# LabJunBMI/E3-invaraint-diffusion-model

Hardware: AMD Instinct MI355X
Metric: denoising-steps/sec (batched pocket graphs) (higher is better)
Workload: dtype f32 storage and accumulation, f16x3 products (fp32 grade); 1 GPU; structure_model sampling step, 256 x 256-residue pockets per GPU, 12+12 layers x 768, T=1000 schedule, encoder recomputed every step (as the reference); pockets_per_gpu=256, seq_len=256, parallelism=pocket-sharded x1, no collective

## Files before the change

### e3-invaraint-diffusion-model_amd/autograd.py

```python
import os

import torch

from . import hip, ops
from .ops import _chk, _p, _stream


def gemm_general(a, a_kmajor, b, b_kmajor, M, N, K, bias=None, act=ops.ACT_NONE, mode=None):
    _chk(a, "gemm_general.a"); _chk(b, "gemm_general.b"); _chk(bias, "gemm_general.bias")
    assert a.dim() == 2 and b.dim() == 2 and a.stride(1) == 1 and b.stride(1) == 1
    out = torch.empty((M, N), device=a.device, dtype=torch.float32)
    terms = ops.GEMM_MODES[ops.GEMM_MODE if mode is None else mode] or 6
    hip.check(hip.lib().e3d_gemm_f32_split_general(_p(a), a.stride(0), int(a_kmajor), _p(b), b.stride(0),
                                                   int(b_kmajor), _p(bias), _p(out), out.stride(0), M, N, K, act,
                                                   terms, _stream()), "e3d_gemm_f32_split_general")
    return out


class deferred_weight_grads:
    active = None

    MAX_BYTES = int(float(os.environ.get("E3D_DEFER_WGRAD_MAX_GB", "16")) * 2 ** 30)

    OVERLAP = os.environ.get("E3D_WGRAD_OVERLAP", "0") == "1"
# ... 406 lines not shown
    @staticmethod
    def forward(ctx, x, residual, gamma, beta, eps, p_drop=0.0, row_keys=None):
        ctx.drop = ops.site_drop(p_drop, row_keys) if p_drop and p_drop > 0 else None
        out, s = ops.residual_layernorm(x, residual, gamma, beta, eps, want_s=True, drop=ctx.drop)
        ctx.save_for_backward(s, gamma)
        ctx.eps, ctx.has_res = eps, residual is not None
        return out

    @staticmethod
    def backward(ctx, dy):
        s, gamma = ctx.saved_tensors
        if ctx.drop is not None:
            ds, dg, db, dsd = layernorm_bwd(dy.contiguous(), s, gamma, ctx.eps, drop=ctx.drop)
            return dsd, (ds if ctx.has_res else None), dg, db, None, None, None
        ds, dg, db = layernorm_bwd(dy.contiguous(), s, gamma, ctx.eps)
        return ds, (ds if ctx.has_res else None), dg, db, None, None, None


class _AdaLNGate(torch.autograd.Function):
    @staticmethod
    def forward(ctx, x, y, mod, branch, rows_per_cond):
        ctx.save_for_backward(y, mod)
        ctx.branch, ctx.rpc = branch, rows_per_cond
        return ops.adaln_gate(x, y, mod, branch, rows_per_cond)

    @staticmethod
    def backward(ctx, dout):
        y, mod = ctx.saved_tensors
        dout = dout.contiguous()
        M, H = y.shape
        dy = torch.empty_like(y)
        dmod = torch.zeros_like(mod)
        hip.check(hip.lib().e3d_adaln_gate_bwd(_p(dout), _p(y), _p(mod), ctx.branch, ctx.rpc, _p(dy), _p(dmod), M, H,
                                               _stream()), "e3d_adaln_gate_bwd")
        return dout, dy, dmod, None, None


class _EmbedLayerNorm(torch.autograd.Function):

    @staticmethod
    def forward(ctx, x, weight, bias, gamma, beta, eps, post_add, rows_per_add):
        out, z = ops.embed_layernorm(x, weight, bias, gamma, beta, eps, post_add, rows_per_add, want_z=True)
        ctx.save_for_backward(x, z, gamma)
        ctx.eps, ctx.rpa, ctx.has_add = eps, rows_per_add, post_add is not None
        return out

    @staticmethod
    def backward(ctx, dout):
        x, z, gamma = ctx.saved_tensors
        dout = dout.contiguous()
        dz, dg, db_ln = layernorm_bwd(dout, z, gamma, ctx.eps)
        dW, db = small_k_wgrad(dz, x)
        dadd = group_sum(dout, ctx.rpa) if (ctx.has_add and ctx.needs_input_grad[6]) else None
        return None, dW, db, dg, db_ln, None, dadd, None


class _HeadLinear(torch.autograd.Function):
    @staticmethod
    def forward(ctx, x, weight, bias):
        ctx.save_for_backward(x, weight)
        return ops.head_linear(x, weight, bias)

    @staticmethod
    def backward(ctx, dout):
        x, weight = ctx.saved_tensors
        dout = dout.contiguous()
        M, H = x.shape
        dx = torch.empty_like(x)
        hip.check(hip.lib().e3d_head_linear_bwd_dx(_p(dout), _p(weight), _p(dx), M, H, weight.shape[0], _stream()),
                  "e3d_head_linear_bwd_dx")
        dW, _ = small_k_wgrad(x, dout, transpose_out=True, want_bias=False)
        return dx, dW, colsum(dout)


FUSE_HIDDEN_DROPOUT = os.environ.get("E3D_FUSE_HIDDEN_DROPOUT", "1") == "1"


def _needs_grad(*tensors):
    return torch.is_grad_enabled() and any(t is not None and t.requires_grad for t in tensors)


class functional:
    @staticmethod
    def linear(x, weight, bias=None, act=ops.ACT_NONE, absmax=None, planes_for=None):
        if _needs_grad(x, weight, bias):
            out = _Linear.apply(x, weight, bias, act, absmax)
        elif planes_for is not None and absmax is None and ops.gemm_planes_ok(x, weight, bias, act, planes_for[0].shape[0],
                                                                              planes_for[1]):
            return ops.gemm(x, weight, bias, act, planes_out=True)
        else:
            out = ops.gemm(x, weight, bias, act, absmax=absmax)
        if absmax is not None:
            out._e3d_absmax = absmax
        return out

    @staticmethod
    def attention(q_src, kv_src, B, nh, Lq, Lk, key_mask=None, dist_emb=None, max_pos=0, drop_p=0.0, row_keys=None,
                  planes_for=None):
        q_abs = getattr(q_src, "_e3d_absmax", None)
        k_abs = q_abs if kv_src is None else getattr(kv_src, "_e3d_absmax", None)
        bounds = (q_abs, k_abs) if q_abs is not None and k_abs is not None else None
        if _needs_grad(q_src, kv_src, dist_emb):
            return _Attention.apply(q_src, kv_src, dist_emb, key_mask, B, nh, Lq, Lk, max_pos, drop_p, bounds, row_keys)
        q, k, v = _Attention._views(q_src, kv_src, nh * 64)
        drop = ops.site_drop(drop_p, row_keys) if drop_p > 0 else None
        planes = (planes_for is not None and drop is None and
                  ops.attention_planes_ok(q, k, v, nh, Lq, Lk, planes_for[0].shape[0], planes_for[1]))
        return ops.attention(q, k, v, B, nh, Lq, Lk, key_mask=key_mask, dist_emb=dist_emb, max_pos=max_pos, drop=drop,
                             bounds=bounds, planes_out=planes)

    @staticmethod
    def dropout(x, p, training=True, row_keys=None):
        if not training or not p:
            return x
        if _needs_grad(x):
            return _Dropout.apply(x, p, row_keys)
        p, seed = ops.site_drop(p, row_keys)[:2]
        return ops.dropout(x.contiguous(), p, seed, row_keys=row_keys)

    @staticmethod
    def residual_layernorm(x, residual, gamma, beta, eps, p_drop=0.0, row_keys=None):
        if _needs_grad(x, residual, gamma, beta):
            return _ResidualLayerNorm.apply(x, residual, gamma, beta, eps, p_drop, row_keys)
        drop = ops.site_drop(p_drop, row_keys) if p_drop and p_drop > 0 else None
        return ops.residual_layernorm(x, residual, gamma, beta, eps, drop=drop)

    @staticmethod
    def linear_residual_layernorm(x, weight, bias, residual, gamma, beta, eps, p_drop=0.0, row_keys=None):
        if not p_drop and not _needs_grad(x, weight, bias, residual, gamma, beta):
            return ops.linear_residual_layernorm(x, weight, bias, residual, gamma, beta, eps)
        fn = functional
        if FUSE_HIDDEN_DROPOUT:
            return fn.residual_layernorm(fn.linear(x, weight, bias), residual, gamma, beta, eps, p_drop, row_keys)
        return fn.residual_layernorm(fn.dropout(fn.linear(x, weight, bias), p_drop, row_keys=row_keys), residual, gamma, beta, eps)

    @staticmethod
    def adaln_gate(x, y, mod, branch, rows_per_cond):
        if _needs_grad(x, y, mod):
            return _AdaLNGate.apply(x, y, mod, branch, rows_per_cond)
        return ops.adaln_gate(x, y, mod, branch, rows_per_cond)

    @staticmethod
    def embed_layernorm(x, weight, bias, gamma, beta, eps, post_add=None, rows_per_add=1):
        if _needs_grad(weight, bias, gamma, beta, post_add):
            return _EmbedLayerNorm.apply(x, weight, bias, gamma, beta, eps, post_add, rows_per_add)
        return ops.embed_layernorm(x, weight, bias, gamma, beta, eps, post_add, rows_per_add)

    @staticmethod
    def head_linear(x, weight, bias):
        if _needs_grad(x, weight, bias):
            return _HeadLinear.apply(x, weight, bias)
        return ops.head_linear(x, weight, bias)
```

### e3-invaraint-diffusion-model_amd/bert.py

```python
from dataclasses import dataclass

import os

import torch
from torch import nn

from . import ops
from .autograd import functional as F


@dataclass
class BertConfig:
    hidden_size: int = 768
    num_attention_heads: int = 12
    intermediate_size: int = 1024
    num_hidden_layers: int = 12
    max_position_embeddings: int = 64
    position_embedding_type: str = "relative_key"
    hidden_dropout_prob: float = 0.1
    attention_probs_dropout_prob: float = 0.1
    layer_norm_eps: float = 1e-12
    hidden_act: str = "gelu"
    use_cache: bool = False
    is_decoder: bool = False
# ... 92 lines not shown

    @staticmethod
    def backward(ctx, gw, gb):
        gws = gw.split(ctx.rows, 0) if gw is not None else (None,) * ctx.n
        gbs = gb.split(ctx.rows, 0) if gb is not None else (None,) * ctx.n
        return (None, None, None) + tuple(gws) + tuple(gbs)


def _tie(owner, name, tensors):
    tied = owner.__dict__.setdefault("_e3d_tied", {})
    ent = tied.get(name)
    ok = ent is not None and ent.device == tensors[0].device
    if ok:
        at = ent.data_ptr()
        for t in tensors:
            if t.data_ptr() != at or not t.is_contiguous():
                ok = False
                break
            at += 4 * t.numel()
    if not ok:
        with torch.no_grad():
            ent = torch.cat([t.detach() for t in tensors], dim=0).contiguous()
            r0 = 0
            for t in tensors:
                t.data = ent[r0:r0 + t.shape[0]]
                r0 += t.shape[0]
        tied[name] = ent
    return ent


def _packed(owner, name, weights, biases):
    if torch.is_grad_enabled() and any(t.requires_grad for t in weights):
        if TIE_PACKED and all(t.dtype == torch.float32 for t in list(weights) + list(biases)):
            w, b = _TiedPack.apply(_tie(owner, "w_" + name, weights), _tie(owner, "b_" + name, biases), len(weights),
                                   *weights, *biases)
        else:
            w, b = torch.cat(list(weights), dim=0), torch.cat(list(biases), dim=0)
        w._e3d_parts, b._e3d_parts = list(weights), list(biases)
        return w, b
    out = []
    cache = owner.__dict__.setdefault("_e3d_pack", {})
    for key_name, tensors in (("w_" + name, weights), ("b_" + name, biases)):
        key = ops.weight_key(*tensors)
        hit = cache.get(key_name)
        if hit is None or hit[0] != key:
            with torch.no_grad():
                hit = (key, torch.cat([t.detach() for t in tensors], dim=0).contiguous())
            cache[key_name] = hit
        out.append(hit[1])
    return out[0], out[1]


def qkv_weights(sa):
    return _packed(sa, "qkv", [sa.query.weight, sa.key.weight, sa.value.weight], [sa.query.bias, sa.key.bias, sa.value.bias])


def kv_weights(sa):
    return _packed(sa, "kv", [sa.key.weight, sa.value.weight], [sa.key.bias, sa.value.bias])


def dropout_rates(module):
    if not module.training:
        return 0.0, 0.0
    cfg = module.config
    return float(getattr(cfg, "hidden_dropout_prob", 0.0)), float(getattr(cfg, "attention_probs_dropout_prob", 0.0))


def _attention_output(att, ctx, x, p_hidden=0.0, row_keys=None):
    return F.linear_residual_layernorm(ctx, att.output.dense.weight, att.output.dense.bias, x, att.output.LayerNorm.weight,
                                       att.output.LayerNorm.bias, att.eps, p_hidden, row_keys)


def _planes_for(att, x, drop):
    return (att.output.dense.weight, x) if drop[0] == 0 and drop[1] == 0 else None


def drop_keys(drop):
    return drop[2] if len(drop) > 2 else None


def run_self_attention(att, x, mask, B, L, drop=(0.0, 0.0), layout=None):
    sa = att.self
    w, b = qkv_weights(sa)
    qkv = F.linear(x, w, b, absmax=ops.absmax_slot(sa, "qkv", x.device))
    relkey = sa.position_embedding_type == "relative_key"
    if layout is not None:
        H = att.num_heads * 64
        ctx = ops.attention_varlen(qkv[:, :H], qkv[:, H:2 * H], qkv[:, 2 * H:], layout, layout, att.num_heads,
                                   dist_emb=sa.distance_embedding.weight if relkey else None,
                                   max_pos=sa.max_position_embeddings)
        return _attention_output(att, ctx, x)
    ctx = F.attention(qkv, None, B, att.num_heads, L, L, key_mask=mask,
                      dist_emb=sa.distance_embedding.weight if relkey else None,
                      max_pos=sa.max_position_embeddings, drop_p=drop[1], row_keys=drop_keys(drop),
                      planes_for=_planes_for(att, x, drop))
    return _attention_output(att, ctx, x, drop[0], drop_keys(drop))


def project_cross_kv(att, enc):
    w, b = kv_weights(att.self)
    return F.linear(enc, w, b, absmax=torch.zeros(1, device=enc.device, dtype=torch.float32))


def run_cross_attention(att, x, kv, enc_mask, B, Lq, Lk, drop=(0.0, 0.0), layout=None, enc_layout=None):
    q = F.linear(x, att.self.query.weight, att.self.query.bias, absmax=ops.absmax_slot(att.self, "q", x.device))
    if layout is not None:
        H = att.num_heads * 64
        ctx = ops.attention_varlen(q, kv[:, :H], kv[:, H:], layout, enc_layout, att.num_heads)
        return _attention_output(att, ctx, x)
    ctx = F.attention(q, kv, B, att.num_heads, Lq, Lk, key_mask=enc_mask, drop_p=drop[1], row_keys=drop_keys(drop),
                      planes_for=_planes_for(att, x, drop))
    return _attention_output(att, ctx, x, drop[0], drop_keys(drop))


def run_layer(layer, x, mask, B, L, cross_kv=None, enc_mask=None, Lk=None, drop=(0.0, 0.0), layout=None,
              enc_layout=None):
    x = run_self_attention(layer.attention, x, mask, B, L, drop, layout=layout)
    if hasattr(layer, "crossattention"):
        if cross_kv is None:
            raise ValueError("decoder layer needs encoder states")
        x = run_cross_attention(layer.crossattention, x, cross_kv, enc_mask, B, L, Lk, drop, layout=layout,
                                enc_layout=enc_layout)
    inter = F.linear(x, layer.intermediate.dense.weight, layer.intermediate.dense.bias, ops.ACT_GELU,
                     planes_for=(layer.output.dense.weight, x) if drop[0] == 0 and drop[1] == 0 else None)
    return F.linear_residual_layernorm(inter, layer.output.dense.weight, layer.output.dense.bias, x,
                                       layer.output.LayerNorm.weight, layer.output.LayerNorm.bias, layer.eps, drop[0],
                                       drop_keys(drop))


def run_encoder(encoder, x, mask, B, L, enc=None, enc_mask=None, Lk=None, cross_kv=None, layout=None, enc_layout=None,
                row_keys=None):
    drop = dropout_rates(encoder)
    if layout is not None and drop != (0.0, 0.0):
        raise RuntimeError("packed layouts are inference-only: put the model in eval mode")
    if row_keys is not None:
        drop = drop + (row_keys,)
    for i, layer in enumerate(encoder.layer):
        kv = None
        if hasattr(layer, "crossattention"):
            kv = cross_kv[i] if cross_kv is not None else project_cross_kv(layer.crossattention, enc)
        x = run_layer(layer, x, mask, B, L, kv, enc_mask, Lk, drop, layout=layout, enc_layout=enc_layout)
    return x
```

### e3-invaraint-diffusion-model_amd/csrc/attn_relkey_coop.hip

```cpp
#include <type_traits>

#include "e3d_common.h"

namespace {

typedef __bf16 bf16x8 __attribute__((ext_vector_type(8)));
typedef __bf16 bf16x4 __attribute__((ext_vector_type(4)));
typedef _Float16 f16x8 __attribute__((ext_vector_type(8)));
typedef _Float16 f16x4 __attribute__((ext_vector_type(4)));
template <typename E> struct AV;
template <> struct AV<__bf16> { typedef bf16x8 x8; typedef bf16x4 x4; };
template <> struct AV<_Float16> { typedef f16x8 x8; typedef f16x4 x4; };
template <typename X> struct Elem;
template <> struct Elem<bf16x8> { typedef __bf16 type; };
template <> struct Elem<bf16x4> { typedef __bf16 type; };
template <> struct Elem<f16x8> { typedef _Float16 type; };
template <> struct Elem<f16x4> { typedef _Float16 type; };
__device__ __forceinline__ f32x16 mma16(const bf16x8 a, const bf16x8 b, const f32x16 c) {
    return __builtin_amdgcn_mfma_f32_32x32x16_bf16(a, b, c, 0, 0, 0);
}
__device__ __forceinline__ f32x16 mma16(const f16x8 a, const f16x8 b, const f32x16 c) {
    return __builtin_amdgcn_mfma_f32_32x32x16_f16(a, b, c, 0, 0, 0);
}

constexpr int D = 64;
constexpr int RING_LD = 34;
constexpr int RING_F = 64 * RING_LD;
constexpr int OUT_LD = 68;
constexpr int K_ROW_B = 144;
constexpr int V_ROW_B = 192;
constexpr int K_PLANE_B = 32 * K_ROW_B, V_PLANE_B = 32 * V_ROW_B;
constexpr float LOG2E = 1.4426950408889634f, LN2 = 0.6931471805599453f;
constexpr float Q_SCALE = 0.125f * LOG2E;
constexpr float MASK_BIAS = -10000.0f * LOG2E;
float g_rescale_tau = 8.0f;
constexpr int KV_BUF_B = 2 * K_PLANE_B + 2 * V_PLANE_B + 128;

template <typename X4>
__device__ __forceinline__ void split4x2(const f32x4 v, X4& hi, X4& lo) {
    typedef typename Elem<X4>::type E;
#pragma unroll
    for (int j = 0; j < 4; ++j) {
        const E p = (E)v[j];
        hi[j] = p;
        lo[j] = (E)(v[j] - (float)p);
    }
}

template <typename X8>
__device__ __forceinline__ void split8x2(const float (&x)[8], X8& hi, X8& lo) {
    typedef typename Elem<X8>::type E;
#pragma unroll
    for (int j = 0; j < 8; ++j) {
        const E p = (E)x[j];
        hi[j] = p;
        lo[j] = (E)(x[j] - (float)p);
    }
}

__device__ __forceinline__ void split4x2(const f32x4 v, f16x4& hi, f16x4& lo) {
    e3d_f16x2 h0, l0, h1, l1;
    e3d_split2_f16(v[0], v[1], h0, l0);
    e3d_split2_f16(v[2], v[3], h1, l1);
    hi = f16x4{h0[0], h0[1], h1[0], h1[1]};
    lo = f16x4{l0[0], l0[1], l1[0], l1[1]};
}
__device__ __forceinline__ void split8x2(const float (&x)[8], f16x8& hi, f16x8& lo) {
#pragma unroll
    for (int j = 0; j < 8; j += 2) {
        e3d_f16x2 h, l;
        e3d_split2_f16(x[j], x[j + 1], h, l);
        hi[j] = h[0]; hi[j + 1] = h[1];
        lo[j] = l[0]; lo[j + 1] = l[1];
    }
}

template <typename X8>
__device__ __forceinline__ f32x16 mfma3(const X8 (&a)[2], const X8 (&b)[2], f32x16 acc) {
    acc = mma16(a[0], b[1], acc);
    acc = mma16(a[1], b[0], acc);
    acc = mma16(a[0], b[0], acc);
    return acc;
}

typedef short short4v __attribute__((ext_vector_type(4)));
typedef short short8v __attribute__((ext_vector_type(8)));
template <typename X8>
__device__ __forceinline__ X8 tr_read8(const unsigned char* lo4, const unsigned char* hi4) {
    typedef __attribute__((address_space(3))) short4v* lds_p;
    const short4v a = __builtin_amdgcn_ds_read_tr16_b64_v4i16((lds_p)(lo4));
    const short4v b = __builtin_amdgcn_ds_read_tr16_b64_v4i16((lds_p)(hi4));
    const short8v c = __builtin_shufflevector(a, b, 0, 1, 2, 3, 4, 5, 6, 7);
    return __builtin_bit_cast(X8, c);
}

template <typename E>
__global__ __launch_bounds__(256) void e_fragments_kernel(const float* __restrict__ e, typename AV<E>::x8* __restrict__ frag,
                                                          int P, int J0, int n_items, float* __restrict__ e_absmax) {
    const int i = blockIdx.x * 256 + threadIdx.x;
    if (i >= n_items) return;
    const int lane = i & 63, kb = (i >> 6) & 3, plane = (i >> 8) & 1, j = i >> 9;
    const int row = min(max(P + 32 * (j - J0) + (lane & 31), 0), 2 * P - 2);
    const float* src = e + row * D + 16 * kb + 8 * (lane >> 5);
    typename AV<E>::x8 out;
    unsigned amax = 0;
#pragma unroll
    for (int t = 0; t < 8; ++t) {
        const float v = src[t];
        const E hi = (E)v;
        out[t] = plane ? (E)(v - (float)hi) : hi;
        e3d_absmax_accum(amax, v);
    }
    frag[i] = out;
    if (e_absmax && plane == 0) e3d_absmax_commit(amax, e_absmax, lane);
}

#ifdef E3D_ATTN_STAMPS
__device__ long long e3d_attn_stamps[16][8];
#define ASTAMP(slot)                                                                                     \
    do {                                                                                                 \
        if (blockIdx.x == 1000 && wid == 1 && lane == 0 && kt < 16) e3d_attn_stamps[kt][slot] = __builtin_readcyclecounter(); \
    } while (0)
#define KSTAMP(i)                                                                                        \
    do {                                                                                                 \
        if (blockIdx.x == 1000 && wid == 1 && lane == 0) e3d_attn_stamps[15][i] = __builtin_readcyclecounter(); \
    } while (0)
#else
#define ASTAMP(slot) do {} while (0)
#define KSTAMP(i) do {} while (0)
#endif

template <int W, bool RELKEY, typename E, bool DROP = false, bool PLANES = false>
__global__ __launch_bounds__(W * 64, 2) void attn_coop_kernel(
    const float* __restrict__ q, int64_t q_bs, int64_t q_rs, const float* __restrict__ k, int64_t k_bs,
    int64_t k_rs, const float* __restrict__ v, int64_t v_bs, int64_t v_rs, const typename AV<E>::x8* __restrict__ e_frag,
    int P, const float* __restrict__ key_mask, float* __restrict__ out, float* __restrict__ lse, int nh, int Lq, int Lk,
    int groups_per_bh, int skip_padded_tiles, E3dBounds bnd, float rescale_tau, E3dDrop drop_in) {
    const E3dDrop drop = e3d_drop_resolve(drop_in);
    typedef typename AV<E>::x8 bf16x8;
    typedef typename AV<E>::x4 bf16x4;
    extern __shared__ __attribute__((aligned(16))) unsigned char smem_raw[];
    constexpr int NT = W * 64, NI = 512 / NT;
    const int tid = threadIdx.x, lane = tid & 63, wid = tid >> 6;
    const int qi = lane & 31, half = lane >> 5;
    const int blk = xcd_remap(blockIdx.x, gridDim.x);
    const int grp = blk % groups_per_bh, bh = blk / groups_per_bh, h = bh % nh, b = bh / nh;
    const int q0 = (grp * W + wid) * 32;
    float* ring = reinterpret_cast<float*>(smem_raw + 2 * KV_BUF_B) + wid * RING_F;
    KSTAMP(0);

    const float* kb_ = k + b * k_bs + h * D;
    const float* vb_ = v + b * v_bs + h * D;
    const float* mb = key_mask ? key_mask + (int64_t)b * Lk : nullptr;
    f32x4 qraw[8];
    {
        const float* qrow = q + b * q_bs + (int64_t)min(q0 + qi, Lq - 1) * q_rs + h * D + 8 * half;
#pragma unroll
        for (int kb = 0; kb < 4; ++kb) {
            qraw[2 * kb] = *reinterpret_cast<const f32x4*>(qrow + 16 * kb);
            qraw[2 * kb + 1] = *reinterpret_cast<const f32x4*>(qrow + 16 * kb + 4);
        }
    }
    uint64_t drop_row = 0;
    if (DROP) drop_row = e3d_drop_attn_row(drop, b, h, nh, Lq, Lk, min(q0 + qi, Lq - 1));
    const bool scan_mask = mb && skip_padded_tiles && e3d_mask_skip_is_exact(bnd);
    float mv[4];
    {
        const float* mp = mb ? mb : kb_;
#pragma unroll
        for (int c = 0; c < 4; ++c) mv[c] = mp[min(64 * c + lane, Lk - 1)];
    }

    bf16x8 qf[4][2];
    int k_tiles = (Lk + 31) >> 5;

    constexpr bool DEEP = NI <= 2;
    constexpr int NSET = DEEP ? 2 : 1;
    f32x4 sk[NSET][NI], sv[NSET][NI];
    float smask[NSET];
    int voff_k[NI], voff_v[NI];
#pragma unroll
    for (int i = 0; i < NI; ++i) {
        const int f = tid + NT * i;
        voff_k[i] = ((f >> 4) * (int)k_rs + 4 * (f & 15)) * 4;
        voff_v[i] = ((f >> 4) * (int)v_rs + 4 * (f & 15)) * 4;
    }
    const int voff_m = (tid & 31) * 4;
    auto tile_rsrc = [&](const float* base, int64_t rs, int r0, int tail_floats) {
        const int rows = Lk - r0;
        return __builtin_amdgcn_make_buffer_rsrc(const_cast<float*>(base + (int64_t)r0 * rs), 0,
                                                 (int)(((int64_t)(rows - 1) * rs + tail_floats) * 4), 0x00020000);
    };
    auto stage_load = [&](auto set_tag, int r0) {
        constexpr int SET = decltype(set_tag)::value;
        const auto rk = tile_rsrc(kb_, k_rs, r0, D), rv = tile_rsrc(vb_, v_rs, r0, D);
#pragma unroll
        for (int i = 0; i < NI; ++i) {
            sk[SET][i] = __builtin_bit_cast(f32x4, __builtin_amdgcn_raw_buffer_load_b128(rk, voff_k[i], 0, 0));
            sv[SET][i] = __builtin_bit_cast(f32x4, __builtin_amdgcn_raw_buffer_load_b128(rv, voff_v[i], 0, 0));
        }
        const auto rm = tile_rsrc(mb ? mb : kb_, 1, r0, 1);
        const float mval = __builtin_bit_cast(float, __builtin_amdgcn_raw_buffer_load_b32(rm, voff_m, 0, 0));
        smask[SET] = mb ? mval : 1.0f;
    };
    auto stage_store = [&](auto set_tag, int r0, unsigned char* buf) {
        constexpr int SET = decltype(set_tag)::value;
#pragma unroll
        for (int i = 0; i < NI; ++i) {
            const int f = tid + NT * i, row = f >> 4, c4 = f & 15;
            bf16x4 hi, lo;
            split4x2(sk[SET][i], hi, lo);
            *reinterpret_cast<bf16x4*>(buf + row * K_ROW_B + 8 * c4) = hi;
            *reinterpret_cast<bf16x4*>(buf + K_PLANE_B + row * K_ROW_B + 8 * c4) = lo;
            split4x2(sv[SET][i], hi, lo);
            *reinterpret_cast<bf16x4*>(buf + 2 * K_PLANE_B + row * V_ROW_B + 8 * c4) = hi;
            *reinterpret_cast<bf16x4*>(buf + 2 * K_PLANE_B + V_PLANE_B + row * V_ROW_B + 8 * c4) = lo;
        }
        if (tid < 32)
            reinterpret_cast<float*>(buf + 2 * K_PLANE_B + 2 * V_PLANE_B)[tid] =
                r0 + tid < Lk ? (1.0f - smask[SET]) * MASK_BIAS : -INFINITY;
    };
    using Set0 = std::integral_constant<int, 0>;
    using Set1 = std::integral_constant<int, DEEP ? 1 : 0>;

    bf16x8 ef[4][2];
    const int J0 = (Lk + 31) >> 5, qt = q0 >> 5;
    const auto e_rsrc = __builtin_amdgcn_make_buffer_rsrc(const_cast<bf16x8*>(e_frag ? e_frag : reinterpret_cast<const bf16x8*>(k)), 0,
                                                          2 * ((Lk + 31) >> 5) * 512 * 16, 0x00020000);
    const int voff_e = lane * 16;
    auto e_load = [&](int j) {
        const int so = __builtin_amdgcn_readfirstlane(j * 8192);
#pragma unroll
        for (int kb = 0; kb < 4; ++kb) {
            ef[kb][0] = __builtin_bit_cast(bf16x8, __builtin_amdgcn_raw_buffer_load_b128(e_rsrc, voff_e + kb * 1024, so, 0));
            ef[kb][1] = __builtin_bit_cast(bf16x8, __builtin_amdgcn_raw_buffer_load_b128(e_rsrc, voff_e + kb * 1024, so + 4096, 0));
        }
    };
    auto dot_q_acc = [&](const bf16x8 (&x)[4][2], f32x16 acc) {
#pragma unroll
        for (int kb = 0; kb < 4; ++kb) acc = mfma3(x[kb], qf[kb], acc);
        return acc;
    };
    auto dot_q = [&](const bf16x8 (&x)[4][2]) {
        f32x16 acc;
#pragma unroll
        for (int r = 0; r < 16; ++r) acc[r] = 0.f;
        return dot_q_acc(x, acc);
    };

    stage_load(Set0{}, 0);
    if (RELKEY) e_load(qt + J0);

    if (scan_mask) {
        int last = -1;
#pragma unroll
        for (int c = 0; c < 4; ++c) {
            const bool valid = 64 * c + lane < Lk && mv[c] != 0.f;
            const unsigned long long bits = __ballot(valid);
            if (bits) last = 64 * c + 63 - __builtin_clzll(bits);
        }
        for (int base = 256; base < Lk; base += 64) {
            const int key = base + lane;
            const bool valid = key < Lk && mb[key] != 0.f;
            const unsigned long long bits = __ballot(valid);
            if (bits) last = base + 63 - __builtin_clzll(bits);
        }
        if (last >= 0) k_tiles = (last >> 5) + 1;
    }
#pragma unroll
    for (int kb = 0; kb < 4; ++kb) {
        const f32x4 lo4 = qraw[2 * kb], hi4 = qraw[2 * kb + 1];
        float x[8] = {lo4[0] * Q_SCALE, lo4[1] * Q_SCALE, lo4[2] * Q_SCALE, lo4[3] * Q_SCALE,
                      hi4[0] * Q_SCALE, hi4[1] * Q_SCALE, hi4[2] * Q_SCALE, hi4[3] * Q_SCALE};
#pragma unroll
        for (int j = 0; j < 8; ++j) asm volatile("" : "+v"(x[j]));
        split8x2(x, qf[kb][0], qf[kb][1]);
    }
    if (RELKEY) {
        f32x16 t = dot_q(ef);
        e_load(qt - 1 + J0);
#pragma unroll
        for (int r = 0; r < 16; ++r) ring[(32 + mfma32_row(r, half)) * RING_LD + qi] = t[r];
        t = dot_q(ef);
        e_load(qt - (k_tiles > 1 ? 1 : 0) - 1 + J0);
#pragma unroll
        for (int r = 0; r < 16; ++r) ring[mfma32_row(r, half) * RING_LD + qi] = t[r];
    }
    stage_store(Set0{}, 0, smem_raw);
    if (DEEP) stage_load(Set1{}, (k_tiles > 1 ? 1 : 0) * 32);
    __syncthreads();
    KSTAMP(1);

    f32x16 o0, o1;
#pragma unroll
    for (int r = 0; r < 16; ++r) { o0[r] = 0.f; o1[r] = 0.f; }
    float m_run = 0.f, l_run = 0.f;
    float* const ring_w = ring + 4 * half * RING_LD + qi;
    const float* const ring_e = ring + (qi + 31 - 4 * half - 27) * RING_LD + qi;
    int rd_odd[16];
    if (RELKEY) {
#pragma unroll
        for (int r = 0; r < 16; ++r) rd_odd[r] = (((qi - mfma32_row(r, half) + 31) ^ 32) * RING_LD + qi);
    }

    auto tile = [&](auto par_tag, int kt) {
        constexpr int PAR = decltype(par_tag)::value;
        const unsigned char* buf = smem_raw + PAR * KV_BUF_B;
        const bool more = kt + 1 < k_tiles;
        const int kt_next = more ? kt + 1 : kt;
        ASTAMP(0);
        ASTAMP(1);

        const float* kbias = reinterpret_cast<const float*>(buf + 2 * K_PLANE_B + 2 * V_PLANE_B);
        f32x16 s;
#pragma unroll
        for (int g = 0; g < 4; ++g) {
            const f32x4 bv = *reinterpret_cast<const f32x4*>(kbias + 8 * g + 4 * half);
#pragma unroll
            for (int j = 0; j < 4; ++j) s[4 * g + j] = bv[j] - m_run;
        }
        if (RELKEY) {
#pragma unroll
            for (int r = 0; r < 16; ++r)
                s[r] += PAR ? ring[rd_odd[r]] : ring_e[(27 - ((r & 3) + 8 * (r >> 2))) * RING_LD];
        }
        {
            bf16x8 kf[4][2];
            const unsigned char* kr = buf + qi * K_ROW_B + 16 * half;
#pragma unroll
            for (int kb = 0; kb < 4; ++kb) {
                kf[kb][0] = *reinterpret_cast<const bf16x8*>(kr + 32 * kb);
                kf[kb][1] = *reinterpret_cast<const bf16x8*>(kr + K_PLANE_B + 32 * kb);
            }
            s = dot_q_acc(kf, s);
        }
        ASTAMP(2);
        const int kt_ld = DEEP ? (kt + 2 < k_tiles ? kt + 2 : k_tiles - 1) : kt_next;
        if (PAR == 0) stage_load(Set0{}, kt_ld * 32);
        else stage_load(Set1{}, kt_ld * 32);
        ASTAMP(3);

        float tmax = -INFINITY;
#pragma unroll
        for (int r = 0; r < 16; ++r) tmax = fmaxf(tmax, s[r]);
        tmax = fmaxf(tmax, __shfl_xor(tmax, 32, 64));
        const bool grow = kt == 0 || tmax > rescale_tau;
        if (__builtin_amdgcn_ballot_w64(grow) != 0ull) {
            const float delta = grow ? tmax : 0.f;
            const float alpha = kt == 0 ? 0.f : __builtin_amdgcn_exp2f(-delta);
            m_run += delta;
            l_run *= alpha;
#pragma unroll
            for (int r = 0; r < 16; ++r) { o0[r] *= alpha; o1[r] *= alpha; s[r] -= delta; }
        }
        float psum = 0.f;
#pragma unroll
        for (int r = 0; r < 16; ++r) {
            s[r] = __builtin_amdgcn_exp2f(s[r]);
            psum += s[r];
        }
        l_run += psum;
        if (DROP) {
#pragma unroll
            for (int g = 0; g < 4; ++g) {
                float m[4];
                e3d_drop_mult4_row(drop, drop_row, (uint32_t)(kt * 8 + 2 * g + half), m);
#pragma unroll
                for (int j = 0; j < 4; ++j) s[4 * g + j] *= m[j];
            }
        }
        ASTAMP(4);

        const unsigned char* vr = buf + 2 * K_PLANE_B + (4 * half + ((lane >> 2) & 3)) * V_ROW_B +
                                  2 * (16 * ((lane >> 4) & 1) + 4 * (lane & 3));
#pragma unroll
        for (int st = 0; st < 2; ++st) {
            float pv[8];
#pragma unroll
            for (int j = 0; j < 8; ++j) pv[j] = s[8 * st + j];
            bf16x8 pb[2], a0[2], a1[2];
            split8x2(pv, pb[0], pb[1]);
            const unsigned char* v0 = vr + 16 * st * V_ROW_B;
#pragma unroll
            for (int pl = 0; pl < 2; ++pl) {
                a0[pl] = tr_read8<bf16x8>(v0 + pl * V_PLANE_B, v0 + pl * V_PLANE_B + 8 * V_ROW_B);
                a1[pl] = tr_read8<bf16x8>(v0 + pl * V_PLANE_B + 64, v0 + pl * V_PLANE_B + 8 * V_ROW_B + 64);
            }
            o0 = mfma3(a0, pb, o0);
            o1 = mfma3(a1, pb, o1);
        }

        ASTAMP(5);
        if (more) {
            if (DEEP == (PAR == 0)) stage_store(Set1{}, kt_next * 32, smem_raw + (PAR ^ 1) * KV_BUF_B);
            else stage_store(Set0{}, kt_next * 32, smem_raw + (PAR ^ 1) * KV_BUF_B);
        }
        ASTAMP(6);
        if (RELKEY && more) {
            const f32x16 t = dot_q(ef);
            e_load(qt - (kt + 2 < k_tiles ? kt + 2 : k_tiles - 1) - 1 + J0);
#pragma unroll
            for (int r = 0; r < 16; ++r) ring_w[(32 * (PAR ^ 1) + (r & 3) + 8 * (r >> 2)) * RING_LD] = t[r];
        }
        __syncthreads();
        ASTAMP(7);
    };
    for (int kt = 0; kt < k_tiles; kt += 2) {
        tile(std::integral_constant<int, 0>{}, kt);
        if (kt + 1 < k_tiles) tile(std::integral_constant<int, 1>{}, kt + 1);
    }

    KSTAMP(2);
    const float l_tot = l_run + __shfl_xor(l_run, 32, 64);
    const float inv = 1.0f / l_tot;
    if constexpr (PLANES) {
        unsigned char* pb = reinterpret_cast<unsigned char*>(out) +
                            ((((int64_t)b * Lq + q0) >> 5) * (nh * 4) + 4 * h) * 2048 + lane * 16;
#pragma unroll
        for (int ks = 0; ks < 4; ++ks) {
            const int r0 = 8 * (ks & 1);
            float x[8];
#pragma unroll
            for (int j = 0; j < 4; ++j) {
                float a = (ks < 2 ? o0[r0 + j] : o1[r0 + j]) * inv, c = (ks < 2 ? o0[r0 + 4 + j] : o1[r0 + 4 + j]) * inv;
                asm volatile("" : "+v"(a));
                asm volatile("" : "+v"(c));
                const auto sw = __builtin_amdgcn_permlane32_swap(__float_as_uint(a), __float_as_uint(c), false, false);
                x[j] = __uint_as_float(sw[0]);
                x[4 + j] = __uint_as_float(sw[1]);
            }
            bf16x8 hi, lo;
            split8x2(x, hi, lo);
            *reinterpret_cast<bf16x8*>(pb + ks * 2048) = hi;
            *reinterpret_cast<bf16x8*>(pb + ks * 2048 + 1024) = lo;
        }
        if (lse && half == 0 && q0 + qi < Lq) lse[((int64_t)b * nh + h) * Lq + q0 + qi] = m_run * LN2 + logf(l_tot);
        return;
    }
    __builtin_amdgcn_wave_barrier();
#pragma unroll
    for (int g = 0; g < 4; ++g) {
        f32x4 a, c;
#pragma unroll
        for (int j = 0; j < 4; ++j) { a[j] = o0[4 * g + j] * inv; c[j] = o1[4 * g + j] * inv; }
        *reinterpret_cast<f32x4*>(ring + qi * OUT_LD + 8 * g + 4 * half) = a;
        *reinterpret_cast<f32x4*>(ring + qi * OUT_LD + 32 + 8 * g + 4 * half) = c;
    }
    __builtin_amdgcn_fence(__ATOMIC_RELEASE, "wavefront");
    __builtin_amdgcn_wave_barrier();
    __builtin_amdgcn_fence(__ATOMIC_ACQUIRE, "wavefront");
    float* obase = out + ((int64_t)b * Lq + q0) * (nh * D) + h * D;
#pragma unroll
    for (int i = 0; i < 8; ++i) {
        const int row = 4 * i + (lane >> 4);
        if (q0 + row < Lq)
            *reinterpret_cast<f32x4*>(obase + (int64_t)row * (nh * D) + 4 * (lane & 15)) =
                *reinterpret_cast<const f32x4*>(ring + row * OUT_LD + 4 * (lane & 15));
    }
    if (lse && half == 0 && q0 + qi < Lq) lse[((int64_t)b * nh + h) * Lq + q0 + qi] = m_run * LN2 + logf(l_tot);
    KSTAMP(3);
#ifdef E3D_ATTN_STAMPS
    asm volatile("s_waitcnt vmcnt(0)" ::: "memory");
    KSTAMP(4);
#endif
}

template <int W, bool RELKEY, typename E>
int launch_w(const E3dAttnFwd& a, const void* e_frag, int skip, E3dBounds bnd, const E3dAttnDrop& drop, bool planes,
             hipStream_t s) {
    const size_t lds = 2 * KV_BUF_B + (size_t)W * RING_F * sizeof(float);
    const int groups = (a.Lq + 31) / 32 / W;
    auto go = [&](auto kernel, std::atomic<uint64_t>& ok, const char* what) {
        e3d_allow_lds(ok, kernel, lds);
        hipLaunchKernelGGL(kernel, dim3(a.B * a.nh * groups), dim3(W * 64), lds, s, E3D_VIEW(a.q), E3D_VIEW(a.k), E3D_VIEW(a.v),
                           reinterpret_cast<const typename AV<E>::x8*>(e_frag), a.P, a.key_mask, a.out, a.lse, a.nh, a.Lq, a.Lk,
                           groups, skip, bnd, g_rescale_tau, drop.d);
        return e3d_launch_status(what);
    };
    if (planes) {
        if constexpr (W == 4) {
            static std::atomic<uint64_t> lds_ok_p{0};
            if (!drop.on() && a.Lq % 32 == 0)
                return go(attn_coop_kernel<W, RELKEY, E, false, true>, lds_ok_p, "e3d_relkey_attn_fwd_split_planes (cooperative)");
        }
        e3d_set_error("attn_coop: plane output exists for the 4-wave inference forms with Lq %% 32 == 0 only");
        return -1;
    }
    if constexpr (std::is_same<E, __bf16>::value) {
        static std::atomic<uint64_t> lds_ok_d{0};
        if (drop.on()) return go(attn_coop_kernel<W, RELKEY, E, true>, lds_ok_d, "e3d_relkey_attn_fwd_split (cooperative, dropout)");
    }
    static std::atomic<uint64_t> lds_ok{0};
    return go(attn_coop_kernel<W, RELKEY, E>, lds_ok, "e3d_relkey_attn_fwd_split (cooperative)");
}

template <bool RELKEY, typename E>
int launch_any(int W, const E3dAttnFwd& a, const void* e_frag, int skip, E3dBounds bnd, const E3dAttnDrop& drop, bool planes,
               hipStream_t s) {
    if (W == 8) return launch_w<8, RELKEY, E>(a, e_frag, skip, bnd, drop, planes, s);
    return launch_w<4, RELKEY, E>(a, e_frag, skip, bnd, drop, planes, s);
}

}

template <typename E>
static int coop_launch_t(const E3dAttnFwd& a, int skip, E3dBounds bnd, void* e_scratch, int e_ready, const E3dAttnDrop& drop,
                         bool planes, hipStream_t s) {
    const int q_tiles = (a.Lq + 31) / 32;
    static int w_pref = 0;
    if (!w_pref) {
        const char* e = getenv("E3D_ATTN_W");
        w_pref = e ? atoi(e) : 4;
    }
    const int W = (w_pref == 8 && q_tiles % 8 == 0) ? 8 : 4;
    if (!a.dist_emb) return launch_any<false, E>(W, a, nullptr, skip, bnd, drop, planes, s);
    if (!e_scratch) {
        e3d_set_error("attn_coop: rel-key attention needs the caller's scratch for the distance-table planes");
        return -1;
    }
    const int J0 = (a.Lk + 31) / 32, n_items = 2 * J0 * 512;
    if (!e_ready)
        hipLaunchKernelGGL(e_fragments_kernel<E>, dim3((n_items + 255) / 256), dim3(256), 0, s, a.dist_emb,
                           reinterpret_cast<typename AV<E>::x8*>(e_scratch), a.P, J0, n_items, (float*)nullptr);
    return launch_any<true, E>(W, a, e_scratch, skip, bnd, drop, planes, s);
}

int e3d_attn_coop_waves(int Lq) {
    const char* e = getenv("E3D_ATTN_W");
    return ((e ? atoi(e) : 4) == 8 && ((Lq + 31) / 32) % 8 == 0) ? 8 : 4;
}

int e3d_attn_coop_launch(const E3dAttnFwd& a, int skip, E3dBounds bnd, void* e_scratch, int e_ready, int f16,
                         const E3dAttnDrop& drop, bool planes, hipStream_t s) {
    if (f16) return coop_launch_t<_Float16>(a, skip, bnd, e_scratch, e_ready, drop, planes, s);
    return coop_launch_t<__bf16>(a, skip, bnd, e_scratch, e_ready, drop, planes, s);
}

extern "C" float e3d_attn_rescale_tau(float tau) {
    const float prev = g_rescale_tau;
    if (tau >= 0.f) g_rescale_tau = tau;
    return prev;
}

#ifdef E3D_ATTN_STAMPS
extern "C" int e3d_debug_read_attn_stamps(long long* host_out) {
    return (int)hipMemcpyFromSymbol(host_out, HIP_SYMBOL(e3d_attn_stamps), sizeof(long long) * 16 * 8);
}
#endif

int e3d_attn_fill_planes(const float* dist_emb, int P, int Lk, void* scratch, int f16, float* e_absmax, hipStream_t s) {
    const int J0 = (Lk + 31) / 32, n_items = 2 * J0 * 512;
    if (f16)
        hipLaunchKernelGGL(e_fragments_kernel<_Float16>, dim3((n_items + 255) / 256), dim3(256), 0, s, dist_emb,
                           reinterpret_cast<f16x8*>(scratch), P, J0, n_items, e_absmax);
    else
        hipLaunchKernelGGL(e_fragments_kernel<__bf16>, dim3((n_items + 255) / 256), dim3(256), 0, s, dist_emb,
                           reinterpret_cast<bf16x8*>(scratch), P, J0, n_items, e_absmax);
    return e3d_launch_status("e3d_relkey_attn_fwd_split (distance-table planes)");
}

extern "C" int64_t e3d_attn_scratch_bytes(int Lk) { return (int64_t)2 * ((Lk + 31) / 32) * 512 * 16; }
```

### e3-invaraint-diffusion-model_amd/csrc/attn_relkey_split.hip

```cpp
#include "attn_split_frag.h"

namespace {

template <int NS, bool RELKEY, bool DROP, typename E>
__global__ __launch_bounds__(256, 2) void attn_fwd_split_kernel(
    const float* __restrict__ q, int64_t q_bs, int64_t q_rs, const float* __restrict__ k, int64_t k_bs,
    int64_t k_rs, const float* __restrict__ v, int64_t v_bs, int64_t v_rs, const float* __restrict__ dist_emb,
    int P, const float* __restrict__ key_mask, float* __restrict__ out, float* __restrict__ lse, int nh, int Lq,
    int Lk, int q_tiles, int n_units, int skip_padded_tiles, E3dBounds bnd, E3dDrop drop_in) {
    const E3dDrop drop = e3d_drop_resolve(drop_in);
    typedef typename AV<E>::x8 bf16x8;
    extern __shared__ __attribute__((aligned(16))) float smem[];
    const int lane = threadIdx.x & 63, wid = threadIdx.x >> 6;
    const int qi = lane & 31, half = lane >> 5;
    const int unit = xcd_remap(blockIdx.x, gridDim.x) * (blockDim.x >> 6) + wid;
    if (unit >= n_units) return;
    const int qt = unit % q_tiles, bh = unit / q_tiles, h = bh % nh, b = bh / nh;
    float* ring = smem + wid * WAVE_LDS_F;
    float* stg = ring + RING_F;
    float* kbias = stg + STG_F;

    const int q0 = qt * 32;
    const int lq = min(q0 + qi, Lq - 1);
    uint64_t drop_row = 0;
// ... 204 lines not shown
    hipStream_t s = (hipStream_t)stream;
    if (a.dist_emb && e_scratch && !e_scratch_ready) {
        const int rc = e3d_attn_fill_planes(a.dist_emb, a.P, a.Lk, e_scratch, f16, e_absmax, s);
        if (rc) return rc;
        e_scratch_ready = 1;
    }
    if (attn_coop_ok(a.k.rs, a.v.bs, a.v.rs, a.Lq, a.Lk, terms, drop.on(), !a.dist_emb || e_scratch))
        return e3d_attn_coop_launch(a, g_skip_padded, bnd, e_scratch, e_scratch_ready, f16, drop, planes_out, s);
    E3D_REQUIRE(!planes_out, "attn_split: plane output needs the cooperative kernel (e3d_attn_planes_supported)");
    if (drop.on())
        return terms == 3 ? launch<2, true>(a, bnd, s, drop.d) : launch<3, true>(a, bnd, s, drop.d);
    if (f16) return launch<2, false, _Float16>(a, bnd, s);
    return terms == 3 ? launch<2>(a, bnd, s) : launch<3>(a, bnd, s);
}

extern "C" int e3d_relkey_attn_fwd_split_ex(const float* q, int64_t q_bs, int64_t q_rs, const float* k, int64_t k_bs,
                                            int64_t k_rs, const float* v, int64_t v_bs, int64_t v_rs,
                                            const float* dist_emb, int P, const float* key_mask, float* out,
                                            float* lse, int B, int nh, int Lq, int Lk, int terms, float drop_p,
                                            uint64_t drop_seed, void* e_scratch, int e_scratch_ready, const float* q_absmax,
                                            const float* k_absmax, float* e_absmax, void* stream) {
    return attn_fwd_dispatch({{q, q_bs, q_rs}, {k, k_bs, k_rs}, {v, v_bs, v_rs}, dist_emb, P, key_mask, out, lse, B, nh, Lq, Lk},
                             terms, {drop_p, e3d_drop_make(drop_p, drop_seed)}, e_scratch, e_scratch_ready, q_absmax, k_absmax,
                             e_absmax, stream);
}

extern "C" int e3d_relkey_attn_fwd_split_ex_keyed(const float* q, int64_t q_bs, int64_t q_rs, const float* k, int64_t k_bs,
                                                  int64_t k_rs, const float* v, int64_t v_bs, int64_t v_rs,
                                                  const float* dist_emb, int P, const float* key_mask, float* out,
                                                  float* lse, int B, int nh, int Lq, int Lk, int terms, float drop_p,
                                                  uint32_t site, const uint64_t* row_keys, void* e_scratch, int e_scratch_ready,
                                                  const float* q_absmax, const float* k_absmax, float* e_absmax, void* stream) {
    E3D_REQUIRE(row_keys && drop_p > 0.f, "attn_split (keyed): row keys and drop_p > 0 required");
    E3D_REQUIRE(site < E3D_DROP_MAX_SITE && nh < E3D_DROP_MAX_HEADS, "attn_split (keyed): site %u / %d heads out of range", site, nh);
    return attn_fwd_dispatch({{q, q_bs, q_rs}, {k, k_bs, k_rs}, {v, v_bs, v_rs}, dist_emb, P, key_mask, out, lse, B, nh, Lq, Lk},
                             terms, {drop_p, e3d_drop_make_keyed(drop_p, site, row_keys)}, e_scratch, e_scratch_ready, q_absmax,
                             k_absmax, e_absmax, stream);
}

extern "C" int e3d_relkey_attn_fwd_split(const float* q, int64_t q_bs, int64_t q_rs, const float* k, int64_t k_bs,
                                         int64_t k_rs, const float* v, int64_t v_bs, int64_t v_rs,
                                         const float* dist_emb, int P, const float* key_mask, float* out, float* lse,
                                         int B, int nh, int Lq, int Lk, int terms, void* stream) {
    return e3d_relkey_attn_fwd_split_ex(q, q_bs, q_rs, k, k_bs, k_rs, v, v_bs, v_rs, dist_emb, P, key_mask, out, lse, B,
                                        nh, Lq, Lk, terms, 0.f, 0, nullptr, 0, nullptr, nullptr, nullptr, stream);
}

extern "C" int e3d_relkey_attn_fwd_split_drop(const float* q, int64_t q_bs, int64_t q_rs, const float* k, int64_t k_bs,
                                              int64_t k_rs, const float* v, int64_t v_bs, int64_t v_rs,
                                              const float* dist_emb, int P, const float* key_mask, float* out,
                                              float* lse, int B, int nh, int Lq, int Lk, int terms, float drop_p,
                                              uint64_t drop_seed, void* stream) {
    return e3d_relkey_attn_fwd_split_ex(q, q_bs, q_rs, k, k_bs, k_rs, v, v_bs, v_rs, dist_emb, P, key_mask, out, lse, B,
                                        nh, Lq, Lk, terms, drop_p, drop_seed, nullptr, 0, nullptr, nullptr, nullptr, stream);
}

extern "C" int e3d_relkey_attn_fwd_split_drop_keyed(const float* q, int64_t q_bs, int64_t q_rs, const float* k, int64_t k_bs,
                                                    int64_t k_rs, const float* v, int64_t v_bs, int64_t v_rs,
                                                    const float* dist_emb, int P, const float* key_mask, float* out,
                                                    float* lse, int B, int nh, int Lq, int Lk, int terms, float drop_p,
                                                    uint32_t site, const uint64_t* row_keys, void* stream) {
    return e3d_relkey_attn_fwd_split_ex_keyed(q, q_bs, q_rs, k, k_bs, k_rs, v, v_bs, v_rs, dist_emb, P, key_mask, out, lse, B,
                                              nh, Lq, Lk, terms, drop_p, site, row_keys, nullptr, 0, nullptr, nullptr, nullptr,
                                              stream);
}

extern "C" int e3d_attn_planes_supported(int64_t k_rs, int64_t v_bs, int64_t v_rs, int Lq, int Lk, int terms, int have_scratch) {
    return (terms == 3 || terms == E3D_TERMS_F16X3) && Lq > 0 && Lq % 32 == 0 && Lk > 0 &&
           attn_coop_ok(k_rs, v_bs, v_rs, Lq, Lk, terms, false, have_scratch != 0) && e3d_attn_coop_waves(Lq) == 4;
}

extern "C" int e3d_relkey_attn_fwd_split_planes(const float* q, int64_t q_bs, int64_t q_rs, const float* k, int64_t k_bs,
                                                int64_t k_rs, const float* v, int64_t v_bs, int64_t v_rs,
                                                const float* dist_emb, int P, const float* key_mask, void* out_planes,
                                                int B, int nh, int Lq, int Lk, int terms, void* e_scratch, int e_scratch_ready,
                                                const float* q_absmax, const float* k_absmax, float* e_absmax, void* stream) {
    E3D_REQUIRE(e3d_attn_planes_supported(k_rs, v_bs, v_rs, Lq, Lk, terms, !dist_emb || e_scratch),
                "attn_split (planes): this call does not land on the 4-wave cooperative kernel (Lq=%d Lk=%d terms=%d)", Lq, Lk, terms);
    return attn_fwd_dispatch({{q, q_bs, q_rs}, {k, k_bs, k_rs}, {v, v_bs, v_rs}, dist_emb, P, key_mask,
                              reinterpret_cast<float*>(out_planes), nullptr, B, nh, Lq, Lk},
                             terms, {0.f, e3d_drop_make(0.f, 0)}, e_scratch, e_scratch_ready, q_absmax, k_absmax, e_absmax, stream,
                             true);
}
```

### e3-invaraint-diffusion-model_amd/csrc/e3d_common.h

```cpp
#pragma once
#include <hip/hip_runtime.h>
#include <stdint.h>
#include <stdio.h>
#include <math.h>
#include <atomic>
#include <type_traits>

#include "../../include/e3d_hip.h"

typedef float f32x4 __attribute__((ext_vector_type(4)));
typedef float f32x16 __attribute__((ext_vector_type(16)));

void e3d_set_error(const char* fmt, ...);

struct E3dBounds { const float* q; const float* k; const float* e; };


#define E3D_REQUIRE(cond, ...)       \
    do {                             \
        if (!(cond)) {               \
            e3d_set_error(__VA_ARGS__); \
            return -1;               \
        }                            \
    } while (0)
// ... 136 lines not shown
    return d;
}
#define E3D_DROP_MAX_SITE (1u << 24)
#define E3D_DROP_MAX_HEADS (1 << 16)
static inline E3dDrop e3d_drop_make_keyed(float p, uint32_t site, const uint64_t* row_keys) {
    E3dDrop d = e3d_drop_make(p, 0);
    d.epoch = nullptr;
    d.row_keys = row_keys;
    d.site = (uint64_t)site << 40;
    return d;
}
__device__ __forceinline__ E3dDrop e3d_drop_resolve(E3dDrop d) {
    if (d.epoch) d.seed += *d.epoch * 0xD1342543DE82EF95ull;
    d.epoch = nullptr;
    return d;
}
__device__ __forceinline__ void e3d_drop_mult4_row(const E3dDrop d, uint64_t row_term, uint32_t group, float (&m)[4]) {
    uint64_t z = row_term + group;
    z = (z ^ (z >> 30)) * 0xBF58476D1CE4E5B9ull;
    z = (z ^ (z >> 27)) * 0x94D049BB133111EBull;
    z ^= z >> 31;
#pragma unroll
    for (int j = 0; j < 4; ++j) m[j] = ((uint32_t)(z >> (16 * j)) & 0xFFFFu) >= d.thr ? d.scale : 0.f;
}
__device__ __forceinline__ uint64_t e3d_drop_hidden_row(const E3dDrop d, int64_t row, int H4) {
    if (d.row_keys) return d.row_keys[row] * 0x9E3779B97F4A7C15ull + 0x9E3779B97F4A7C15ull + d.site;
    return (uint64_t)row * (uint64_t)H4 + d.seed * 0x9E3779B97F4A7C15ull + 0x9E3779B97F4A7C15ull;
}
__device__ __forceinline__ uint64_t e3d_drop_attn_row(const E3dDrop d, int b, int h, int nh, int Lq, int Lk, int q) {
    if (d.row_keys)
        return d.row_keys[(int64_t)b * Lq + q] * 0x9E3779B97F4A7C15ull + 0x9E3779B97F4A7C15ull + (d.site | (uint64_t)h << 24);
    return ((uint64_t)(b * nh + h) * Lq + q) * (uint64_t)((Lk + 3) >> 2) + d.seed * 0x9E3779B97F4A7C15ull +
           0x9E3779B97F4A7C15ull;
}
__device__ __forceinline__ void e3d_drop_mult4(const E3dDrop d, uint64_t idx4, float (&m)[4]) {
    uint64_t z = idx4 + d.seed * 0x9E3779B97F4A7C15ull + 0x9E3779B97F4A7C15ull;
    z = (z ^ (z >> 30)) * 0xBF58476D1CE4E5B9ull;
    z = (z ^ (z >> 27)) * 0x94D049BB133111EBull;
    z ^= z >> 31;
#pragma unroll
    for (int j = 0; j < 4; ++j) m[j] = ((uint32_t)(z >> (16 * j)) & 0xFFFFu) >= d.thr ? d.scale : 0.f;
}

int e3d_attn_fill_planes(const float* dist_emb, int P, int Lk, void* scratch, int f16, float* e_absmax, hipStream_t s);

template <typename T>
struct E3dViewT { T* p; int64_t bs, rs; };
typedef E3dViewT<const float> E3dView;
typedef E3dViewT<float> E3dGradView;
#define E3D_VIEW(x) (x).p, (x).bs, (x).rs
struct E3dAttnFwd {
    E3dView q, k, v;
    const float* dist_emb; int P; const float* key_mask;
    float *out, *lse;
    int B, nh, Lq, Lk;
};
struct E3dAttnBwd {
    E3dView q, k, v;
    const float* dist_emb; int P; const float* key_mask;
    const float *out, *lse, *dout;
    E3dGradView dq, dk, dv;
    float* d_dist_emb;
    int B, nh, Lq, Lk;
};
struct E3dAttnDrop {
    float p;
    E3dDrop d;
    bool on() const { return p > 0.f; }
};
template <typename F>
static inline void e3d_attn_form(bool relkey, bool dropping, F&& f) {
    if (relkey) {
        if (dropping) f(std::true_type{}, std::true_type{});
        else f(std::true_type{}, std::false_type{});
    } else {
        if (dropping) f(std::false_type{}, std::true_type{});
        else f(std::false_type{}, std::false_type{});
    }
}

int e3d_attn_coop_launch(const E3dAttnFwd& a, int skip, E3dBounds bnd, void* e_scratch, int e_ready, int f16,
                         const E3dAttnDrop& drop, bool planes, hipStream_t s);
int e3d_attn_coop_waves(int Lq);

struct E3dBwdLayout { int64_t Pm, dSm, part, chunk_sums, unit_live, total; };
E3dBwdLayout e3d_attn_bwd_layout(int B, int nh, int Lq, int Lk, bool relkey);

int e3d_attn_bwd_split_launch(const E3dAttnBwd& a, float* workspace, const E3dBwdLayout& w, const E3dAttnDrop& drop,
                              hipStream_t s);

bool e3d_attn_bwd_coop_supported(int Lq, int Lk, bool dropping);
int e3d_attn_bwd_coop_launch(const E3dAttnBwd& a, float* workspace, const E3dBwdLayout& w, const E3dAttnDrop& drop,
                             hipStream_t s);

__device__ __forceinline__ int xcd_remap(int id, int n) {
    const int q = n >> 3, r = n & 7, xcd = id & 7, slot = id >> 3;
    return (xcd < r ? xcd * (q + 1) : r * (q + 1) + (xcd - r) * q) + slot;
}
```

### e3-invaraint-diffusion-model_amd/csrc/gemm_split.hip

```cpp
#include <type_traits>

#include "e3d_common.h"

namespace {

typedef __bf16 bf16x8 __attribute__((ext_vector_type(8)));
typedef __bf16 bf16x4 __attribute__((ext_vector_type(4)));
typedef _Float16 f16x8 __attribute__((ext_vector_type(8)));
typedef _Float16 f16x4 __attribute__((ext_vector_type(4)));

template <typename E> struct Vec;
template <> struct Vec<__bf16> { typedef bf16x8 x8; typedef bf16x4 x4; };
template <> struct Vec<_Float16> { typedef f16x8 x8; typedef f16x4 x4; };
__device__ __forceinline__ f32x16 mma16(const bf16x8 a, const bf16x8 b, const f32x16 c) {
    return __builtin_amdgcn_mfma_f32_32x32x16_bf16(a, b, c, 0, 0, 0);
}
__device__ __forceinline__ f32x16 mma16(const f16x8 a, const f16x8 b, const f32x16 c) {
    return __builtin_amdgcn_mfma_f32_32x32x16_f16(a, b, c, 0, 0, 0);
}

struct Epi { float* absmax; float scale; int plan_m = 0; const int* run_if = nullptr; };

constexpr int BN = 128, BK = 32;
#ifdef GEMM_STAMPS
// ... 635 lines not shown
                            item_load(i, kt2);
                        }
                }
#pragma unroll
                for (int n = 0; n < 2; ++n) {
                    if constexpr (NS == 3) {
                        acc[m][n] = mma16(fa[1][m], fb[1][n], acc[m][n]);
                        acc[m][n] = mma16(fa[0][m], fb[NS - 1][n], acc[m][n]);
                        acc[m][n] = mma16(fa[NS - 1][m], fb[0][n], acc[m][n]);
                    }
                    if constexpr (NS >= 2) {
                        acc[m][n] = mma16(fa[0][m], fb[1][n], acc[m][n]);
                        acc[m][n] = mma16(fa[1][m], fb[0][n], acc[m][n]);
                    }
                    acc[m][n] = mma16(fa[0][m], fb[0][n], acc[m][n]);
                }
                if (PIPE) __builtin_amdgcn_sched_barrier(0);
            }
            STAMP(2 + ks);
        }
        if (PIPE) {
            STAMP(5);
            __syncthreads();
            STAMP(6);
            cur ^= 1;
        } else if (NBUF == 2) {
#ifdef E3D_STAMPS
            asm volatile("s_waitcnt vmcnt(0)" ::: "memory");
            STAMP(4);
#endif
            if (more) {
#pragma unroll
                for (int i = 0; i < NI; ++i) item_store(i, next);
            }
            STAMP(5);
            __syncthreads();
            STAMP(6);
            cur ^= 1;
        } else {
            __syncthreads();
            if (more) {
#pragma unroll
                for (int i = 0; i < NI; ++i) item_store(i, smem_raw);
            }
            __syncthreads();
        }
    }

    STAMP_K(3);
    unsigned amax = 0;
#pragma unroll
    for (int m = 0; m < 4; ++m) {
#pragma unroll
        for (int n = 0; n < 2; ++n) {
            const int col = col0 + wc * 64 + n * 32 + l31;
            const float bv = bias ? bias[col] : 0.f;
#pragma unroll
            for (int r = 0; r < 16; ++r) {
                const int row = row0 + wr * 128 + m * 32 + mfma32_row(r, half);
                float v = fmaf(acc[m][n][r], out_scale, bv);
                if (ACT == E3D_ACT_GELU) v = gelu_erf(v);
                if (ACT == E3D_ACT_SILU) v = silu(v);
                if (row < M) {
                    out[(int64_t)row * ldc + col] = v;
                    if (ACT == E3D_ACT_NONE && absmax) e3d_absmax_accum(amax, v);
                }
            }
        }
    }
    if (ACT == E3D_ACT_NONE && absmax) e3d_absmax_commit(amax, absmax, lane);
    STAMP_K(4);
#ifdef E3D_STAMPS
    asm volatile("s_waitcnt vmcnt(0)" ::: "memory");
    STAMP_K(5);
#endif
}

#ifdef E3D_NT_STORES
#define E3D_STORE_OUT(ptr, val) __builtin_nontemporal_store((val), (ptr))
#else
#define E3D_STORE_OUT(ptr, val) (*(ptr) = (val))
#endif

template <int ACT, typename E, bool PLANES = false>
__global__ __launch_bounds__(512, 2) void gemm_split256p_kernel(const float* __restrict__ A, int64_t lda,
                                                                 const float* __restrict__ W,
                                                                 const float* __restrict__ bias,
                                                                 float* __restrict__ out, int64_t ldc, int N, int K,
                                                                 int tiles_m, int tiles_n, float* __restrict__ absmax, float out_scale,
                                                                 const int* __restrict__ run_if) {
    if (run_if && *run_if == 0) return;
    extern __shared__ __attribute__((aligned(16))) unsigned char smem_raw[];
    constexpr int NS = 2, T_BYTES = BT * ROW64, BUF_BYTES = 2 * NS * T_BYTES;
    constexpr int NI = 8;
    const int total = tiles_m * tiles_n, nk = K / BK;
    const int tid = threadIdx.x, lane = tid & 63, wid = tid >> 6;
    const int wr = wid >> 2, wc = wid & 3;
    const int l31 = lane & 31, half = lane >> 5;

    unsigned goff[NI];
    int dst[NI];
#pragma unroll
    for (int i = 0; i < NI; ++i) {
        const int f = tid + 512 * (i & 3), r = f >> 3, kg = f & 7;
        goff[i] = (unsigned)(r * (i < 4 ? (int)lda : K) + kg * 4);
        dst[i] = (i < 4 ? 0 : NS * T_BYTES) + swz_off(r, kg >> 1) + (kg & 1) * 8;
    }

    int ld_tile = blockIdx.x, ld_k = 0;
    const float* ld_a;
    const float* ld_w;
    auto cursor_bases = [&]() {
        const int lid = xcd_remap(ld_tile, total);
        ld_a = A + (int64_t)(lid / tiles_n) * BT * lda + ld_k * BK;
        ld_w = W + (int64_t)(lid % tiles_n) * BT * K + ld_k * BK;
    };
    auto cursor_advance = [&]() {
        if (ld_k + 1 < nk) {
            ++ld_k;
            ld_a += BK;
            ld_w += BK;
        } else if (ld_tile + (int)gridDim.x < total) {
            ld_tile += gridDim.x;
            ld_k = 0;
            cursor_bases();
        }
    };
    f32x4 rg[NI];
    auto item_load = [&](int i) { rg[i] = *reinterpret_cast<const f32x4*>((i < 4 ? ld_a : ld_w) + goff[i]); };
    auto item_store = [&](int i, unsigned char* buf) {
        typename Vec<E>::x4 p[NS];
        split4<NS, E>(rg[i], p);
#pragma unroll
        for (int s = 0; s < NS; ++s) *reinterpret_cast<typename Vec<E>::x4*>(buf + s * T_BYTES + dst[i]) = p[s];
    };
    cursor_bases();
#pragma unroll
    for (int i = 0; i < NI; ++i) item_load(i);
    cursor_advance();
#pragma unroll
    for (int i = 0; i < NI; ++i) item_store(i, smem_raw);
#pragma unroll
    for (int i = 0; i < NI; ++i) item_load(i);
    cursor_advance();
    __syncthreads();

    int a_row[4], b_row[2];
#pragma unroll
    for (int m = 0; m < 4; ++m) a_row[m] = wr * 128 + m * 32 + l31;
#pragma unroll
    for (int n = 0; n < 2; ++n) b_row[n] = wc * 64 + n * 32 + l31;
    int cur = 0;
    unsigned amax = 0;

    for (int tile = blockIdx.x; tile < total; tile += gridDim.x) {
        f32x16 acc[4][2];
#pragma unroll
        for (int m = 0; m < 4; ++m)
#pragma unroll
            for (int n = 0; n < 2; ++n)
#pragma unroll
                for (int r = 0; r < 16; ++r) acc[m][n][r] = 0.f;
        for (int kt = 0; kt < nk; ++kt) {
            const unsigned char* base = smem_raw + cur * BUF_BYTES;
            unsigned char* next = smem_raw + (cur ^ 1) * BUF_BYTES;
#pragma unroll
            for (int ks = 0; ks < 2; ++ks) {
                typename Vec<E>::x8 fa[NS][4], fb[NS][2];
#pragma unroll
                for (int s = 0; s < NS; ++s) {
#pragma unroll
                    for (int n = 0; n < 2; ++n)
                        fb[s][n] = *reinterpret_cast<const typename Vec<E>::x8*>(base + (NS + s) * T_BYTES +
                                                                    swz_off(b_row[n], 2 * ks + half));
#pragma unroll
                    for (int m = 0; m < 4; ++m)
                        fa[s][m] = *reinterpret_cast<const typename Vec<E>::x8*>(base + s * T_BYTES + swz_off(a_row[m], 2 * ks + half));
                }
#pragma unroll
                for (int m = 0; m < 4; ++m) {
                    const int g = ks * 4 + m;
                    item_store(g, next);
                    item_load(g);
#pragma unroll
                    for (int n = 0; n < 2; ++n) {
                        if constexpr (PLANES) {
                            acc[m][n] = mma16(fb[1][n], fa[0][m], acc[m][n]);
                            acc[m][n] = mma16(fb[0][n], fa[1][m], acc[m][n]);
                            acc[m][n] = mma16(fb[0][n], fa[0][m], acc[m][n]);
                        } else {
                            acc[m][n] = mma16(fa[0][m], fb[1][n], acc[m][n]);
                            acc[m][n] = mma16(fa[1][m], fb[0][n], acc[m][n]);
                            acc[m][n] = mma16(fa[0][m], fb[0][n], acc[m][n]);
                        }
                    }
                    __builtin_amdgcn_sched_barrier(0);
                }
            }
            cursor_advance();
            __syncthreads();
            cur ^= 1;
        }

        if constexpr (PLANES) {
            const int lid = xcd_remap(tile, total);
            const int row0 = (lid / tiles_n) * BT, col0 = (lid % tiles_n) * BT;
            unsigned char* const ob = reinterpret_cast<unsigned char*>(out) + lane * 16;
            const int nks = N >> 4;
#pragma unroll
            for (int n = 0; n < 2; ++n) {
                const int colb = __builtin_amdgcn_readfirstlane(col0 + wc * 64 + n * 32);
                float bs[32];
#pragma unroll
                for (int c = 0; c < 32; ++c) bs[c] = 0.f;
                if (bias) {
#pragma unroll
                    for (int c = 0; c < 32; ++c) bs[c] = bias[colb + c];
                }
                float bl[16];
#pragma unroll
                for (int r = 0; r < 16; ++r) {
                    bl[r] = half ? bs[8 * (r >> 2) + 4 + (r & 3)] : bs[8 * (r >> 2) + (r & 3)];
                    asm volatile("" : "+v"(bl[r]));
                }
#pragma unroll
                for (int m = 0; m < 4; ++m) {
                    unsigned char* o = ob + ((int64_t)((row0 + wr * 128 + m * 32) >> 5) * nks + (colb >> 4)) * 2048;
#pragma unroll
                    for (int kl = 0; kl < 2; ++kl) {
                        f32x4 x0, x1;
#pragma unroll
                        for (int j = 0; j < 4; ++j) {
                            float a = fmaf(acc[m][n][8 * kl + j], out_scale, bl[8 * kl + j]);
                            float c = fmaf(acc[m][n][8 * kl + 4 + j], out_scale, bl[8 * kl + 4 + j]);
                            if (ACT == E3D_ACT_GELU) { a = gelu_erf(a); c = gelu_erf(c); }
                            if (ACT == E3D_ACT_SILU) { a = silu(a); c = silu(c); }
                            if (ACT == E3D_ACT_NONE && absmax) { e3d_absmax_accum(amax, a); e3d_absmax_accum(amax, c); }
                            asm volatile("" : "+v"(a));
                            asm volatile("" : "+v"(c));
                            const auto sw = __builtin_amdgcn_permlane32_swap(__float_as_uint(a), __float_as_uint(c), false, false);
                            x0[j] = __uint_as_float(sw[0]);
                            x1[j] = __uint_as_float(sw[1]);
                        }
                        typename Vec<E>::x4 p0[2], p1[2];
                        split4<2, E>(x0, p0);
                        split4<2, E>(x1, p1);
                        typedef typename Vec<E>::x8 X8;
                        *reinterpret_cast<X8*>(o + kl * 2048) = __builtin_shufflevector(p0[0], p1[0], 0, 1, 2, 3, 4, 5, 6, 7);
                        *reinterpret_cast<X8*>(o + kl * 2048 + 1024) = __builtin_shufflevector(p0[1], p1[1], 0, 1, 2, 3, 4, 5, 6, 7);
                    }
                }
            }
            continue;
        }
        const int lid = xcd_remap(tile, total);
        const int row0 = (lid / tiles_n) * BT, col0 = (lid % tiles_n) * BT;
#pragma unroll
        for (int m = 0; m < 4; ++m) {
#pragma unroll
            for (int n = 0; n < 2; ++n) {
                const int col = col0 + wc * 64 + n * 32 + l31;
                const float bv = bias ? bias[col] : 0.f;
                float* o = out + (int64_t)(row0 + wr * 128 + m * 32 + 4 * half) * ldc + col;
#pragma unroll
                for (int r = 0; r < 16; ++r) {
                    float v = fmaf(acc[m][n][r], out_scale, bv);
                    if (ACT == E3D_ACT_GELU) v = gelu_erf(v);
                    if (ACT == E3D_ACT_SILU) v = silu(v);
                    E3D_STORE_OUT(&o[(int64_t)((r & 3) + 8 * (r >> 2)) * ldc], v);
                    if (ACT == E3D_ACT_NONE && absmax) e3d_absmax_accum(amax, v);
                }
            }
        }
    }
    if (ACT == E3D_ACT_NONE && absmax) e3d_absmax_commit(amax, absmax, lane);
}

template <int ACT, typename E, bool PLANES = false>
int launch256p(const float* A, int64_t lda, const float* W, const float* bias, float* out, int64_t ldc, int M, int N,
               int K, Epi epi, hipStream_t s) {
    const int tiles_m = M / BT, tiles_n = N / BT;
    constexpr size_t lds = 2 * 2 * 2 * BT * ROW64;
    static std::atomic<uint64_t> lds_ok{0};
    const int n_cu = e3d_cu_count();
    const int total = tiles_m * tiles_n;
    e3d_allow_lds(lds_ok, gemm_split256p_kernel<ACT, E, PLANES>, lds);
    hipLaunchKernelGGL((gemm_split256p_kernel<ACT, E, PLANES>), dim3(total < n_cu ? total : n_cu), dim3(512), lds, s, A, lda, W, bias, out,
                       ldc, N, K, tiles_m, tiles_n, epi.absmax, epi.scale, epi.run_if);
    return e3d_launch_status(PLANES ? "e3d_gemm_bias_act_planes_split (persistent 256x256)" : "e3d_gemm_f32_split (persistent 256x256)");
}

int g_general_form = -1;
int g_tile_pref = -1;

template <int NS, int ACT, int WR, int WC, int NBUF, bool PIPE, typename E>
int launch256(const float* A, int64_t lda, const float* W, const float* bias, float* out, int64_t ldc, int M, int N,
              int K, Epi epi, hipStream_t s) {
    constexpr int TM = WR * 128, TN = WC * 64;
    const int tiles_m = (M + TM - 1) / TM, tiles_n = N / TN;
    const size_t lds = (size_t)NBUF * NS * (TM + TN) * ROW64;
    static std::atomic<uint64_t> lds_ok{0};
    e3d_allow_lds(lds_ok, gemm_split256_kernel<NS, ACT, WR, WC, NBUF, PIPE, E>, lds);
    hipLaunchKernelGGL((gemm_split256_kernel<NS, ACT, WR, WC, NBUF, PIPE, E>), dim3(tiles_m * tiles_n), dim3(WR * WC * 64), lds, s,
                       A, lda, W, bias, out, ldc, M, N, K, tiles_m, tiles_n, epi.absmax, epi.scale, epi.run_if);
    return e3d_launch_status("e3d_gemm_f32_split (128x64 wave tiles)");
}

template <int NS, int ACT, bool A_KMAJ, bool B_KMAJ, int WM, int WN, typename E, int TN = 2, bool TR = false>
int launch_general(const float* A, int64_t lda, const float* B, int64_t ldb, const float* bias, float* out, int64_t ldc,
                   int M, int N, int K, Epi epi, hipStream_t s);

int p_min() {
    static int v = 0;
    if (!v) {
        const char* e = getenv("E3D_GEMM_P_MIN");
        v = e ? atoi(e) : 160;
    }
    return v;
}

bool persistent_ok(int M, int Mp, int N, int K, int64_t lda, int64_t ldb, int k_min = 2 * BK) {
    if (g_tile_pref < 0) {
        const char* e = getenv("E3D_GEMM_TILE");
        g_tile_pref = e ? atoi(e) : 4;
    }
    const int64_t n_tiles = (int64_t)(Mp / BT) * (N / BT);
    return N % BT == 0 && M % BT == 0 && Mp % BT == 0 && ldb == K && g_tile_pref >= 4 && K >= k_min && lda < (1 << 22) &&
           (g_tile_pref >= 5 || n_tiles >= p_min() || (n_tiles >= 96 && N >= 6 * BT && !getenv("E3D_GEMM_P_MIN")));
}

template <int NS, int ACT, bool A_KMAJ, bool B_KMAJ, typename E>
int launch(const float* A, int64_t lda, const float* B, int64_t ldb, const float* bias, float* out, int64_t ldc,
           int M, int N, int K, Epi epi, hipStream_t s) {
    if (g_tile_pref < 0) {
        const char* e = getenv("E3D_GEMM_TILE");
        g_tile_pref = e ? atoi(e) : 4;
    }
    const int Mp = epi.plan_m > 0 ? epi.plan_m : M;
    if constexpr (!A_KMAJ && !B_KMAJ) {
        if constexpr (NS == 2) {
            if (persistent_ok(M, Mp, N, K, lda, ldb))
                return launch256p<ACT, E>(A, lda, B, bias, out, ldc, M, N, K, epi, s);
            if (N % BT == 0 && ldb == K && g_tile_pref >= 3 && (int64_t)((Mp + BT - 1) / BT) * (N / BT) >= 256)
                return launch256<NS, ACT, 2, 4, 2, true, E>(A, lda, B, bias, out, ldc, M, N, K, epi, s);
        }
        if constexpr (NS == 1) {
            if (N % BT == 0 && ldb == K && g_tile_pref >= 3 && (int64_t)((Mp + BT - 1) / BT) * (N / BT) >= 160)
                return launch256<NS, ACT, 2, 4, 2, true, E>(A, lda, B, bias, out, ldc, M, N, K, epi, s);
        }
        if (N % BT == 0 && ldb == K && g_tile_pref >= 1 &&
            (int64_t)((Mp + BT - 1) / BT) * (N / BT) >= 256)
            return launch256<NS, ACT, 2, 4, (NS <= 2 ? 2 : 1), false, E>(A, lda, B, bias, out, ldc, M, N, K, epi, s);
    }
    if (g_general_form < 0) {
        const char* e = getenv("E3D_GEMM_FORM");
        g_general_form = e ? atoi(e) : 0;
    }
    int form = g_general_form;
    if (form != 1 && form != 2 && form != 3 && form != 4) {
        const int64_t g256 = (int64_t)((Mp + 255) / 256) * ((N + 127) / 128), g128 = (int64_t)((Mp + 127) / 128) * ((N + 127) / 128);
        const int64_t cus = e3d_cu_count();
        if (NS == 3) form = g256 < 128 && !A_KMAJ && !B_KMAJ ? 2 : 1;
        else if (A_KMAJ && B_KMAJ) form = 1;
        else if (A_KMAJ) form = g128 <= cus ? 2 : (g256 <= cus ? 1 : (45 * ((g128 + 2 * cus - 1) / (2 * cus)) < 37 * ((g256 + cus - 1) / cus) ? 2 : 1));
        else form = 25 * ((g128 + cus - 1) / cus) <= 38 * ((g256 + cus - 1) / cus) ? 3 : 1;
        if (NS == 2 && !A_KMAJ && !B_KMAJ && Mp <= 2048 && N <= 1024) form = 4;
    }
    if constexpr (NS == 2 && !A_KMAJ && !B_KMAJ) {
        if (form == 4) return launch_general<NS, ACT, A_KMAJ, B_KMAJ, 2, 2, E, 1>(A, lda, B, ldb, bias, out, ldc, M, N, K, epi, s);
    }
    if (form == 4) form = 3;
// ... 201 lines not shown
                    "gemm_wgrad_ragged: bad shape in problem %d: N=%d K=%d ldz=%lld ldx=%lld", q, N[q], K[q], (long long)ldz[q],
                    (long long)ldx[q]);
        g.dz[p] = dz[q]; g.x[p] = x[q]; g.dw[p] = dw[q]; g.db[p] = db ? db[q] : nullptr;
        g.N[p] = N[q]; g.K[p] = K[q]; g.ldz[p] = (int)ldz[q]; g.ldx[p] = (int)ldx[q];
        g.tile_start[p] = (int)tiles;
        if (p < count) {
            tiles += (int64_t)((N[q] + 255) / 256) * ((K[q] + 127) / 128);
            tr = tr && N[q] % 4 == 0 && K[q] % 4 == 0 && ldz[q] % 4 == 0 && ldx[q] % 4 == 0 && ((uintptr_t)dz[q] % 16) == 0 &&
                 ((uintptr_t)x[q] % 16) == 0 && e3d_tr_span_ok(M, ldz[q]) && e3d_tr_span_ok(M, ldx[q]);
        }
    }
    E3D_REQUIRE(tiles < (1ll << 30), "gemm_wgrad_ragged: too many tiles");
    for (int p = count; p <= 64; ++p) g.tile_start[p] = (int)tiles;
    g.accumulate = accumulate_bits;
    const dim3 grid((unsigned)tiles), block(512);
    hipStream_t s = (hipStream_t)stream;
    auto go = [&](auto kern, size_t lds, std::atomic<uint64_t>& lds_ok) {
        e3d_allow_lds(lds_ok, kern, lds);
        hipLaunchKernelGGL(kern, grid, block, lds, s, g, M, count);
    };
    static std::atomic<uint64_t> ok1{0}, ok1t{0}, ok2{0}, ok2t{0}, ok3{0}, ok3t{0};
    if (terms == E3D_TERMS_BF16) {
        const size_t lds = (size_t)2 * 1 * (256 + 128) * ROW_B;
        if (tr) go(gemm_wgrad_ragged_kernel<1, true>, lds, ok1t);
        else go(gemm_wgrad_ragged_kernel<1, false>, lds, ok1);
    } else if (terms == 3) {
        const size_t lds = (size_t)2 * 2 * (256 + 128) * ROW_B;
        if (tr) go(gemm_wgrad_ragged_kernel<2, true>, lds, ok2t);
        else go(gemm_wgrad_ragged_kernel<2, false>, lds, ok2);
    } else {
        const size_t lds = (size_t)1 * 3 * (256 + 128) * ROW_B;
        if (tr) go(gemm_wgrad_ragged_kernel<3, true>, lds, ok3t);
        else go(gemm_wgrad_ragged_kernel<3, false>, lds, ok3);
    }
    return e3d_launch_status("e3d_gemm_wgrad_ragged_f32_split");
}

extern "C" int e3d_gemm_bias_act_f32_split(const float* A, int64_t lda, const float* W,
                                           const float* bias, float* out, int64_t ldc, int M,
                                           int N, int K, int act, int terms, void* stream) {
    E3D_REQUIRE(N % BN == 0, "gemm_split: need N%%128==0 (N=%d)", N);
    return gemm_split_general(A, lda, 0, W, (int64_t)K, 0, bias, out, ldc, M, N, K, act, terms, nullptr, 1.0f, stream);
}

extern "C" int e3d_gemm_bias_act_f32_split_ex(const float* A, int64_t lda, const float* W, const float* bias, float* out,
                                              int64_t ldc, int M, int N, int K, int act, int terms, float* out_absmax,
                                              float out_scale, void* stream) {
    E3D_REQUIRE(N % BN == 0, "gemm_split: need N%%128==0 (N=%d)", N);
    return gemm_split_general(A, lda, 0, W, (int64_t)K, 0, bias, out, ldc, M, N, K, act, terms, out_absmax, out_scale, stream);
}

extern "C" int e3d_gemm_bias_act_f32_split_gated(const float* A, int64_t lda, const float* W, const float* bias, float* out,
                                                 int64_t ldc, int M, int N, int K, int act, int terms, float* out_absmax,
                                                 float out_scale, int plan_m, const int* run_if, void* stream) {
    E3D_REQUIRE(N % BN == 0, "gemm_split: need N%%128==0 (N=%d)", N);
    return gemm_split_general(A, lda, 0, W, (int64_t)K, 0, bias, out, ldc, M, N, K, act, terms, out_absmax, out_scale, stream,
                              plan_m, run_if);
}

extern "C" int e3d_gemm_planes_supported(int M, int N, int K, int64_t lda, int act, int terms) {
    return (terms == 3 || terms == E3D_TERMS_F16X3) && (act == E3D_ACT_NONE || act == E3D_ACT_GELU) && M > 0 && N > 0 && K > 0 &&
           K % BK == 0 && lda >= K && lda % 4 == 0 && persistent_ok(M, M, N, K, lda, K, BK);
}

extern "C" int e3d_gemm_bias_act_planes_split(const float* A, int64_t lda, const float* W, const float* bias, void* out_planes,
                                              int M, int N, int K, int act, int terms, float* out_absmax, float out_scale,
                                              void* stream) {
    E3D_REQUIRE(A && W && out_planes, "gemm_split (planes): null pointer");
    E3D_REQUIRE(e3d_gemm_planes_supported(M, N, K, lda, act, terms),
                "gemm_split (planes): this launch does not take the persistent kernel (M=%d N=%d K=%d act=%d terms=%d)", M, N, K, act, terms);
    E3D_REQUIRE(((uintptr_t)A % 16) == 0 && ((uintptr_t)W % 16) == 0 && ((uintptr_t)bias % 16) == 0 && ((uintptr_t)out_planes % 16) == 0,
                "gemm_split (planes): A, W, bias and the planes must be 16-byte aligned");
    E3D_REQUIRE(!out_absmax || act == E3D_ACT_NONE, "gemm_split (planes): out_absmax exists for act = none");
    const Epi epi{out_absmax, out_scale, 0, nullptr};
    hipStream_t s = (hipStream_t)stream;
    float* out = reinterpret_cast<float*>(out_planes);
    if (terms == 3) {
        if (act == E3D_ACT_GELU) return launch256p<E3D_ACT_GELU, __bf16, true>(A, lda, W, bias, out, N, M, N, K, epi, s);
        return launch256p<E3D_ACT_NONE, __bf16, true>(A, lda, W, bias, out, N, M, N, K, epi, s);
    }
    if (act == E3D_ACT_GELU) return launch256p<E3D_ACT_GELU, _Float16, true>(A, lda, W, bias, out, N, M, N, K, epi, s);
    return launch256p<E3D_ACT_NONE, _Float16, true>(A, lda, W, bias, out, N, M, N, K, epi, s);
}
```

### e3-invaraint-diffusion-model_amd/hip.py

```python
import ctypes
import os
from ctypes import c_char_p, c_float, c_int, c_int64, c_uint32, c_uint64, c_void_p

_HERE = os.path.dirname(os.path.abspath(__file__))
LIB_PATH = os.environ.get("E3D_HIP_LIB", os.path.join(_HERE, "libe3d_hip.so"))
ABI_VERSION = 5

_P = c_void_p
_VIEW = [_P, c_int64, c_int64]
_QKV = 3 * _VIEW + [_P, c_int, _P]
_SHAPE = 4 * [c_int]
_ATTN_FWD = _QKV + [_P, _P] + _SHAPE
_ATTN_BWD = _QKV + 3 * [_P] + 3 * _VIEW + [_P, _P] + _SHAPE
_STREAM = [_P]
_DROP = [c_float, c_uint64]
_DROP_KEYED = [c_float, c_uint32, _P]
_BOUNDS = [_P, c_int, _P, _P, _P]
_SIGNATURES = {
    "e3d_abi_version": (c_int, []),
    "e3d_last_error": (c_char_p, []),
    "e3d_gemm_bias_act_f32": (c_int, [_P, c_int64, _P, _P, _P, c_int64, c_int, c_int, c_int, c_int, _P]),
    "e3d_gemm_bias_act_f32_split": (c_int, [_P, c_int64, _P, _P, _P, c_int64, c_int, c_int, c_int, c_int, c_int, _P]),
    "e3d_gemm_bias_act_f32_split_ex": (c_int, [_P, c_int64, _P, _P, _P, c_int64, c_int, c_int, c_int, c_int, c_int, _P, c_float, _P]),
    "e3d_gemm_bias_act_f32_split_gated": (c_int, [_P, c_int64, _P, _P, _P, c_int64, c_int, c_int, c_int, c_int, c_int, _P, c_float,
                                                  c_int, _P, _P]),
    "e3d_absmax_f32": (c_int, [_P, c_int64, _P, _P]),
    "e3d_relkey_attn_fwd": (c_int, _ATTN_FWD + _STREAM),
    "e3d_relkey_attn_fwd_split": (c_int, _ATTN_FWD + [c_int] + _STREAM),
    "e3d_gemm_skinny_workspace_bytes": (c_int64, [c_int, c_int, c_int]),
    "e3d_gemm_skinny_f32_split": (c_int, [_P, c_int64, _P, _P, _P, c_int64, c_int, c_int, c_int, c_int, c_int, _P, c_int64, _P]),
    "e3d_gemm_skinny_f32_split_ex": (c_int, [_P, c_int64, _P, _P, _P, c_int64, c_int, c_int, c_int, c_int, c_int, _P, c_int64, _P, c_float, _P]),
    "e3d_gemm_skinny_plan_select": (None, [c_int, c_int]),
    "e3d_gemm_skinny_residual_layernorm_f32_split": (c_int, [_P, c_int64, _P, _P, _P, _P, _P, c_float, _P, c_int, c_int, c_int,
                                                     c_int, _P, c_int64, _P]),
    "e3d_gemm_skinny_residual_layernorm_f32_split_ex": (c_int, [_P, c_int64, _P, _P, _P, _P, _P, c_float, _P, c_int, c_int, c_int,
                                                        c_int, _P, c_int64, c_float, _P]),
    "e3d_attn_skip_padded_tiles": (c_int, [c_int]),
    "e3d_gemm_kernel_select": (c_int, [c_int]),
    "e3d_gemm_general_select": (c_int, [c_int]),
    "e3d_attn_rescale_tau": (c_float, [c_float]),
    "e3d_residual_layernorm_fwd": (c_int, [_P, _P, _P, _P, c_float, _P, _P, c_int, c_int, _P]),
    "e3d_adaln_gate_fwd": (c_int, [_P, _P, _P, c_int, c_int, _P, c_int, c_int, _P]),
    "e3d_embed_layernorm_fwd": (c_int, [_P, c_int, _P, _P, _P, _P, c_float, _P, c_int, _P, _P, c_int, c_int, _P]),
    "e3d_adaln_gate_indexed_fwd": (c_int, [_P, _P, _P, _P, c_int, _P, c_int, _P, c_int, c_int, _P]),
    "e3d_classify_onehot_rows": (c_int, [_P, c_int, _P, _P, c_int, _P]),
    "e3d_embed_layernorm_fwd_ex": (c_int, [_P, c_int, _P, _P, _P, _P, c_float, _P, c_int, _P, _P, c_int, c_int, _P, _P]),
    "e3d_nerf_backbone": (c_int, [_P, _P, _P, c_int, c_int, c_int, _P]),
    "e3d_gemm_f32_split_general": (c_int, [_P, c_int64, c_int, _P, c_int64, c_int, _P, _P, c_int64, c_int, c_int,
                                           c_int, c_int, c_int, _P]),
    "e3d_transpose_grouped_f32": (c_int, [_P, _P, c_int, c_int, c_int, c_int64, c_int64, _P]),
    "e3d_gemm_wgrad_grouped_f32_split": (c_int, [_P, _P, _P, _P, c_uint64, c_int, c_int64, c_int64, c_int, c_int, c_int, c_int, _P]),
    "e3d_residual_layernorm_drop_fwd": (c_int, [_P, _P, _P, _P, c_float, _P, _P, c_int, c_int, c_float, c_uint64, _P]),
    "e3d_layernorm_bwd_drop": (c_int, [_P, _P, _P, c_float, _P, _P, _P, _P, c_int, c_int, c_float, c_uint64, _P]),
    "e3d_weight_planes_bytes": (c_int64, [c_int, c_int]),
    "e3d_weight_planes_f32_split": (c_int, [_P, c_int, c_int, c_int, _P, _P]),
    "e3d_gemm_residual_layernorm_supported": (c_int, [c_int, c_int, c_int, c_int64]),
    "e3d_gemm_residual_layernorm_f32_split": (c_int, [_P, c_int64, _P, _P, _P, c_int64, _P, _P, c_float, _P, c_int64,
                                                      c_int, c_int, c_int, c_int, c_float, _P]),
    "e3d_activation_planes_bytes": (c_int64, [c_int, c_int]),
    "e3d_activation_planes_f32_split": (c_int, [_P, c_int64, c_int, c_int, c_int, _P, _P]),
    "e3d_gemm_residual_layernorm_planes_split": (c_int, [_P, _P, _P, _P, c_int64, _P, _P, c_float, _P, c_int64,
                                                         c_int, c_int, c_int, c_int, c_float, _P]),
    "e3d_gemm_planes_supported": (c_int, [c_int, c_int, c_int, c_int64, c_int, c_int]),
    "e3d_gemm_bias_act_planes_split": (c_int, [_P, c_int64, _P, _P, _P, c_int, c_int, c_int, c_int, c_int, _P, c_float, _P]),
    "e3d_attn_planes_supported": (c_int, [c_int64, c_int64, c_int64, c_int, c_int, c_int, c_int]),
    "e3d_relkey_attn_fwd_split_planes": (c_int, _QKV + [_P] + _SHAPE + [c_int] + _BOUNDS + _STREAM),
    "e3d_gemm_wgrad_ragged_f32_split": (c_int, [_P, _P, _P, _P, _P, _P, _P, _P, c_uint64, c_int, c_int, c_int, _P]),
    "e3d_relkey_attn_bwd_workspace_floats": (c_int64, [c_int, c_int, c_int, c_int, c_int]),
    "e3d_relkey_attn_bwd": (c_int, _ATTN_BWD + _STREAM),
    "e3d_dropout_f32": (c_int, [_P, c_float, c_uint64, _P, c_int64, _P]),
    "e3d_relkey_attn_fwd_split_drop": (c_int, _ATTN_FWD + [c_int] + _DROP + _STREAM),
    "e3d_relkey_attn_fwd_split_ex": (c_int, _ATTN_FWD + [c_int] + _DROP + _BOUNDS + _STREAM),
    "e3d_attn_scratch_bytes": (c_int64, [c_int]),
    "e3d_ddpm_step_wrap_table": (c_int, [_P, _P, _P, _P, _P, c_int, _P, c_int64, _P]),
    "e3d_relkey_attn_bwd_drop": (c_int, _ATTN_BWD + _DROP + _STREAM),
    "e3d_relkey_attn_bwd_ex": (c_int, _ATTN_BWD + [c_int] + _DROP + _STREAM),
    "e3d_attn_dropout_mask": (c_int, [c_int, c_int, c_int, c_int, c_float, c_uint64, _P, _P]),
    "e3d_layernorm_bwd": (c_int, [_P, _P, _P, c_float, _P, _P, _P, c_int, c_int, _P]),
    "e3d_layernorm_bwd_workspace_floats": (c_int64, [c_int, c_int]),
    "e3d_layernorm_bwd_ws": (c_int, [_P, _P, _P, c_float, _P, _P, _P, _P, c_int, c_int, c_float, c_uint64, _P, c_int64, _P]),
    "e3d_adaln_gate_bwd": (c_int, [_P, _P, _P, c_int, c_int, _P, _P, c_int, c_int, _P]),
    "e3d_act_fwd": (c_int, [_P, c_int, _P, c_int64, _P]),
    "e3d_act_bwd": (c_int, [_P, _P, c_int, _P, c_int64, _P]),
    "e3d_colsum": (c_int, [_P, c_int64, _P, c_int, c_int, _P]),
    "e3d_group_sum": (c_int, [_P, c_int, _P, c_int, c_int, _P]),
    "e3d_small_k_wgrad": (c_int, [_P, _P, _P, _P, c_int, c_int, c_int, c_int, _P]),
    "e3d_head_linear_bwd_dx": (c_int, [_P, _P, _P, c_int, c_int, c_int, _P]),
    "e3d_head_linear_fwd": (c_int, [_P, _P, _P, _P, c_int, c_int, c_int, _P]),
    "e3d_ddpm_step_wrap": (c_int, [_P, _P, _P, c_float, c_float, c_float, c_float, c_int, _P, c_int64, _P]),
    "e3d_q_sample_wrap": (c_int, [_P, _P, _P, _P, _P, _P, c_int, c_int64, _P]),
    "e3d_discrete_posterior_sample": (c_int, [_P, _P, _P, _P, _P, c_int, _P, _P, c_int, c_int, c_int, _P]),
    "e3d_discrete_q_sample": (c_int, [_P, _P, _P, c_int, _P, c_int, c_int, c_int, _P]),
    "e3d_optim_chunk_elems": (c_int, []),
    "e3d_grad_global_norm": (c_int, [_P, _P, _P, _P, c_int, c_float, _P, _P, _P]),
    "e3d_adamw_step_dyn": (c_int, [_P, _P, _P, _P, _P, _P, _P, c_int, _P, _P, c_float, c_float, c_float, c_float, _P]),
    "e3d_adamw_step_dev": (c_int, [_P, _P, _P, _P, _P, _P, _P, c_int, _P, _P, _P]),
    "e3d_dropout_set_epoch_ptr": (c_int, [_P]),
    "e3d_adamw_step": (c_int, [_P, _P, _P, _P, _P, _P, _P, c_int, _P, c_float, c_float, c_float, c_float, c_float, c_int, _P]),
    "e3d_adamw_ema_step": (c_int, [_P, _P, _P, _P, _P, _P, _P, _P, c_int, _P, c_float, c_float, c_float, c_float, c_float, c_int,
                                   c_float, _P]),
    "e3d_adamw_ema_step_dev": (c_int, [_P, _P, _P, _P, _P, _P, _P, _P, c_int, _P, _P, _P]),
    "e3d_attn_varlen_fwd": (c_int, [_P, c_int64, _P, c_int64, _P, c_int64, _P, _P, _P, _P, _P, c_int, _P, c_int, _P,
                                    c_int64, c_int, c_int, c_int, c_int, _P]),
    "e3d_keyed_ddpm_step_wrap": (c_int, [_P, _P, _P, _P, _P, c_uint64, c_int, _P, c_int64, c_int, _P]),
    "e3d_keyed_discrete_posterior_sample": (c_int, [_P, _P, _P, _P, _P, c_uint64, _P, _P, c_int, c_int, c_int, _P]),
    "e3d_keyed_draws": (c_int, [_P, c_uint64, c_int, c_int, c_int, c_int, c_int, c_float, _P, c_int64, _P]),
    "e3d_strided_step_wrap": (c_int, [_P, _P, _P, _P, _P, c_int, c_int, c_int, _P, c_int64, _P]),
    "e3d_keyed_strided_step_wrap": (c_int, [_P, _P, _P, _P, c_int, _P, c_uint64, c_int, c_int, _P, c_int64, c_int, _P]),
    "e3d_known_compose_wrap": (c_int, [_P, _P, _P, _P, _P, _P, c_int, c_float, c_int64, _P]),
    "e3d_keyed_known_compose_wrap": (c_int, [_P, _P, _P, _P, _P, c_int, c_float, _P, c_uint64, c_int64, c_int, _P]),
    "e3d_discrete_known_compose": (c_int, [_P, _P, _P, _P, _P, c_int, c_int, c_int, c_int, _P]),
    "e3d_keyed_discrete_known_compose": (c_int, [_P, _P, _P, _P, _P, c_uint64, _P, c_int, c_int, c_int, _P]),
    "e3d_discrete_posterior_sample_ctl": (c_int, [_P, _P, _P, c_float, _P, _P, _P, c_int, _P, _P, c_int, c_int, c_int, _P]),
    "e3d_keyed_discrete_posterior_sample_ctl": (c_int, [_P, _P, _P, c_float, _P, _P, _P, c_uint64, _P, _P, c_int, c_int, c_int,
                                                        _P]),
    "e3d_discrete_final_pick": (c_int, [_P, _P, c_float, _P, _P, _P, c_int64, c_int, _P]),
    "e3d_keyed_discrete_forward_levels": (c_int, [_P, _P, _P, _P, c_int, c_uint64, _P, c_int, c_int, c_int, _P]),
    "e3d_discrete_score_rows": (c_int, [_P, _P, _P, _P, _P, _P, _P, _P, _P, _P, c_int, c_int, c_int, _P]),
    "e3d_masked_item_sums": (c_int, [_P, _P, _P, _P, c_int, c_int, _P]),
    "e3d_keyed_timesteps": (c_int, [_P, _P, c_uint64, c_int, c_int, _P, c_int, _P]),
    "e3d_keyed_q_sample_wrap": (c_int, [_P, _P, _P, _P, c_int, c_float, _P, _P, c_uint64, _P, _P, c_int, c_int, c_int, _P]),
    "e3d_keyed_discrete_q_sample": (c_int, [_P, _P, _P, _P, c_uint64, _P, c_int, c_int, c_int, _P]),
    "e3d_keyed_drop_row_keys": (c_int, [_P, c_int, c_int, _P, c_uint64, c_int, _P, _P]),
    "e3d_dropout_f32_keyed": (c_int, [_P, c_float, c_uint32, _P, _P, c_int, c_int, _P]),
    "e3d_keyed_attn_dropout_mask": (c_int, [c_int, c_int, c_int, c_int, c_float, c_uint32, _P, _P, _P]),
    "e3d_residual_layernorm_drop_fwd_keyed": (c_int, [_P, _P, _P, _P, c_float, _P, _P, c_int, c_int, c_float, c_uint32, _P, _P]),
    "e3d_layernorm_bwd_drop_keyed": (c_int, [_P, _P, _P, c_float, _P, _P, _P, _P, c_int, c_int, c_float, c_uint32, _P, _P]),
    "e3d_layernorm_bwd_ws_keyed": (c_int, [_P, _P, _P, c_float, _P, _P, _P, _P, c_int, c_int, c_float, c_uint32, _P, _P, c_int64,
                                           _P]),
    "e3d_relkey_attn_fwd_split_drop_keyed": (c_int, _ATTN_FWD + [c_int] + _DROP_KEYED + _STREAM),
    "e3d_relkey_attn_fwd_split_ex_keyed": (c_int, _ATTN_FWD + [c_int] + _DROP_KEYED + _BOUNDS + _STREAM),
    "e3d_relkey_attn_bwd_drop_keyed": (c_int, _ATTN_BWD + _DROP_KEYED + _STREAM),
    "e3d_relkey_attn_bwd_ex_keyed": (c_int, _ATTN_BWD + [c_int] + _DROP_KEYED + _STREAM),
    "e3d_backbone_angles": (c_int, [_P, _P, _P, _P, c_int, c_float, _P]),
    "e3d_contact_residues": (c_int, [_P, _P, _P, _P, _P, _P, c_int, c_int, c_int, c_int, c_float, _P]),
    "e3d_superpose_pairs": (c_int, [_P, _P, _P, _P, _P, _P, _P, _P, c_int, c_int, c_int, _P]),
}
EXPORTS = tuple(_SIGNATURES)

_lib = None


class HipExtensionMissing(RuntimeError):
    pass


def lib():
    global _lib
    if _lib is None:
# ... 21 lines not shown
```

### e3-invaraint-diffusion-model_amd/ops.py

```python
import contextlib
import math
import os
import warnings

import torch

from . import hip, keyed

ACT_NONE, ACT_GELU, ACT_SILU = 0, 1, 2


def _stream():
    return torch.cuda.current_stream().cuda_stream


TRACE = None


_ROCTX = None


def _roctx():
    global _ROCTX
    if _ROCTX is None:
# ... 538 lines not shown
        return ent[1], ent[2]
    if torch.cuda.is_current_stream_capturing():
        raise RuntimeError("weight_planes: cache miss inside a stream capture (warm the op up before capturing)")
    src, scale = f16_weight(weight) if terms == 19 else (weight.detach(), 1.0)
    N, K = src.shape
    nbytes = hip.lib().e3d_weight_planes_bytes(N, K)
    if nbytes < 0:
        raise ValueError(f"weight_planes: unsupported shape {tuple(src.shape)}")
    planes = torch.empty((nbytes,), dtype=torch.uint8, device=src.device)
    hip.check(hip.lib().e3d_weight_planes_f32_split(_p(src), N, K, terms, _p(planes), _stream()), "e3d_weight_planes_f32_split")
    try:
        weight._e3d_planes_w = (key, planes, scale)
    except AttributeError:
        pass
    return planes, scale


def rowln_ok(terms, M, H, K, a, residual=None):
    return (terms in (3, 19) and M >= ROWLN_MIN_M and (a is None or (a.stride(1) == 1 and a.data_ptr() % 16 == 0))
            and (residual is None or (residual.stride(1) == 1 and residual.stride(0) % 4 == 0 and residual.data_ptr() % 16 == 0))
            and bool(hip.lib().e3d_gemm_residual_layernorm_supported(M, H, K, K if a is None else a.stride(0))))


ACT_PLANES = {"1": True, "0": False, "gemm": "gemm", "attn": "attn"}.get(os.environ.get("E3D_ACT_PLANES", "1"))
if ACT_PLANES is None:
    raise ValueError(f"E3D_ACT_PLANES must be 1, 0, gemm or attn, got {os.environ['E3D_ACT_PLANES']!r}")
ACT_PLANES_CALLS = 0


class ActPlanes:
    __slots__ = ("data", "shape", "terms")
    requires_grad = False

    def __init__(self, data, M, K, terms):
        self.data, self.shape, self.terms = data, (M, K), terms

    @property
    def device(self):
        return self.data.device

    def decode(self):
        M, K = self.shape
        dt = torch.float16 if self.terms == 19 else torch.bfloat16
        t = self.data.view(dt).view(M // 32, K // 16, 2, 2, 32, 8)
        t = t.permute(2, 0, 4, 1, 3, 5).reshape(2, M, K)
        return t[0], t[1]


def activation_planes(x, mode=None):
    _chk(x, "activation_planes.x")
    M, K = x.shape
    terms = GEMM_MODES[GEMM_MODE if mode is None else mode]
    nbytes = hip.lib().e3d_activation_planes_bytes(M, K)
    if nbytes < 0 or terms not in (3, 19) or x.stride(1) != 1:
        raise ValueError(f"activation_planes: unsupported shape {tuple(x.shape)} / terms {terms}")
    out = torch.empty((nbytes,), dtype=torch.uint8, device=x.device)
    hip.check(hip.lib().e3d_activation_planes_f32_split(_p(x), x.stride(0), M, K, terms, _p(out), _stream()),
              "e3d_activation_planes_f32_split")
    return ActPlanes(out, M, K, terms)


def gemm_planes_ok(a, weight, bias, act, out_features, residual=None, mode=None):
    if ACT_PLANES not in (True, "gemm") or torch.is_grad_enabled():
        return False
    terms = GEMM_MODES[GEMM_MODE if mode is None else mode]
    M, K = a.shape
    N = weight.shape[0]
    return (terms in (3, 19) and rowln_ok(terms, M, out_features, N, None, residual) and a.stride(1) == 1
            and a.data_ptr() % 16 == 0 and (bias is None or bias.data_ptr() % 16 == 0)
            and not (_skinny_ok(terms, M, N, K, a) and M <= min(SKINNY_MAX_M, SKINNY_GEMM_MAX_M))
            and bool(hip.lib().e3d_gemm_planes_supported(M, N, K, a.stride(0), act, terms)))


def attention_planes_ok(q, k, v, nh, Lq, Lk, out_features, residual=None, mode=None):
    if ACT_PLANES not in (True, "attn") or torch.is_grad_enabled():
        return False
    terms = GEMM_MODES[ATTN_MODE if mode is None else mode]
    if terms != GEMM_MODES[GEMM_MODE] or terms not in (3, 19):
        return False
    return (rowln_ok(terms, q.shape[0], out_features, nh * 64, None, residual) and v.stride(1) == 1 and k.stride(1) == 1
            and bool(hip.lib().e3d_attn_planes_supported(k.stride(0), Lk * v.stride(0), v.stride(0), Lq, Lk, terms, 1)))


def linear_residual_layernorm(a, weight, bias, residual, gamma, beta, eps, mode=None):
    M, K = a.shape
    H = weight.shape[0]
    terms = GEMM_MODES[GEMM_MODE if mode is None else mode]
    if isinstance(a, ActPlanes):
        global ACT_PLANES_CALLS
        if a.terms != terms or not rowln_ok(terms, M, H, K, None, residual):
            raise RuntimeError(f"linear_residual_layernorm: no kernel reads activation planes at M={M} H={H} K={K} terms={terms}")
        _chk(a.data, "linear_residual_layernorm.a", torch.uint8)
        for t, n in ((weight, "weight"), (bias, "bias"), (residual, "residual"), (gamma, "gamma"), (beta, "beta")):
            _chk(t, "linear_residual_layernorm." + n)
        assert weight.is_contiguous() and weight.shape[1] == K and (residual is None or residual.shape == (M, H))
        planes, scale = weight_planes(weight, terms)
        out = torch.empty((M, H), device=a.device, dtype=torch.float32)
        with _timed("gemm_layernorm", (M, H, K)):
            hip.check(hip.lib().e3d_gemm_residual_layernorm_planes_split(
                _p(a.data), _p(planes), _p(bias), _p(residual), residual.stride(0) if residual is not None else 0,
                _p(gamma), _p(beta), eps, _p(out), out.stride(0), M, H, K, terms, scale, _stream()),
                "e3d_gemm_residual_layernorm_planes_split")
        ACT_PLANES_CALLS += 1
        return out
    if rowln_ok(terms, M, H, K, a, residual):
        for t, n in ((a, "a"), (weight, "weight"), (bias, "bias"), (residual, "residual"), (gamma, "gamma"), (beta, "beta")):
            _chk(t, "linear_residual_layernorm." + n)
        assert weight.is_contiguous() and weight.shape[1] == K and (residual is None or residual.shape == (M, H))
        planes, scale = weight_planes(weight, terms)
        out = torch.empty((M, H), device=a.device, dtype=torch.float32)
        with _timed("gemm_layernorm", (M, H, K)):
            hip.check(hip.lib().e3d_gemm_residual_layernorm_f32_split(
                _p(a), a.stride(0), _p(planes), _p(bias), _p(residual), residual.stride(0) if residual is not None else 0,
                _p(gamma), _p(beta), eps, _p(out), out.stride(0), M, H, K, terms, scale, _stream()),
                "e3d_gemm_residual_layernorm_f32_split")
        return out
    if not (_skinny_ok(terms, M, H, K, a) and H in (256, 512, 768, 1024) and a.stride(1) == 1):
        return residual_layernorm(gemm(a, weight, bias, mode=mode), residual, gamma, beta, eps)
    for t, n in ((a, "a"), (weight, "weight"), (bias, "bias"), (residual, "residual"), (gamma, "gamma"), (beta, "beta")):
        _chk(t, "linear_residual_layernorm." + n)
    assert weight.is_contiguous() and weight.shape[1] == K and (residual is None or (residual.is_contiguous() and residual.shape == (M, H)))
    out = torch.empty((M, H), device=a.device, dtype=torch.float32)
    ws = _skinny_workspace(a.device, M, H, K)
    scale = 1.0
    if terms == 19:
        weight, scale = f16_weight(weight)
    with _timed("gemm_layernorm", (M, H, K)):
        hip.check(hip.lib().e3d_gemm_skinny_residual_layernorm_f32_split_ex(
            _p(a), a.stride(0), _p(weight), _p(bias), _p(residual), _p(gamma), _p(beta), eps, _p(out), M, H, K, terms,
            _p(ws), ws.numel(), scale, _stream()), "e3d_gemm_skinny_residual_layernorm_f32_split_ex")
    return out

def adaln_gate(x, y, mod, branch, rows_per_cond):
    for n, t in (("x", x), ("y", y), ("mod", mod)):
        _chk(t, "adaln_gate." + n)
    assert x.is_contiguous() and y.is_contiguous() and mod.is_contiguous()
    M, H = x.shape
    assert mod.shape[1] == 6 * H and mod.shape[0] * rows_per_cond == M, (mod.shape, M, rows_per_cond)
    out = torch.empty_like(x)
    with _timed("adaln_gate", (M, H)):
        hip.check(hip.lib().e3d_adaln_gate_fwd(_p(x), _p(y), _p(mod), branch, rows_per_cond, _p(out),
                                               M, H, _stream()), "e3d_adaln_gate_fwd")
    return out


def adaln_gate_indexed(x, y, idx, table, mod, branch):
    for n, t in (("x", x), ("y", y), ("table", table), ("mod", mod)):
        _chk(t, "adaln_gate_indexed." + n)
    _chk(idx, "adaln_gate_indexed.idx", torch.int32)
    assert x.is_contiguous() and y.is_contiguous() and mod.is_contiguous() and table.is_contiguous() and idx.is_contiguous()
    M, H = x.shape
    assert y.shape == x.shape and mod.shape == (M, 6 * H) and table.shape[1] == 6 * H and idx.shape == (M,), (mod.shape, table.shape, idx.shape)
    out = torch.empty_like(x)
    with _timed("adaln_gate", (M, H)):
        hip.check(hip.lib().e3d_adaln_gate_indexed_fwd(_p(x), _p(y), _p(idx), _p(table), table.shape[0], _p(mod), branch,
                                                       _p(out), M, H, _stream()), "e3d_adaln_gate_indexed_fwd")
    return out


def classify_onehot_rows(x, flag=None):
    _chk(x, "classify_onehot_rows.x")
    assert x.dim() == 2 and x.is_contiguous()
    M, F = x.shape
    if flag is None:
        flag = torch.zeros(1, device=x.device, dtype=torch.int32)
    _chk(flag, "classify_onehot_rows.flag", torch.int32)
# ... 436 lines not shown
```

### e3-invaraint-diffusion-model_amd/structure_model/model.py

```python
import functools
from typing import List

import torch
from torch import nn

from .. import bert, keyed, ops
from ..blocks import (BertEmbeddings, GaussianFourierProjection, KeyedDropoutSwitch, Predictor, SELayer, drop_row_keys,
                      flat2d, onehot_modulation, require_gpu)
from ..training import adamw
import os

from .utils import elementwise_form, radian_l1_loss, radian_smooth_l1_loss

MASKED_LOSS = os.environ.get("E3D_MASKED_LOSS", "1") == "1"


class ReceptorCache:

    def __init__(self, encoder_states, cross_kv, mask, B, L, layout=None):
        self.encoder_states, self.cross_kv, self.mask, self.B, self.L = encoder_states, cross_kv, mask, B, L
        self.layout = layout


class ConditionalBertForDiffusionBase(nn.Module):
    def __init__(self, encoder_config, decoder_config, feature_size: int) -> None:
        super().__init__()
        self.encoder_config = encoder_config
        self.decoder_config = decoder_config
        self.receptor_seq_emb = BertEmbeddings(20, encoder_config)
        self.receptor_angle_emb = BertEmbeddings(feature_size, encoder_config)
        self.receptor_emb = SELayer(encoder_config)
        self.encoder = bert.BertEncoder(encoder_config)
        self.ligand_angle_emb = BertEmbeddings(feature_size, decoder_config)
        self.timestep_projector = GaussianFourierProjection(decoder_config.hidden_size)
        self.timestep_emb = SELayer(decoder_config)
        self.decoder = bert.BertEncoder(decoder_config)
        self.angles_predictor = Predictor(decoder_config.hidden_size, feature_size)

    def encode_receptor(self, receptor_seq, receptor_angles, receptor_attention_masks,
                        project_cross_kv=True, layout=None) -> ReceptorCache:
        require_gpu(receptor_seq, receptor_angles, receptor_attention_masks)
        B, L = receptor_angles.shape[:2]
        ops.reset_absmax(receptor_angles.device)
        if layout is not None:
            ang = self.receptor_angle_emb.run(flat2d(layout.pack(receptor_angles)))
            seq2d = flat2d(layout.pack(receptor_seq))
            mod = onehot_modulation(self.receptor_emb, self.receptor_seq_emb, seq2d)
            seq = self.receptor_seq_emb.run(seq2d) if mod is None else None
            x = self.receptor_emb.run(ang, seq, None, 1, layout.rows, mod=mod, layout=layout)
            x = bert.run_encoder(self.encoder, x, None, 1, layout.rows, layout=layout)
            kv = [bert.project_cross_kv(layer.crossattention, x) for layer in self.decoder.layer] if project_cross_kv else None
            return ReceptorCache(x, kv, None, B, L, layout=layout)
        mask = receptor_attention_masks.contiguous().float()
        rk = drop_row_keys(keyed.DROP_POCKET, L)
        ang = self.receptor_angle_emb.run(flat2d(receptor_angles), row_keys=rk)
        seq2d = flat2d(receptor_seq)
        mod = onehot_modulation(self.receptor_emb, self.receptor_seq_emb, seq2d)
        seq = self.receptor_seq_emb.run(seq2d, row_keys=rk) if mod is None else None
        x = self.receptor_emb.run(ang, seq, mask, B, L, mod=mod, row_keys=rk)
        x = bert.run_encoder(self.encoder, x, mask, B, L, row_keys=rk)
        kv = None
        if project_cross_kv:
            kv = [bert.project_cross_kv(layer.crossattention, x) for layer in self.decoder.layer]
        return ReceptorCache(x, kv, mask, B, L)

    def timestep_modulation(self, timesteps):
        temb = self.timestep_projector(timesteps.reshape(-1)).contiguous()
        return self.timestep_emb.modulation(temb)

    def decode(self, timestep, noised_ligand_angles, ligand_attention_masks, receptor: ReceptorCache, mod=None,
               layout=None):
        if layout is not None:
            return self._decode_packed(timestep, noised_ligand_angles, receptor, mod, layout)
        require_gpu(timestep, noised_ligand_angles, ligand_attention_masks)
        B, L = noised_ligand_angles.shape[:2]
        mask = ligand_attention_masks.contiguous().float()
        lk = drop_row_keys(keyed.DROP_LIGAND, L)
        x = self.ligand_angle_emb.run(flat2d(noised_ligand_angles), row_keys=lk)
        if mod is None:
            mod = self.timestep_modulation(timestep.squeeze(dim=-1))
        x = self.timestep_emb.run(x, None, mask, B, L, mod=mod, row_keys=lk)
        x = bert.run_encoder(self.decoder, x, mask, B, L, enc=receptor.encoder_states,
                             enc_mask=receptor.mask, Lk=receptor.L, cross_kv=receptor.cross_kv, row_keys=lk)
        return self.angles_predictor.run(x).view(B, L, -1)

    def _decode_packed(self, timestep, x_packed, receptor, mod, layout):
        require_gpu(x_packed)
        if receptor.layout is None:
            raise ValueError("a packed decode needs the pocket packed as well: encode_receptor(..., layout=)")
        assert x_packed.dim() == 2 and x_packed.shape[0] == layout.rows, (tuple(x_packed.shape), layout.rows)
        if mod is None:
            t = timestep.reshape(-1)
            assert bool((t == t[0]).all()), "a packed batch shares one timestep"
            mod = self.timestep_modulation(t[:1])
        assert mod.shape[0] == 1, "a packed batch shares one timestep: mod must be one row [1,6H]"
        x = self.ligand_angle_emb.run(x_packed.contiguous().float())
        x = self.timestep_emb.run(x, None, None, 1, layout.rows, mod=mod, layout=layout)
        x = bert.run_encoder(self.decoder, x, None, 1, layout.rows, enc=receptor.encoder_states,
                             cross_kv=receptor.cross_kv, layout=layout, enc_layout=receptor.layout)
        return self.angles_predictor.run(x)

    def forward(self, timestep, noised_ligand_angles, ligand_attention_masks,
                receptor_seq, receptor_angles, receptor_attention_masks,
                ligand_pos_ids=None, receptor_pos_ids=None):
        rec = self.encode_receptor(receptor_seq, receptor_angles, receptor_attention_masks,
                                   project_cross_kv=False)
        return self.decode(timestep, noised_ligand_angles, ligand_attention_masks, rec)


class ConditionalBertForDiffusion(KeyedDropoutSwitch, ConditionalBertForDiffusionBase):
    diheral_loss_func = radian_l1_loss
    angle_loss_func = functools.partial(radian_smooth_l1_loss, beta=torch.pi / 10)

    def __init__(self, encoder_config, decoder_config, feature_names: List[str], loss_func: List,
                 epochs: int = 1, lr_scheduler=None, l2_lambda: float = 0.0,
                 steps_per_epoch: int = 250, learning_rate: float = 5e-5, **kwargs):
        super().__init__(encoder_config, decoder_config, len(feature_names))
        self.steps_per_epoch = steps_per_epoch
        self.learning_rate = learning_rate
        self.feature_names = feature_names
        self.lr_scheduler = lr_scheduler
        self.loss_func = loss_func
        self.epochs = epochs
        self.l2_lambda = l2_lambda
        self.train_epoch_losses, self.valid_epoch_losses = [], []
        self.train_epoch_counter = 0

    def _get_loss_terms(self, batch) -> torch.Tensor:
        known_noise = batch["known_noise"]
        predicted_noise = self.forward(
            timestep=batch["timestep"], noised_ligand_angles=batch["noised_ligand_angle"],
            ligand_attention_masks=batch["ligand_attn_mask"], receptor_seq=batch["receptor_seq"],
            receptor_angles=batch["receptor_angles"], receptor_attention_masks=batch["receptor_attn_mask"])
        assert known_noise.shape == predicted_noise.shape, f"{known_noise.shape} != {predicted_noise.shape}"
        return self.loss_terms_from_prediction(predicted_noise, known_noise, batch["ligand_attn_mask"])

    def loss_terms_from_prediction(self, predicted_noise, known_noise, ligand_attn_mask):
        n_feat = known_noise.shape[-1]
        fns = [self.loss_func[i] if isinstance(self.loss_func, list) else self.loss_func for i in range(n_feat)]
        elems = [elementwise_form(fn) for fn in fns]
        if all(e is not None for e in elems) and MASKED_LOSS:
            sel = (ligand_attn_mask != 0).unsqueeze(-1)
            count = sel.sum().to(predicted_noise.dtype)
            groups = {}
            for i, fn in enumerate(fns):
                key = (fn.func, tuple(sorted(fn.keywords.items()))) if isinstance(fn, functools.partial) else (fn, ())
# ... 52 lines not shown
```

### e3-invaraint-diffusion-model_amd/structure_model/sample.py

```python
if __package__ in (None, ""):
    import os as _os, sys as _sys
    _sys.path.insert(0, _os.path.dirname(_os.path.dirname(_os.path.dirname(_os.path.abspath(__file__)))))
    import __graft_entry__ as _g
    _g.load_package()
    __package__ = "e3diff_amd.structure_model"

import os
import pickle
import warnings
from dataclasses import dataclass

import torch
from torch import nn

from .. import keyed, ops, packing
from ..bert import BertConfig
from ..packing import trimmed_length
from .dataset import LigandBindingSiteDataset, NoisedAnglesDataset
from .model import ConditionalBertForDiffusion
from .utils import CosineTables, KnownLevels, StridedTables

MODEL_PATH = ""
OUTPUT = "./data/output.pkl"
DATA_FILE = "./data/biolip.pt"
# ... 114 lines not shown
        return t_index != 0

    def compose_draws(self, t_index):
        return self.known_x0 is not None and self.keyed is None and float(self.known_levels.levels[t_index, 1]) != 0.0

    def update(self, x, eps_hat, t_dev, noise, out, wrap, t_index=None):
        eps_hat = eps_hat.contiguous()
        if t_index is not None:
            noise = _eager_noise(x, noise, self.update_draws(t_index))
        if self.strided is not None:
            if self.keyed is not None:
                return ops.keyed_strided_step_wrap(x, eps_hat, self.coef, t_dev, *self.keyed, wrap=wrap,
                                                   wrap_x0=self.wrap_x0, out=out)
            return ops.strided_step_wrap(x, eps_hat, noise, self.coef, t_dev, wrap=wrap, wrap_x0=self.wrap_x0, out=out)
        if self.keyed is not None:
            return ops.keyed_ddpm_step_wrap(x, eps_hat, self.coef, t_dev, *self.keyed, wrap=wrap, out=out)
        if t_index is None:
            return ops.ddpm_step_wrap_table(x, eps_hat, noise, self.coef, t_dev, wrap=wrap, out=out)
        sra, beta, s1m, sigma = (float(c[t_index]) for c in (self.tab.sqrt_recip_alphas, self.tab.betas,
                                                             self.tab.sqrt_one_minus_alphas_cumprod, self.tab.sigma))
        return ops.ddpm_step_wrap(x, eps_hat, noise, sra, beta, s1m, 0.0 if noise is None else sigma, wrap=wrap, out=out)

    def compose(self, x, t_dev, noise, t_index=None):
        if self.known_x0 is None:
            return x
        if self.keyed is not None:
            return ops.keyed_known_compose_wrap(x, self.known_x0, self.known_mask, self.levels, t_dev, *self.keyed,
                                                self.known_scale)
        if t_index is not None:
            noise = _eager_noise(x, noise, self.compose_draws(t_index))
        return ops.known_compose_wrap(x, self.known_x0, self.known_mask, noise, self.levels, t_dev, self.known_scale)


def _eager_noise(x, noise, draws):
    if not draws:
        return None
    return torch.randn_like(x) if noise is None else noise.contiguous()


def step_plan(betas, dev=None, table=False, strided=None, wrap_x0=False, row_keys=None, seed=None, known=None,
              known_mask=None, known_levels=None, known_scale=1.0):
    tab = _tables(betas)
    if strided is None and wrap_x0:
        raise ValueError("step_plan: wrap_x0 belongs to the strided update; pass strided=StridedTables(...)")
    if strided is not None and not isinstance(strided, StridedTables):
        raise TypeError(f"step_plan: strided must be a StridedTables, got {type(strided).__name__}")
    if (row_keys is None) != (seed is None):
        raise ValueError("step_plan: keyed draws need both row_keys and a seed")
    if known is not None and not isinstance(known_levels, KnownLevels):
        raise ValueError("step_plan: held positions need known_levels=KnownLevels(tables, order of the chain)")
    if seed is not None:
        keyed.check_steps(tab.betas.shape[0])
    coef = None
    if strided is not None:
        coef = strided.coef.contiguous().to(dev)
    elif table or seed is not None:
        coef = torch.stack([tab.sqrt_recip_alphas, tab.betas, tab.sqrt_one_minus_alphas_cumprod, tab.sigma],
                           dim=1).float().contiguous().to(dev)
    held = {} if known is None else dict(known_x0=known.contiguous(), known_mask=known_mask.contiguous(),
                                         known_levels=known_levels, levels=known_levels.levels.to(dev),
                                         known_scale=float(known_scale))
    return StepPlan(tab, coef, strided, bool(wrap_x0), None if seed is None else (row_keys, keyed.check_seed(seed)), **held)


def keyed_x_T(seed, item_ids, L, n_ft=8, scale=1.0, device=None):
    device = DEVICE if device is None else device
    ids = keyed.item_ids(item_ids, len(item_ids))
    keys = keyed.padded_keys(ids, L, device)
    return ops.keyed_initial_angles(keys, seed, n_ft, scale).reshape(len(ids), L, n_ft)


def _reverse_step(model, ligand_mask, x_t, receptor_seq, receptor_mask, receptor_angle, timestep,
                  betas, noise, receptor_cache, out, wrap, mod=None, layout=None, plan=None, known_noise=None):
    plan = step_plan(betas) if plan is None else plan
    if isinstance(timestep, int):
        t_index = timestep
        timestep = t_dev = torch.full((x_t.shape[0],), t_index, device=x_t.device, dtype=torch.long)
    else:
        t_unique = torch.unique(timestep)
        assert len(t_unique) == 1, f"Got multiple values for t: {t_unique}"
        t_index = int(t_unique.item())
        t_dev = timestep.to(device=x_t.device, dtype=torch.long).contiguous()
    if receptor_cache is None:
        receptor_cache = model.encode_receptor(receptor_seq, receptor_angle, receptor_mask)
    eps_hat = model.decode(timestep, x_t, ligand_mask, receptor_cache, mod=mod, layout=layout)
    x = plan.update(x_t.contiguous().float(), eps_hat, t_dev, noise, out, wrap, t_index)
    return plan.compose(x, t_dev, known_noise, t_index)


class GraphedReverseStep:

    def __init__(self, model, ligand_mask, cache, tab, x_like, wrap=True, draw=True, mod_table=None, layout=None,
                 row_keys=None, seed=None, strided=None, wrap_x0=False, known=None):
        dev = x_like.device
        plan = tab if isinstance(tab, StepPlan) else step_plan(tab, dev, True, strided, wrap_x0, row_keys, seed,
                                                               *(known or (None, None, None, 1.0)))
        if plan.keyed is not None and not draw:
            raise ValueError("a keyed graph draws its own noise")
        if plan.coef is None:
            raise ValueError("a captured step reads its coefficients from the plan's table: step_plan(..., table=True)")
        self.model, self.mask, self.cache, self.plan, self.wrap = model, ligand_mask, cache, plan, wrap
        self.mod_table, self.layout, self.draw = mod_table, layout, draw
        self.x, self.out = x_like.clone(), torch.empty_like(x_like)
        self.noise = torch.zeros_like(x_like) if any(map(plan.update_draws, plan.order)) else None
        self.known_noise = torch.zeros_like(x_like) if any(map(plan.compose_draws, plan.order)) else None
        self.t = torch.full((x_like.shape[0],), plan.order[-1], device=dev, dtype=torch.long)
        self.graph, _ = packing.warm_up_and_capture(self._body, dev)

    def _body(self):
        mod = None if self.mod_table is None else self.mod_table.index_select(0, self.t[:1])
        eps_hat = self.model.decode(self.t, self.x, self.mask, self.cache, mod=mod, layout=self.layout)
        if self.draw and self.noise is not None:
            self.noise.normal_()
        self.plan.update(self.x, eps_hat, self.t, self.noise, self.out, self.wrap)
        if self.draw and self.known_noise is not None:
            self.known_noise.normal_()
        self.plan.compose(self.out, self.t, self.known_noise)

    def step(self, i, x, noise=None, known_noise=None):
        if (noise is not None) == self.draw:
            raise ValueError("this graph was captured %s injected noise" % ("without" if self.draw else "with"))
        if known_noise is not None:
            if self.known_noise is None or self.draw:
                raise ValueError("this graph takes no injected draw for held positions")
            self.known_noise.copy_(known_noise)
        elif self.known_noise is not None and not self.draw:
            raise ValueError("this graph was captured with injected noise: pass the held positions' draw too")
        self.t.fill_(i)
        if x is not self.x:
            self.x.copy_(x)
        if noise is not None and self.noise is not None:
            self.noise.copy_(noise)
        self.graph.replay()
        return self.out


@torch.no_grad()
def p_sample_loop(model: nn.Module, ligand_mask, ligand_angle_noise, receptor_seq, receptor_mask,
                  receptor_angle, total_timesteps: int, betas, disable_pbar: bool = False,
                  noises=None, return_device: bool = False, step: int = None, use_graph: bool = None,
                  trim_padding: bool = False, pack: bool = False, seed: int = None, item_ids=None,
                  update: str = "ancestral", eta: float = 0.0, wrap_x0: bool = False, known=None, known_mask=None,
                  known_noises=None, known_scale: float = 1.0) -> torch.Tensor:
    if update not in ("ancestral", "strided"):
        raise ValueError(f"p_sample_loop: update must be 'ancestral' or 'strided', got {update!r}")
    if update == "ancestral" and (eta != 0.0 or wrap_x0):
        raise ValueError("p_sample_loop: eta and wrap_x0 belong to update='strided'")
    step = STEP if step is None else step
    tab = _tables(betas)
    order = list(reversed(range(0, total_timesteps, step)))
    strided = StridedTables(tab, order, eta) if update == "strided" else None
    x = ligand_angle_noise.contiguous().float()
    x0, m8, known_noises = _known_chain(known, known_mask, known_noises, seed, ligand_mask, x, len(order), "p_sample_loop")
    if x0 is not None and (noises is None) != (known_noises is None) and seed is None:
        raise ValueError("p_sample_loop: inject noises and known_noises together, or neither")
    if seed is not None and noises is not None:
        raise ValueError("p_sample_loop: pass either injected noises or a seed, not both")
    if seed is None and item_ids is not None:
        raise ValueError("p_sample_loop: item_ids key the seeded draws; pass a seed with them")
    ids = None if seed is None else keyed.item_ids(item_ids, x.shape[0])
    frame = packing.Frame(ligand_mask, receptor_mask, trim=trim_padding, pack=pack)
    layout, pocket_layout = frame.layouts or (None, None)
    if pocket_layout is None:
        cache = model.encode_receptor(frame.pocket(receptor_seq), frame.pocket(receptor_angle),
                                      frame.pocket(receptor_mask))
    else:
        cache = model.encode_receptor(receptor_seq, receptor_angle, receptor_mask, layout=pocket_layout)
    x = frame.ligand(x)
    mask = None if layout is not None else frame.ligand(ligand_mask).contiguous().float()
    if noises is not None:
        noises = frame.ligand(noises.to(x.device).float(), dim=1)
    if x0 is not None:
        x0, m8 = frame.ligand(x0), frame.ligand(m8)
        known_noises = None if known_noises is None else frame.ligand(known_noises, dim=1)
    plan = step_plan(tab, x.device, table=True, strided=strided, wrap_x0=wrap_x0,
                     row_keys=None if seed is None else frame.row_keys(ids, x.device), seed=seed, known=x0, known_mask=m8,
                     known_levels=None if x0 is None else KnownLevels(tab, order), known_scale=known_scale)
    traj = torch.empty((len(order),) + tuple(x.shape), device=x.device, dtype=torch.float32)
    mod_rows = model.timestep_modulation(torch.tensor(order, device=x.device, dtype=torch.long))
    mod_table = torch.zeros((total_timesteps, mod_rows.shape[1]), device=x.device, dtype=torch.float32)
    mod_table[order] = mod_rows
    graphed = packing.capture_graph(
        lambda: GraphedReverseStep(model, mask, cache, plan, x, draw=noises is None, mod_table=mod_table, layout=layout),
        frame.rows, len(order), use_graph)
    for n, i in enumerate(order):
        kn = None if known_noises is None else known_noises[n].contiguous()
        if graphed is not None:
            x = graphed.step(i, graphed.out if n else x, None if noises is None else noises[n], kn)
            traj[n].copy_(x)
        else:
            x = _reverse_step(model, mask, x, None, None, None, i, tab, None if noises is None else noises[n], cache,
                              traj[n], wrap=True, mod=mod_table[i:i + 1], layout=layout, plan=plan, known_noise=kn)
    traj = frame.restore(traj, dim=1)
    return traj if return_device else traj.cpu()


def get_dataset(file_path):
    ds = LigandBindingSiteDataset(file_path, "test", CONFIG["max_seq_len"], CONFIG["pocket_ext"])
    return NoisedAnglesDataset(ds, timesteps=CONFIG["timesteps"])


def build_configs(cfg=None):
    cfg = cfg or CONFIG
    common = dict(max_position_embeddings=cfg["max_seq_len"], num_attention_heads=cfg["num_heads"],
                  hidden_size=cfg["hidden_size"], intermediate_size=cfg["intermediate_size"],
                  num_hidden_layers=cfg["num_hidden_layers"],
                  position_embedding_type=cfg["position_embedding_type"],
                  hidden_dropout_prob=cfg["dropout_p"], attention_probs_dropout_prob=cfg["dropout_p"],
                  use_cache=False)
    return BertConfig(**common), BertConfig(**common, is_decoder=True, add_cross_attention=True)


def load_model(dataset, model_path=None):
    encoder_config, decoder_config = build_configs()
    model = ConditionalBertForDiffusion(
        encoder_config=encoder_config, decoder_config=decoder_config,
        feature_names=dataset.feature_names, epochs=CONFIG["max_epochs"],
        lr_scheduler=CONFIG["lr_scheduler"], l2_lambda=CONFIG["l2_norm"],
        steps_per_epoch=len(dataset), learning_rate=CONFIG["lr"],
        loss_func=[ConditionalBertForDiffusion.diheral_loss_func] * 4
        + [ConditionalBertForDiffusion.angle_loss_func] * 4)
    path = MODEL_PATH if model_path is None else model_path
    if path:
        model.load_state_dict(torch.load(path, map_location="cpu", weights_only=True))
    return model.eval().to(DEVICE)


def sample(model, test_angle_ds, all_batches: bool = False, seed: int = None, keep=None):
    seed = SEED if seed is None else seed
    keep = KEEP if keep is None else keep
    bs = CONFIG["batch_size"]
    items = [test_angle_ds[i] for i in range(len(test_angle_ds))]

    def chunk(name):
        return [torch.stack([it[name] for it in items[i:i + bs]]) for i in range(0, len(items), bs)]

    ligand_mask, receptor_angle = chunk("ligand_attn_mask"), chunk("receptor_angles")
    receptor_seq, receptor_mask = chunk("receptor_seq"), chunk("receptor_attn_mask")
    pad, feature_size = items[0]["ligand_angles"].shape
    retval = []
    for idx, lm in enumerate(ligand_mask):
        print(f"Generating Batch {idx}/{len(ligand_mask)}")
        lengths = lm.sum(dim=1).int()
        ids = list(range(idx * bs, idx * bs + len(lengths)))
        held = {}
        if callable(keep) or keep:
            held = dict(known=torch.stack([items[i]["ligand_angles"] for i in ids]).float().to(DEVICE),
                        known_mask=torch.stack([packing.keep_mask(keep, i, pad, int(l)) for i, l in zip(ids, lengths)]).to(DEVICE),
                        known_scale=test_angle_ds.angular_var_scale)
        if seed is None:
            x_T = test_angle_ds.sample_noise(torch.zeros((len(lengths), pad, feature_size)))
# ... 31 lines not shown
```

### include/e3d_hip.h

```cpp
#ifndef E3D_HIP_H
#define E3D_HIP_H

#include <stdint.h>

#ifdef __cplusplus
extern "C" {
#endif

#define E3D_ABI_VERSION 5

#define E3D_TERMS_BF16 1
#define E3D_TERMS_BF16X3 3
#define E3D_TERMS_BF16X6 6
#define E3D_TERMS_F16X3 19

#define E3D_ACT_NONE 0
#define E3D_ACT_GELU 1
#define E3D_ACT_SILU 2

int e3d_abi_version(void);
const char* e3d_last_error(void);

int e3d_gemm_bias_act_f32(const float* A, int64_t lda, const float* W, const float* bias,
                          float* out, int64_t ldc, int M, int N, int K, int act, void* stream);
// ... 195 lines not shown
                                   uint64_t drop_seed, void* stream);

int64_t e3d_attn_scratch_bytes(int Lk);
int e3d_relkey_attn_fwd_split_ex(const float* q, int64_t q_bs, int64_t q_rs, const float* k, int64_t k_bs,
                                 int64_t k_rs, const float* v, int64_t v_bs, int64_t v_rs,
                                 const float* dist_emb, int P, const float* key_mask, float* out,
                                 float* lse, int B, int nh, int Lq, int Lk, int terms, float drop_p,
                                 uint64_t drop_seed, void* e_scratch, int e_scratch_ready, const float* q_absmax,
                                 const float* k_absmax, float* e_absmax, void* stream);

int e3d_attn_varlen_fwd(const float* q, int64_t q_rs, const float* k, int64_t k_rs, const float* v, int64_t v_rs,
                        const int* q_start, const int* q_len, const int* k_start, const int* k_len, const int* tiles,
                        int n_tiles, const float* dist_emb, int P, float* out, int64_t out_rows, int nh, int max_q_len,
                        int max_k_len, int terms, void* stream);

int e3d_relkey_attn_bwd_drop(const float* q, int64_t q_bs, int64_t q_rs, const float* k, int64_t k_bs,
                             int64_t k_rs, const float* v, int64_t v_bs, int64_t v_rs,
                             const float* dist_emb, int P, const float* key_mask, const float* out,
                             const float* lse, const float* dout, float* dq, int64_t dq_bs,
                             int64_t dq_rs, float* dk, int64_t dk_bs, int64_t dk_rs, float* dv,
                             int64_t dv_bs, int64_t dv_rs, float* d_dist_emb, float* workspace, int B,
                             int nh, int Lq, int Lk, float drop_p, uint64_t drop_seed, void* stream);

int e3d_relkey_attn_bwd_ex(const float* q, int64_t q_bs, int64_t q_rs, const float* k, int64_t k_bs,
                           int64_t k_rs, const float* v, int64_t v_bs, int64_t v_rs,
                           const float* dist_emb, int P, const float* key_mask, const float* out,
                           const float* lse, const float* dout, float* dq, int64_t dq_bs, int64_t dq_rs,
                           float* dk, int64_t dk_bs, int64_t dk_rs, float* dv, int64_t dv_bs,
                           int64_t dv_rs, float* d_dist_emb, float* workspace, int B, int nh, int Lq,
                           int Lk, int terms, float drop_p, uint64_t drop_seed, void* stream);

int e3d_attn_dropout_mask(int B, int nh, int Lq, int Lk, float p, uint64_t seed, float* out, void* stream);

int e3d_layernorm_bwd(const float* dy, const float* s, const float* gamma, float eps, float* ds,
                      float* dgamma, float* dbeta, int M, int H, void* stream);

int e3d_adaln_gate_bwd(const float* dout, const float* y, const float* mod, int branch,
                       int rows_per_cond, float* dy, float* dmod, int M, int H, void* stream);

int e3d_act_fwd(const float* z, int act, float* out, int64_t n, void* stream);
int e3d_act_bwd(const float* dh, const float* z, int act, float* dz, int64_t n, void* stream);

int e3d_colsum(const float* x, int64_t ld, float* out, int M, int N, void* stream);
int e3d_transpose_grouped_f32(const float* const* src, float* const* dst, int count, int rows, int cols, int64_t ld_src,
                              int64_t ld_dst, void* stream);
int e3d_group_sum(const float* x, int rows_per_group, float* out, int M, int H, void* stream);

int e3d_small_k_wgrad(const float* g, const float* x, float* dW, float* db, int M, int H, int F,
                      int transpose_out, void* stream);

int e3d_head_linear_bwd_dx(const float* dout, const float* W, float* dx, int M, int H, int Nout,
                           void* stream);

int e3d_residual_layernorm_drop_fwd(const float* x, const float* residual, const float* gamma, const float* beta, float eps,
                                    float* s_out, float* out, int M, int H, float drop_p, uint64_t drop_seed, void* stream);
int e3d_layernorm_bwd_drop(const float* dy, const float* s, const float* gamma, float eps, float* ds, float* ds_dropped,
                           float* dgamma, float* dbeta, int M, int H, float drop_p, uint64_t drop_seed, void* stream);
int64_t e3d_layernorm_bwd_workspace_floats(int M, int H);
int e3d_layernorm_bwd_ws(const float* dy, const float* s, const float* gamma, float eps, float* ds, float* ds_dropped,
                         float* dgamma, float* dbeta, int M, int H, float drop_p, uint64_t drop_seed, float* workspace,
                         int64_t workspace_floats, void* stream);

int64_t e3d_weight_planes_bytes(int N, int K);
int e3d_weight_planes_f32_split(const float* W, int N, int K, int terms, void* planes, void* stream);
int e3d_gemm_residual_layernorm_supported(int M, int N, int K, int64_t lda);
int e3d_gemm_residual_layernorm_f32_split(const float* A, int64_t lda, const void* w_planes, const float* bias,
                                          const float* residual, int64_t ldr, const float* gamma, const float* beta, float eps,
                                          float* out, int64_t ldo, int M, int N, int K, int terms, float out_scale, void* stream);

int64_t e3d_activation_planes_bytes(int M, int K);
int e3d_activation_planes_f32_split(const float* X, int64_t ldx, int M, int K, int terms, void* planes, void* stream);
int e3d_gemm_residual_layernorm_planes_split(const void* a_planes, const void* w_planes, const float* bias,
                                             const float* residual, int64_t ldr, const float* gamma, const float* beta, float eps,
                                             float* out, int64_t ldo, int M, int N, int K, int terms, float out_scale, void* stream);
int e3d_gemm_planes_supported(int M, int N, int K, int64_t lda, int act, int terms);
int e3d_gemm_bias_act_planes_split(const float* A, int64_t lda, const float* W, const float* bias, void* out_planes,
                                   int M, int N, int K, int act, int terms, float* out_absmax, float out_scale, void* stream);
int e3d_attn_planes_supported(int64_t k_rs, int64_t v_bs, int64_t v_rs, int Lq, int Lk, int terms, int have_scratch);
int e3d_relkey_attn_fwd_split_planes(const float* q, int64_t q_bs, int64_t q_rs, const float* k, int64_t k_bs,
                                     int64_t k_rs, const float* v, int64_t v_bs, int64_t v_rs,
                                     const float* dist_emb, int P, const float* key_mask, void* out_planes,
                                     int B, int nh, int Lq, int Lk, int terms, void* e_scratch, int e_scratch_ready,
                                     const float* q_absmax, const float* k_absmax, float* e_absmax, void* stream);

int e3d_adamw_step_dyn(float* const* params, const float* const* grads, float* const* exp_avg, float* const* exp_avg_sq,
                       const int64_t* numel, const int* chunk_tensor, const int64_t* chunk_first, int n_chunks,
                       const float* norm_and_clip, const float* lr_and_step, float beta1, float beta2, float eps,
                       float weight_decay, void* stream);
int e3d_adamw_step_dev(float* const* params, const float* const* grads, float* const* exp_avg, float* const* exp_avg_sq,
                       const int64_t* numel, const int* chunk_tensor, const int64_t* chunk_first, int n_chunks,
                       const float* norm_and_clip, const float* hyper, void* stream);
int e3d_dropout_set_epoch_ptr(const uint64_t* device_word);
int e3d_optim_chunk_elems(void);
int e3d_grad_global_norm(const float* const* grads, const int64_t* numel, const int* chunk_tensor, const int64_t* chunk_first,
                         int n_chunks, float max_norm, float* partial, float* norm_and_clip, void* stream);
int e3d_adamw_step(float* const* params, const float* const* grads, float* const* exp_avg, float* const* exp_avg_sq,
                   const int64_t* numel, const int* chunk_tensor, const int64_t* chunk_first, int n_chunks,
                   const float* norm_and_clip, float lr, float beta1, float beta2, float eps, float weight_decay, int step,
                   void* stream);

int e3d_adamw_ema_step(float* const* params, const float* const* grads, float* const* exp_avg, float* const* exp_avg_sq,
                       float* const* ema, const int64_t* numel, const int* chunk_tensor, const int64_t* chunk_first,
                       int n_chunks, const float* norm_and_clip, float lr, float beta1, float beta2, float eps,
                       float weight_decay, int step, float ema_decay, void* stream);
int e3d_adamw_ema_step_dev(float* const* params, const float* const* grads, float* const* exp_avg, float* const* exp_avg_sq,
                           float* const* ema, const int64_t* numel, const int* chunk_tensor, const int64_t* chunk_first,
                           int n_chunks, const float* norm_and_clip, const float* hyper, void* stream);

int e3d_keyed_drop_row_keys(const int64_t* ids, int B, int L, const int64_t* epoch_word, uint64_t seed, int stream,
                            uint64_t* out, void* st);
int e3d_dropout_f32_keyed(const float* x, float p, uint32_t site, const uint64_t* row_keys, float* out, int M, int H,
                          void* stream);
int e3d_keyed_attn_dropout_mask(int B, int nh, int Lq, int Lk, float p, uint32_t site, const uint64_t* row_keys, float* out,
                                void* stream);
int e3d_residual_layernorm_drop_fwd_keyed(const float* x, const float* residual, const float* gamma, const float* beta, float eps,
                                          float* s_out, float* out, int M, int H, float drop_p, uint32_t site,
                                          const uint64_t* row_keys, void* stream);
int e3d_layernorm_bwd_drop_keyed(const float* dy, const float* s, const float* gamma, float eps, float* ds, float* ds_dropped,
                                 float* dgamma, float* dbeta, int M, int H, float drop_p, uint32_t site, const uint64_t* row_keys,
                                 void* stream);
int e3d_layernorm_bwd_ws_keyed(const float* dy, const float* s, const float* gamma, float eps, float* ds, float* ds_dropped,
                               float* dgamma, float* dbeta, int M, int H, float drop_p, uint32_t site, const uint64_t* row_keys,
                               float* workspace, int64_t workspace_floats, void* stream);
int e3d_relkey_attn_fwd_split_drop_keyed(const float* q, int64_t q_bs, int64_t q_rs, const float* k, int64_t k_bs,
                                         int64_t k_rs, const float* v, int64_t v_bs, int64_t v_rs, const float* dist_emb,
                                         int P, const float* key_mask, float* out, float* lse, int B, int nh, int Lq, int Lk,
                                         int terms, float drop_p, uint32_t site, const uint64_t* row_keys, void* stream);
int e3d_relkey_attn_fwd_split_ex_keyed(const float* q, int64_t q_bs, int64_t q_rs, const float* k, int64_t k_bs,
                                       int64_t k_rs, const float* v, int64_t v_bs, int64_t v_rs, const float* dist_emb,
                                       int P, const float* key_mask, float* out, float* lse, int B, int nh, int Lq, int Lk,
                                       int terms, float drop_p, uint32_t site, const uint64_t* row_keys, void* e_scratch,
                                       int e_scratch_ready, const float* q_absmax, const float* k_absmax, float* e_absmax,
                                       void* stream);
int e3d_relkey_attn_bwd_drop_keyed(const float* q, int64_t q_bs, int64_t q_rs, const float* k, int64_t k_bs, int64_t k_rs,
                                   const float* v, int64_t v_bs, int64_t v_rs, const float* dist_emb, int P,
                                   const float* key_mask, const float* out, const float* lse, const float* dout, float* dq,
                                   int64_t dq_bs, int64_t dq_rs, float* dk, int64_t dk_bs, int64_t dk_rs, float* dv,
                                   int64_t dv_bs, int64_t dv_rs, float* d_dist_emb, float* workspace, int B, int nh, int Lq,
                                   int Lk, float drop_p, uint32_t site, const uint64_t* row_keys, void* stream);
int e3d_relkey_attn_bwd_ex_keyed(const float* q, int64_t q_bs, int64_t q_rs, const float* k, int64_t k_bs, int64_t k_rs,
                                 const float* v, int64_t v_bs, int64_t v_rs, const float* dist_emb, int P,
                                 const float* key_mask, const float* out, const float* lse, const float* dout, float* dq,
                                 int64_t dq_bs, int64_t dq_rs, float* dk, int64_t dk_bs, int64_t dk_rs, float* dv,
                                 int64_t dv_bs, int64_t dv_rs, float* d_dist_emb, float* workspace, int B, int nh, int Lq,
                                 int Lk, int terms, float drop_p, uint32_t site, const uint64_t* row_keys, void* stream);

int e3d_backbone_angles(const float* coords, const int32_t* seg, float* angles, int32_t* status, int R,
                        float max_peptide_bond, void* stream);
int e3d_contact_residues(const float* rec_xyz, const int32_t* rec_row, const int32_t* rec_off, const float* lig_xyz,
                         const int32_t* lig_off, int32_t* hit, int n_complexes, int n_rec_atoms, int n_lig_atoms, int n_rows,
                         float cutoff, void* stream);

int e3d_superpose_pairs(const double* xyz, const int32_t* off, const int32_t* mob, const int32_t* ref, double* msd,
                        double* rot, double* trans, int32_t* status, int n_structs, int n_atoms, int n_pairs, void* stream);

#ifdef __cplusplus
}
#endif
#endif
```

Measured before the change: 4279 pocket-steps/s.

## Emit QKV/KV projections as pre-split attention operand planes consumed directly by attention

QKV and cross-attention K/V GEMMs now write their outputs directly in the pre-scaled, hi/lo split, tile-swizzled plane layout that the attention kernel wants. A new INP variant of the coop attention kernel streams K/V tiles straight into LDS with global_load_lds, replacing the register staging path, and reads Q fragments directly. This removes the f32 round-trip and the per-tile split and convert work inside attention. The cost is a new plane layout contract between kernels, hand-written asm waitcnt and barrier handling, and extra plumbing of ligand length into the encoder.

```diff
diff --git a/e3-invaraint-diffusion-model_amd/autograd.py b/e3-invaraint-diffusion-model_amd/autograd.py
--- a/e3-invaraint-diffusion-model_amd/autograd.py
+++ b/e3-invaraint-diffusion-model_amd/autograd.py
@@ -512,9 +512,11 @@
 
 class functional:
     @staticmethod
-    def linear(x, weight, bias=None, act=ops.ACT_NONE, absmax=None, planes_for=None):
+    def linear(x, weight, bias=None, act=ops.ACT_NONE, absmax=None, planes_for=None, attn_planes=None):
         if _needs_grad(x, weight, bias):
             out = _Linear.apply(x, weight, bias, act, absmax)
+        elif attn_planes is not None and act == ops.ACT_NONE and ops.qkv_planes_ok(x, weight, bias, attn_planes[3], attn_planes[4]):
+            out = ops.gemm_attn_planes(x, weight, bias, *attn_planes[:3], absmax=absmax)
         elif planes_for is not None and absmax is None and ops.gemm_planes_ok(x, weight, bias, act, planes_for[0].shape[0],
                                                                               planes_for[1]):
             return ops.gemm(x, weight, bias, act, planes_out=True)
@@ -532,6 +534,12 @@
         bounds = (q_abs, k_abs) if q_abs is not None and k_abs is not None else None
         if _needs_grad(q_src, kv_src, dist_emb):
             return _Attention.apply(q_src, kv_src, dist_emb, key_mask, B, nh, Lq, Lk, max_pos, drop_p, bounds, row_keys)
+        if isinstance(q_src, ops.AttnPlanes) or isinstance(kv_src, ops.AttnPlanes):
+            if drop_p > 0 or not isinstance(q_src, ops.AttnPlanes) or not (kv_src is None or isinstance(kv_src, ops.AttnPlanes)):
+                raise RuntimeError("attention: operand planes need every operand as planes and no dropout")
+            planes = planes_for is not None and ops.attention_planes_ok_in(B * Lq, nh, planes_for[0].shape[0], planes_for[1])
+            return ops.attention_in_planes(q_src, kv_src, B, nh, Lq, Lk, key_mask=key_mask, dist_emb=dist_emb, max_pos=max_pos,
+                                           bounds=bounds, planes_out=planes)
         q, k, v = _Attention._views(q_src, kv_src, nh * 64)
         drop = ops.site_drop(drop_p, row_keys) if drop_p > 0 else None
         planes = (planes_for is not None and drop is None and
diff --git a/e3-invaraint-diffusion-model_amd/bert.py b/e3-invaraint-diffusion-model_amd/bert.py
--- a/e3-invaraint-diffusion-model_amd/bert.py
+++ b/e3-invaraint-diffusion-model_amd/bert.py
@@ -198,7 +198,9 @@
 def run_self_attention(att, x, mask, B, L, drop=(0.0, 0.0), layout=None):
     sa = att.self
     w, b = qkv_weights(sa)
-    qkv = F.linear(x, w, b, absmax=ops.absmax_slot(sa, "qkv", x.device))
+    H = att.num_heads * 64
+    as_planes = (H, 2 * H, 3 * H, L, L) if layout is None and drop[0] == 0 and drop[1] == 0 else None
+    qkv = F.linear(x, w, b, absmax=ops.absmax_slot(sa, "qkv", x.device), attn_planes=as_planes)
     relkey = sa.position_embedding_type == "relative_key"
     if layout is not None:
         H = att.num_heads * 64
@@ -213,13 +215,24 @@
     return _attention_output(att, ctx, x, drop[0], drop_keys(drop))
 
 
-def project_cross_kv(att, enc):
+def project_cross_kv(att, enc, Lq=None, Lk=None):
     w, b = kv_weights(att.self)
-    return F.linear(enc, w, b, absmax=torch.zeros(1, device=enc.device, dtype=torch.float32))
+    H = att.num_heads * 64
+    as_planes = (0, H, 2 * H, Lq, Lk) if Lq is not None and Lk is not None and not att.training else None
+    return F.linear(enc, w, b, absmax=torch.zeros(1, device=enc.device, dtype=torch.float32), attn_planes=as_planes)
 
 
 def run_cross_attention(att, x, kv, enc_mask, B, Lq, Lk, drop=(0.0, 0.0), layout=None, enc_layout=None):
-    q = F.linear(x, att.self.query.weight, att.self.query.bias, absmax=ops.absmax_slot(att.self, "q", x.device))
+    kv_planes = isinstance(kv, ops.AttnPlanes)
+    if kv_planes and (layout is not None or drop[0] != 0 or drop[1] != 0 or kv.shape[0] != B * Lk):
+        raise RuntimeError("run_cross_attention: K/V planes were projected for a padded inference frame of other lengths")
+    H = att.num_heads * 64
+    q = F.linear(x, att.self.query.weight, att.self.query.bias, absmax=ops.absmax_slot(att.self, "q", x.device),
+                 attn_planes=(H, 0, 0, Lq, Lk) if kv_planes else None)
+    if kv_planes and not isinstance(q, ops.AttnPlanes):
+        q_abs = q._e3d_absmax
+        q = ops.attn_operand_planes(q, H, 0, 0)
+        q._e3d_absmax = q_abs
     if layout is not None:
         H = att.num_heads * 64
         ctx = ops.attention_varlen(q, kv[:, :H], kv[:, H:], layout, enc_layout, att.num_heads)
@@ -254,6 +267,7 @@
     for i, layer in enumerate(encoder.layer):
         kv = None
         if hasattr(layer, "crossattention"):
-            kv = cross_kv[i] if cross_kv is not None else project_cross_kv(layer.crossattention, enc)
+            kv = cross_kv[i] if cross_kv is not None else project_cross_kv(
+                layer.crossattention, enc, *((L, Lk) if layout is None and drop[:2] == (0.0, 0.0) else ()))
         x = run_layer(layer, x, mask, B, L, kv, enc_mask, Lk, drop, layout=layout, enc_layout=enc_layout)
     return x
diff --git a/e3-invaraint-diffusion-model_amd/csrc/attn_relkey_coop.hip b/e3-invaraint-diffusion-model_amd/csrc/attn_relkey_coop.hip
--- a/e3-invaraint-diffusion-model_amd/csrc/attn_relkey_coop.hip
+++ b/e3-invaraint-diffusion-model_amd/csrc/attn_relkey_coop.hip
@@ -31,10 +31,35 @@
 constexpr int V_ROW_B = 192;
 constexpr int K_PLANE_B = 32 * K_ROW_B, V_PLANE_B = 32 * V_ROW_B;
 constexpr float LOG2E = 1.4426950408889634f, LN2 = 0.6931471805599453f;
-constexpr float Q_SCALE = 0.125f * LOG2E;
+constexpr float Q_SCALE = E3D_ATTN_Q_SCALE;
 constexpr float MASK_BIAS = -10000.0f * LOG2E;
 float g_rescale_tau = 8.0f;
 constexpr int KV_BUF_B = 2 * K_PLANE_B + 2 * V_PLANE_B + 128;
+constexpr int IN_BUF_B = 16384;
+#define E3D_VMCNT(n) asm volatile("s_waitcnt vmcnt(" #n ")" ::: "memory")
+#define E3D_LDS_BARRIER()                                   \
+    do {                                                    \
+        asm volatile("s_waitcnt lgkmcnt(0)" ::: "memory");  \
+        __builtin_amdgcn_s_barrier();                       \
+        asm volatile("" ::: "memory");                      \
+        __builtin_amdgcn_sched_barrier(0);                  \
+    } while (0)
+__device__ __forceinline__ void glds16x4(const void* g, unsigned char* lds_wave_base) {
+    const unsigned base = __builtin_amdgcn_readfirstlane((unsigned)(uintptr_t)(__attribute__((address_space(3))) unsigned char*)lds_wave_base);
+    unsigned m0_was;
+    asm volatile(
+        "s_mov_b32 %0, m0\n\t"
+        "s_mov_b32 m0, %2\n\t"
+        "s_nop 0\n\t"
+        "global_load_lds_dwordx4 %1, off\n\t"
+        "global_load_lds_dwordx4 %1, off offset:1024\n\t"
+        "global_load_lds_dwordx4 %1, off offset:2048\n\t"
+        "global_load_lds_dwordx4 %1, off offset:3072\n\t"
+        "s_mov_b32 m0, %0"
+        : "=&s"(m0_was)
+        : "v"(g), "s"(base)
+        : "memory");
+}
 
 template <typename X4>
 __device__ __forceinline__ void split4x2(const f32x4 v, X4& hi, X4& lo) {
@@ -130,7 +155,7 @@
 #define KSTAMP(i) do {} while (0)
 #endif
 
-template <int W, bool RELKEY, typename E, bool DROP = false, bool PLANES = false>
+template <int W, bool RELKEY, typename E, bool DROP = false, bool PLANES = false, bool INP = false>
 __global__ __launch_bounds__(W * 64, 2) void attn_coop_kernel(
     const float* __restrict__ q, int64_t q_bs, int64_t q_rs, const float* __restrict__ k, int64_t k_bs,
     int64_t k_rs, const float* __restrict__ v, int64_t v_bs, int64_t v_rs, const typename AV<E>::x8* __restrict__ e_frag,
@@ -146,14 +171,39 @@
     const int blk = xcd_remap(blockIdx.x, gridDim.x);
     const int grp = blk % groups_per_bh, bh = blk / groups_per_bh, h = bh % nh, b = bh / nh;
     const int q0 = (grp * W + wid) * 32;
-    float* ring = reinterpret_cast<float*>(smem_raw + 2 * KV_BUF_B) + wid * RING_F;
+    float* ring = reinterpret_cast<float*>(smem_raw + (INP ? 2 * IN_BUF_B + Lk * 4 : 2 * KV_BUF_B)) + wid * RING_F;
+    float* const bias_row = reinterpret_cast<float*>(smem_raw + 2 * IN_BUF_B);
     KSTAMP(0);
 
     const float* kb_ = k + b * k_bs + h * D;
     const float* vb_ = v + b * v_bs + h * D;
     const float* mb = key_mask ? key_mask + (int64_t)b * Lk : nullptr;
+    const unsigned char* kv_src = nullptr;
+    int64_t kv_tile_b = 0;
+    auto issue_tile = [&](int kt, unsigned char* buf) {
+        const unsigned char* g = kv_src + kt * kv_tile_b;
+        unsigned char* l = buf + wid * 4096;
+        glds16x4(g, l);
+    };
+    bf16x8 qf[4][2];
+    if constexpr (INP) {
+        const bool vw = wid >= 2;
+        const int64_t nks = vw ? v_rs : k_rs;
+        kv_tile_b = nks * 2048;
+        kv_src = reinterpret_cast<const unsigned char*>(vw ? v : k) + (((int64_t)b * Lk) >> 5) * kv_tile_b + h * 8192 + (wid & 1) * 4096 +
+                 lane * 16;
+        issue_tile(0, smem_raw);
+        asm volatile("" ::: "memory");
+        __builtin_amdgcn_sched_barrier(0);
+        const unsigned char* qp = reinterpret_cast<const unsigned char*>(q) + ((((int64_t)b * Lq + q0) >> 5) * q_rs + 4 * h) * 2048 + lane * 16;
+#pragma unroll
+        for (int kb = 0; kb < 4; ++kb) {
+            qf[kb][0] = *reinterpret_cast<const bf16x8*>(qp + kb * 2048);
+            qf[kb][1] = *reinterpret_cast<const bf16x8*>(qp + kb * 2048 + 1024);
+        }
+    }
     f32x4 qraw[8];
-    {
+    if constexpr (!INP) {
         const float* qrow = q + b * q_bs + (int64_t)min(q0 + qi, Lq - 1) * q_rs + h * D + 8 * half;
 #pragma unroll
         for (int kb = 0; kb < 4; ++kb) {
@@ -166,12 +216,14 @@
     const bool scan_mask = mb && skip_padded_tiles && e3d_mask_skip_is_exact(bnd);
     float mv[4];
     {
-        const float* mp = mb ? mb : kb_;
+        const float* mp = mb ? mb : (INP ? k : kb_);
 #pragma unroll
         for (int c = 0; c < 4; ++c) mv[c] = mp[min(64 * c + lane, Lk - 1)];
     }
-
-    bf16x8 qf[4][2];
+    if constexpr (INP) {
+        for (int key = tid; key < Lk; key += NT) bias_row[key] = (1.0f - (mb ? mb[key] : 1.0f)) * MASK_BIAS;
+    }
+
     int k_tiles = (Lk + 31) >> 5;
 
     constexpr bool DEEP = NI <= 2;
@@ -248,7 +300,7 @@
         return dot_q_acc(x, acc);
     };
 
-    stage_load(Set0{}, 0);
+    if constexpr (!INP) stage_load(Set0{}, 0);
     if (RELKEY) e_load(qt + J0);
 
     if (scan_mask) {
@@ -268,7 +320,7 @@
         if (last >= 0) k_tiles = (last >> 5) + 1;
     }
 #pragma unroll
-    for (int kb = 0; kb < 4; ++kb) {
+    for (int kb = 0; kb < 4 && !INP; ++kb) {
         const f32x4 lo4 = qraw[2 * kb], hi4 = qraw[2 * kb + 1];
         float x[8] = {lo4[0] * Q_SCALE, lo4[1] * Q_SCALE, lo4[2] * Q_SCALE, lo4[3] * Q_SCALE,
                       hi4[0] * Q_SCALE, hi4[1] * Q_SCALE, hi4[2] * Q_SCALE, hi4[3] * Q_SCALE};
@@ -286,9 +338,15 @@
 #pragma unroll
         for (int r = 0; r < 16; ++r) ring[mfma32_row(r, half) * RING_LD + qi] = t[r];
     }
-    stage_store(Set0{}, 0, smem_raw);
-    if (DEEP) stage_load(Set1{}, (k_tiles > 1 ? 1 : 0) * 32);
-    __syncthreads();
+    if constexpr (INP) {
+        if (RELKEY) E3D_VMCNT(8);
+        else E3D_VMCNT(0);
+        E3D_LDS_BARRIER();
+    } else {
+        stage_store(Set0{}, 0, smem_raw);
+        if (DEEP) stage_load(Set1{}, (k_tiles > 1 ? 1 : 0) * 32);
+        __syncthreads();
+    }
     KSTAMP(1);
 
     f32x16 o0, o1;
@@ -305,13 +363,17 @@
 
     auto tile = [&](auto par_tag, int kt) {
         constexpr int PAR = decltype(par_tag)::value;
-        const unsigned char* buf = smem_raw + PAR * KV_BUF_B;
+        const unsigned char* buf = smem_raw + PAR * (INP ? IN_BUF_B : KV_BUF_B);
         const bool more = kt + 1 < k_tiles;
         const int kt_next = more ? kt + 1 : kt;
         ASTAMP(0);
+        if constexpr (INP) {
+            issue_tile(kt_next, smem_raw + (PAR ^ 1) * IN_BUF_B);
+            asm volatile("" ::: "memory");
+        }
         ASTAMP(1);
 
-        const float* kbias = reinterpret_cast<const float*>(buf + 2 * K_PLANE_B + 2 * V_PLANE_B);
+        const float* kbias = INP ? bias_row + 32 * kt : reinterpret_cast<const float*>(buf + 2 * K_PLANE_B + 2 * V_PLANE_B);
         f32x16 s;
 #pragma unroll
         for (int g = 0; g < 4; ++g) {
@@ -326,18 +388,20 @@
         }
         {
             bf16x8 kf[4][2];
-            const unsigned char* kr = buf + qi * K_ROW_B + 16 * half;
+            const unsigned char* kr = INP ? buf + lane * 16 : buf + qi * K_ROW_B + 16 * half;
 #pragma unroll
             for (int kb = 0; kb < 4; ++kb) {
-                kf[kb][0] = *reinterpret_cast<const bf16x8*>(kr + 32 * kb);
-                kf[kb][1] = *reinterpret_cast<const bf16x8*>(kr + K_PLANE_B + 32 * kb);
+                kf[kb][0] = *reinterpret_cast<const bf16x8*>(kr + (INP ? 2048 : 32) * kb);
+                kf[kb][1] = *reinterpret_cast<const bf16x8*>(kr + (INP ? 1024 : K_PLANE_B) + (INP ? 2048 : 32) * kb);
             }
             s = dot_q_acc(kf, s);
         }
         ASTAMP(2);
-        const int kt_ld = DEEP ? (kt + 2 < k_tiles ? kt + 2 : k_tiles - 1) : kt_next;
-        if (PAR == 0) stage_load(Set0{}, kt_ld * 32);
-        else stage_load(Set1{}, kt_ld * 32);
+        if constexpr (!INP) {
+            const int kt_ld = DEEP ? (kt + 2 < k_tiles ? kt + 2 : k_tiles - 1) : kt_next;
+            if (PAR == 0) stage_load(Set0{}, kt_ld * 32);
+            else stage_load(Set1{}, kt_ld * 32);
+        }
         ASTAMP(3);
 
         float tmax = -INFINITY;
@@ -373,6 +437,10 @@
 
         const unsigned char* vr = buf + 2 * K_PLANE_B + (4 * half + ((lane >> 2) & 3)) * V_ROW_B +
                                   2 * (16 * ((lane >> 4) & 1) + 4 * (lane & 3));
+        const int vg = (lane >> 4) & 1, vp1 = (lane >> 1) & 1;
+        const unsigned char* vq0 = buf + 8192 + vg * 2048 +
+                                   (((lane >> 2) & 3) + 4 * (half ^ vp1) + 8 * vg + 32 * vp1) * 16 + 8 * (lane & 1);
+        const unsigned char* vq1 = vq0 + (vg ? -128 : 128);
 #pragma unroll
         for (int st = 0; st < 2; ++st) {
             float pv[8];
@@ -383,26 +451,41 @@
             const unsigned char* v0 = vr + 16 * st * V_ROW_B;
 #pragma unroll
             for (int pl = 0; pl < 2; ++pl) {
-                a0[pl] = tr_read8<bf16x8>(v0 + pl * V_PLANE_B, v0 + pl * V_PLANE_B + 8 * V_ROW_B);
-                a1[pl] = tr_read8<bf16x8>(v0 + pl * V_PLANE_B + 64, v0 + pl * V_PLANE_B + 8 * V_ROW_B + 64);
+                if constexpr (INP) {
+                    a0[pl] = tr_read8<bf16x8>(vq0 + st * 256 + pl * 1024, vq1 + st * 256 + pl * 1024);
+                    a1[pl] = tr_read8<bf16x8>(vq0 + st * 256 + pl * 1024 + 4096, vq1 + st * 256 + pl * 1024 + 4096);
+                } else {
+                    a0[pl] = tr_read8<bf16x8>(v0 + pl * V_PLANE_B, v0 + pl * V_PLANE_B + 8 * V_ROW_B);
+                    a1[pl] = tr_read8<bf16x8>(v0 + pl * V_PLANE_B + 64, v0 + pl * V_PLANE_B + 8 * V_ROW_B + 64);
+                }
             }
             o0 = mfma3(a0, pb, o0);
             o1 = mfma3(a1, pb, o1);
         }
 
         ASTAMP(5);
-        if (more) {
+        if (more && !INP) {
             if (DEEP == (PAR == 0)) stage_store(Set1{}, kt_next * 32, smem_raw + (PAR ^ 1) * KV_BUF_B);
             else stage_store(Set0{}, kt_next * 32, smem_raw + (PAR ^ 1) * KV_BUF_B);
         }
         ASTAMP(6);
+        bool counted = false;
         if (RELKEY && more) {
             const f32x16 t = dot_q(ef);
             e_load(qt - (kt + 2 < k_tiles ? kt + 2 : k_tiles - 1) - 1 + J0);
 #pragma unroll
             for (int r = 0; r < 16; ++r) ring_w[(32 * (PAR ^ 1) + (r & 3) + 8 * (r >> 2)) * RING_LD] = t[r];
-        }
-        __syncthreads();
+            if constexpr (INP) {
+                E3D_VMCNT(8);
+                counted = true;
+            }
+        }
+        if constexpr (INP) {
+            if (!counted) E3D_VMCNT(0);
+            E3D_LDS_BARRIER();
+        } else {
+            __syncthreads();
+        }
         ASTAMP(7);
     };
     for (int kt = 0; kt < k_tiles; kt += 2) {
@@ -536,6 +619,80 @@
     return coop_launch_t<__bf16>(a, skip, bnd, e_scratch, e_ready, drop, planes, s);
 }
 
+template <typename E>
+__global__ __launch_bounds__(256) void attn_operand_planes_kernel(const float* __restrict__ X, int64_t ldx, int64_t pieces, int nks,
+                                                                  int q_cols, int v_col0, int v_col1, unsigned char* __restrict__ out) {
+    const int lane = threadIdx.x & 63;
+    const int64_t piece = (int64_t)blockIdx.x * 4 + (threadIdx.x >> 6);
+    if (piece >= pieces) return;
+    const int64_t rb = piece / nks;
+    const int ks = (int)(piece % nks), col = ks * 16 + 8 * (lane >> 5);
+    const float* src = X + (rb * 32 + (lane & 31)) * ldx + col;
+    const f32x4 a = *reinterpret_cast<const f32x4*>(src), c = *reinterpret_cast<const f32x4*>(src + 4);
+    float x[8] = {a[0], a[1], a[2], a[3], c[0], c[1], c[2], c[3]};
+    if (col < q_cols) {
+#pragma unroll
+        for (int j = 0; j < 8; ++j) {
+            x[j] *= Q_SCALE;
+            asm volatile("" : "+v"(x[j]));
+        }
+    }
+    typename AV<E>::x8 hi, lo;
+    split8x2(x, hi, lo);
+    const int chunk = (col >= v_col0 && col < v_col1) ? lane ^ E3D_VPLANE_CHUNK(lane >> 5, ks & 1) : lane;
+    unsigned char* dst = out + piece * 2048 + chunk * 16;
+    *reinterpret_cast<typename AV<E>::x8*>(dst) = hi;
+    *reinterpret_cast<typename AV<E>::x8*>(dst + 1024) = lo;
+}
+
+int e3d_attn_operand_planes_launch(const float* X, int64_t ldx, int M, int N, int f16, int q_cols, int v_col0, int v_col1,
+                                   void* planes, hipStream_t s) {
+    const int64_t pieces = (int64_t)(M / 32) * (N / 16);
+    const dim3 grid((unsigned)((pieces + 3) / 4)), block(256);
+    if (f16)
+        hipLaunchKernelGGL(attn_operand_planes_kernel<_Float16>, grid, block, 0, s, X, ldx, pieces, N / 16, q_cols, v_col0, v_col1,
+                           (unsigned char*)planes);
+    else
+        hipLaunchKernelGGL(attn_operand_planes_kernel<__bf16>, grid, block, 0, s, X, ldx, pieces, N / 16, q_cols, v_col0, v_col1,
+                           (unsigned char*)planes);
+    return e3d_launch_status("e3d_attn_operand_planes_f32_split");
+}
+
+template <bool RELKEY, typename E>
+static int launch_in_planes(const E3dAttnFwd& a, const void* e_frag, int skip, E3dBounds bnd, bool planes_out, hipStream_t s) {
+    const size_t lds = 2 * IN_BUF_B + (size_t)a.Lk * 4 + (size_t)4 * RING_F * sizeof(float);
+    const int groups = a.Lq / 128;
+    const E3dAttnDrop drop{0.f, e3d_drop_make(0.f, 0)};
+    auto go = [&](auto kernel, std::atomic<uint64_t>& ok) {
+        e3d_allow_lds(ok, kernel, lds);
+        hipLaunchKernelGGL(kernel, dim3(a.B * a.nh * groups), dim3(256), lds, s, E3D_VIEW(a.q), E3D_VIEW(a.k), E3D_VIEW(a.v),
+                           reinterpret_cast<const typename AV<E>::x8*>(e_frag), a.P, a.key_mask, a.out, (float*)nullptr, a.nh, a.Lq,
+                           a.Lk, groups, skip, bnd, g_rescale_tau, drop.d);
+        return e3d_launch_status("e3d_relkey_attn_fwd_split_in_planes (cooperative)");
+    };
+    static std::atomic<uint64_t> ok_f{0}, ok_p{0};
+    if (planes_out) return go(attn_coop_kernel<4, RELKEY, E, false, true, true>, ok_p);
+    return go(attn_coop_kernel<4, RELKEY, E, false, false, true>, ok_f);
+}
+
+int e3d_attn_coop_launch_in_planes(const E3dAttnFwd& a, int skip, E3dBounds bnd, void* e_scratch, int e_ready, int f16,
+                                   bool planes_out, hipStream_t s) {
+    if (a.dist_emb) {
+        if (!e_scratch) {
+            e3d_set_error("attn_coop: rel-key attention needs the caller's scratch for the distance-table planes");
+            return -1;
+        }
+        if (!e_ready) {
+            const int rc = e3d_attn_fill_planes(a.dist_emb, a.P, a.Lk, e_scratch, f16, nullptr, s);
+            if (rc) return rc;
+        }
+        return f16 ? launch_in_planes<true, _Float16>(a, e_scratch, skip, bnd, planes_out, s)
+                   : launch_in_planes<true, __bf16>(a, e_scratch, skip, bnd, planes_out, s);
+    }
+    return f16 ? launch_in_planes<false, _Float16>(a, nullptr, skip, bnd, planes_out, s)
+               : launch_in_planes<false, __bf16>(a, nullptr, skip, bnd, planes_out, s);
+}
+
 extern "C" float e3d_attn_rescale_tau(float tau) {
     const float prev = g_rescale_tau;
     if (tau >= 0.f) g_rescale_tau = tau;
diff --git a/e3-invaraint-diffusion-model_amd/csrc/attn_relkey_split.hip b/e3-invaraint-diffusion-model_amd/csrc/attn_relkey_split.hip
--- a/e3-invaraint-diffusion-model_amd/csrc/attn_relkey_split.hip
+++ b/e3-invaraint-diffusion-model_amd/csrc/attn_relkey_split.hip
@@ -310,3 +310,57 @@
                              terms, {0.f, e3d_drop_make(0.f, 0)}, e_scratch, e_scratch_ready, q_absmax, k_absmax, e_absmax, stream,
                              true);
 }
+
+extern "C" int e3d_attn_operand_planes_f32_split(const float* X, int64_t ldx, int M, int N, int terms, int q_cols, int v_col0,
+                                                 int v_col1, void* planes, void* stream) {
+    E3D_REQUIRE(X && planes, "attn_operand_planes: null pointer");
+    E3D_REQUIRE(M > 0 && N > 0 && M % 32 == 0 && N % 64 == 0 && ldx >= N && ldx % 4 == 0 && ((uintptr_t)X % 16) == 0 &&
+                    ((uintptr_t)planes % 16) == 0,
+                "attn_operand_planes: need M%%32==0, N%%64==0, ldx%%4==0, 16-byte alignment (M=%d N=%d)", M, N);
+    E3D_REQUIRE(q_cols >= 0 && q_cols <= N && q_cols % 64 == 0 && v_col0 >= 0 && v_col0 <= v_col1 && v_col1 <= N && v_col0 % 64 == 0 &&
+                    v_col1 % 64 == 0, "attn_operand_planes: column ranges must be whole heads inside [0, N] (q_cols=%d v=[%d, %d))",
+                q_cols, v_col0, v_col1);
+    E3D_REQUIRE(terms == 3 || terms == E3D_TERMS_F16X3, "attn_operand_planes: terms must be 3 or 19 (got %d)", terms);
+    return e3d_attn_operand_planes_launch(X, ldx, M, N, terms == E3D_TERMS_F16X3, q_cols, v_col0, v_col1, planes, (hipStream_t)stream);
+}
+
+extern "C" int e3d_attn_in_planes_supported(int Lq, int Lk, int terms, int have_scratch) {
+    return (terms == 3 || terms == E3D_TERMS_F16X3) && Lq > 0 && Lq % 128 == 0 && Lk > 0 && Lk % 32 == 0 && Lk <= 8192 &&
+           attn_coop_ok(64, (int64_t)Lk * 64, 64, Lq, Lk, terms, false, have_scratch != 0) && e3d_attn_coop_waves(Lq) == 4;
+}
+
+extern "C" int e3d_relkey_attn_fwd_split_in_planes(const void* q_planes, int q_nks, int q_k16, const void* kv_planes, int kv_nks,
+                                                   int k_k16, int v_k16, const float* dist_emb, int P, const float* key_mask,
+                                                   void* out, int out_planes, int B, int nh, int Lq, int Lk, int terms,
+                                                   void* e_scratch, int e_scratch_ready, const float* q_absmax,
+                                                   const float* k_absmax, float* e_absmax, void* stream) {
+    E3D_REQUIRE(q_planes && kv_planes && out, "attn_split (operand planes): null pointer");
+    E3D_REQUIRE(B > 0 && nh > 0 && (int64_t)B * nh * ((Lq + 31) / 32) < (1ll << 30), "attn_split (operand planes): bad shape B=%d nh=%d",
+                B, nh);
+    E3D_REQUIRE(e3d_attn_in_planes_supported(Lq, Lk, terms, !dist_emb || e_scratch),
+                "attn_split (operand planes): needs the 4-wave cooperative kernel, Lq %% 128 == 0, Lk %% 32 == 0 (Lq=%d Lk=%d terms=%d)",
+                Lq, Lk, terms);
+    E3D_REQUIRE(q_k16 >= 0 && q_k16 + 4 * nh <= q_nks && k_k16 >= 0 && k_k16 + 4 * nh <= kv_nks && v_k16 >= 0 && v_k16 + 4 * nh <= kv_nks &&
+                    q_k16 % 4 == 0 && k_k16 % 4 == 0 && v_k16 % 4 == 0,
+                "attn_split (operand planes): k16 ranges outside the buffers (q %d+%d/%d, k %d, v %d /%d)", q_k16, 4 * nh, q_nks, k_k16,
+                v_k16, kv_nks);
+    E3D_REQUIRE(((uintptr_t)q_planes % 16) == 0 && ((uintptr_t)kv_planes % 16) == 0 && ((uintptr_t)out % 16) == 0,
+                "attn_split (operand planes): pointers must be 16B aligned");
+    E3D_REQUIRE(!dist_emb || (Lq == Lk && Lq <= P && ((uintptr_t)dist_emb % 16) == 0),
+                "attn_split (operand planes): relative_key needs Lq == Lk <= P and a 16B-aligned table (Lq=%d Lk=%d P=%d)", Lq, Lk, P);
+    E3D_REQUIRE(!dist_emb || !q_absmax || e_absmax, "attn_split (operand planes): rel-key attention with element bounds needs e_absmax too");
+    const E3dBounds bnd{q_absmax, k_absmax, dist_emb ? e_absmax : nullptr};
+    const int f16 = terms == E3D_TERMS_F16X3;
+    hipStream_t s = (hipStream_t)stream;
+    if (dist_emb && !e_scratch_ready) {
+        const int rc = e3d_attn_fill_planes(dist_emb, P, Lk, e_scratch, f16, e_absmax, s);
+        if (rc) return rc;
+    }
+    const unsigned char* qb = reinterpret_cast<const unsigned char*>(q_planes) + (int64_t)q_k16 * 2048;
+    const unsigned char* kb = reinterpret_cast<const unsigned char*>(kv_planes) + (int64_t)k_k16 * 2048;
+    const unsigned char* vb = reinterpret_cast<const unsigned char*>(kv_planes) + (int64_t)v_k16 * 2048;
+    const E3dAttnFwd a{{reinterpret_cast<const float*>(qb), 0, q_nks}, {reinterpret_cast<const float*>(kb), 0, kv_nks},
+                       {reinterpret_cast<const float*>(vb), 0, kv_nks}, dist_emb, P, key_mask, reinterpret_cast<float*>(out), nullptr,
+                       B, nh, Lq, Lk};
+    return e3d_attn_coop_launch_in_planes(a, g_skip_padded, bnd, e_scratch, 1, f16, out_planes != 0, s);
+}
diff --git a/e3-invaraint-diffusion-model_amd/csrc/e3d_common.h b/e3-invaraint-diffusion-model_amd/csrc/e3d_common.h
--- a/e3-invaraint-diffusion-model_amd/csrc/e3d_common.h
+++ b/e3-invaraint-diffusion-model_amd/csrc/e3d_common.h
@@ -242,6 +242,13 @@
 int e3d_attn_coop_launch(const E3dAttnFwd& a, int skip, E3dBounds bnd, void* e_scratch, int e_ready, int f16,
                          const E3dAttnDrop& drop, bool planes, hipStream_t s);
 int e3d_attn_coop_waves(int Lq);
+int e3d_attn_coop_launch_in_planes(const E3dAttnFwd& a, int skip, E3dBounds bnd, void* e_scratch, int e_ready, int f16,
+                                   bool planes_out, hipStream_t s);
+int e3d_attn_operand_planes_launch(const float* X, int64_t ldx, int M, int N, int f16, int q_cols, int v_col0, int v_col1,
+                                   void* planes, hipStream_t s);
+
+constexpr float E3D_ATTN_Q_SCALE = 0.125f * 1.4426950408889634f;
+#define E3D_VPLANE_CHUNK(dim_bit3, dim_bit4) (4 * (dim_bit3) + 8 * (dim_bit4))
 
 struct E3dBwdLayout { int64_t Pm, dSm, part, chunk_sums, unit_live, total; };
 E3dBwdLayout e3d_attn_bwd_layout(int B, int nh, int Lq, int Lk, bool relkey);
diff --git a/e3-invaraint-diffusion-model_amd/csrc/gemm_split.hip b/e3-invaraint-diffusion-model_amd/csrc/gemm_split.hip
--- a/e3-invaraint-diffusion-model_amd/csrc/gemm_split.hip
+++ b/e3-invaraint-diffusion-model_amd/csrc/gemm_split.hip
@@ -741,13 +741,13 @@
 #define E3D_STORE_OUT(ptr, val) (*(ptr) = (val))
 #endif
 
-template <int ACT, typename E, bool PLANES = false>
+template <int ACT, typename E, int PLANES = 0>
 __global__ __launch_bounds__(512, 2) void gemm_split256p_kernel(const float* __restrict__ A, int64_t lda,
                                                                  const float* __restrict__ W,
                                                                  const float* __restrict__ bias,
                                                                  float* __restrict__ out, int64_t ldc, int N, int K,
                                                                  int tiles_m, int tiles_n, float* __restrict__ absmax, float out_scale,
-                                                                 const int* __restrict__ run_if) {
+                                                                 const int* __restrict__ run_if, int q_cols, int v_col0, int v_col1) {
     if (run_if && *run_if == 0) return;
     extern __shared__ __attribute__((aligned(16))) unsigned char smem_raw[];
     constexpr int NS = 2, T_BYTES = BT * ROW64, BUF_BYTES = 2 * NS * T_BYTES;
@@ -864,7 +864,7 @@
         if constexpr (PLANES) {
             const int lid = xcd_remap(tile, total);
             const int row0 = (lid / tiles_n) * BT, col0 = (lid % tiles_n) * BT;
-            unsigned char* const ob = reinterpret_cast<unsigned char*>(out) + lane * 16;
+            unsigned char* const ob = reinterpret_cast<unsigned char*>(out) + (PLANES == 2 ? 0 : lane * 16);
             const int nks = N >> 4;
 #pragma unroll
             for (int n = 0; n < 2; ++n) {
@@ -881,6 +881,15 @@
                 for (int r = 0; r < 16; ++r) {
                     bl[r] = half ? bs[8 * (r >> 2) + 4 + (r & 3)] : bs[8 * (r >> 2) + (r & 3)];
                     asm volatile("" : "+v"(bl[r]));
+                }
+                float q_mul = 1.0f;
+                int chunk_b[2] = {lane * 16, lane * 16};
+                if constexpr (PLANES == 2) {
+                    if (colb < q_cols) q_mul = E3D_ATTN_Q_SCALE;
+                    if (colb >= v_col0 && colb < v_col1) {
+                        chunk_b[0] = (lane ^ E3D_VPLANE_CHUNK(half, 0)) * 16;
+                        chunk_b[1] = (lane ^ E3D_VPLANE_CHUNK(half, 1)) * 16;
+                    }
                 }
 #pragma unroll
                 for (int m = 0; m < 4; ++m) {
@@ -897,6 +906,12 @@
                             if (ACT == E3D_ACT_NONE && absmax) { e3d_absmax_accum(amax, a); e3d_absmax_accum(amax, c); }
                             asm volatile("" : "+v"(a));
                             asm volatile("" : "+v"(c));
+                            if constexpr (PLANES == 2) {
+                                a *= q_mul;
+                                c *= q_mul;
+                                asm volatile("" : "+v"(a));
+                                asm volatile("" : "+v"(c));
+                            }
                             const auto sw = __builtin_amdgcn_permlane32_swap(__float_as_uint(a), __float_as_uint(c), false, false);
                             x0[j] = __uint_as_float(sw[0]);
                             x1[j] = __uint_as_float(sw[1]);
@@ -905,8 +920,9 @@
                         split4<2, E>(x0, p0);
                         split4<2, E>(x1, p1);
                         typedef typename Vec<E>::x8 X8;
-                        *reinterpret_cast<X8*>(o + kl * 2048) = __builtin_shufflevector(p0[0], p1[0], 0, 1, 2, 3, 4, 5, 6, 7);
-                        *reinterpret_cast<X8*>(o + kl * 2048 + 1024) = __builtin_shufflevector(p0[1], p1[1], 0, 1, 2, 3, 4, 5, 6, 7);
+                        unsigned char* const ok = PLANES == 2 ? o + chunk_b[kl] : o;
+                        *reinterpret_cast<X8*>(ok + kl * 2048) = __builtin_shufflevector(p0[0], p1[0], 0, 1, 2, 3, 4, 5, 6, 7);
+                        *reinterpret_cast<X8*>(ok + kl * 2048 + 1024) = __builtin_shufflevector(p0[1], p1[1], 0, 1, 2, 3, 4, 5, 6, 7);
                     }
                 }
             }
@@ -935,9 +951,9 @@
     if (ACT == E3D_ACT_NONE && absmax) e3d_absmax_commit(amax, absmax, lane);
 }
 
-template <int ACT, typename E, bool PLANES = false>
+template <int ACT, typename E, int PLANES = 0>
 int launch256p(const float* A, int64_t lda, const float* W, const float* bias, float* out, int64_t ldc, int M, int N,
-               int K, Epi epi, hipStream_t s) {
+               int K, Epi epi, hipStream_t s, int q_cols = 0, int v_col0 = 0, int v_col1 = 0) {
     const int tiles_m = M / BT, tiles_n = N / BT;
     constexpr size_t lds = 2 * 2 * 2 * BT * ROW64;
     static std::atomic<uint64_t> lds_ok{0};
@@ -945,7 +961,7 @@
     const int total = tiles_m * tiles_n;
     e3d_allow_lds(lds_ok, gemm_split256p_kernel<ACT, E, PLANES>, lds);
     hipLaunchKernelGGL((gemm_split256p_kernel<ACT, E, PLANES>), dim3(total < n_cu ? total : n_cu), dim3(512), lds, s, A, lda, W, bias, out,
-                       ldc, N, K, tiles_m, tiles_n, epi.absmax, epi.scale, epi.run_if);
+                       ldc, N, K, tiles_m, tiles_n, epi.absmax, epi.scale, epi.run_if, q_cols, v_col0, v_col1);
     return e3d_launch_status(PLANES ? "e3d_gemm_bias_act_planes_split (persistent 256x256)" : "e3d_gemm_f32_split (persistent 256x256)");
 }
 
@@ -1313,3 +1329,24 @@
     if (act == E3D_ACT_GELU) return launch256p<E3D_ACT_GELU, _Float16, true>(A, lda, W, bias, out, N, M, N, K, epi, s);
     return launch256p<E3D_ACT_NONE, _Float16, true>(A, lda, W, bias, out, N, M, N, K, epi, s);
 }
+
+extern "C" int e3d_gemm_attn_planes_supported(int M, int N, int K, int64_t lda, int terms, int q_cols, int v_col0, int v_col1) {
+    return e3d_gemm_planes_supported(M, N, K, lda, E3D_ACT_NONE, terms) && q_cols >= 0 && q_cols <= N && q_cols % 64 == 0 &&
+           v_col0 >= 0 && v_col0 <= v_col1 && v_col1 <= N && v_col0 % 64 == 0 && v_col1 % 64 == 0 && (q_cols <= v_col0 || v_col0 == v_col1);
+}
+
+extern "C" int e3d_gemm_bias_act_attn_planes_split(const float* A, int64_t lda, const float* W, const float* bias, void* out_planes,
+                                                   int M, int N, int K, int terms, int q_cols, int v_col0, int v_col1,
+                                                   float* out_absmax, float out_scale, void* stream) {
+    E3D_REQUIRE(A && W && out_planes, "gemm_split (attention planes): null pointer");
+    E3D_REQUIRE(e3d_gemm_attn_planes_supported(M, N, K, lda, terms, q_cols, v_col0, v_col1),
+                "gemm_split (attention planes): needs the persistent kernel and whole-head column ranges (M=%d N=%d K=%d terms=%d q_cols=%d "
+                "v=[%d, %d))", M, N, K, terms, q_cols, v_col0, v_col1);
+    E3D_REQUIRE(((uintptr_t)A % 16) == 0 && ((uintptr_t)W % 16) == 0 && ((uintptr_t)bias % 16) == 0 && ((uintptr_t)out_planes % 16) == 0,
+                "gemm_split (attention planes): A, W, bias and the planes must be 16-byte aligned");
+    const Epi epi{out_absmax, out_scale, 0, nullptr};
+    hipStream_t s = (hipStream_t)stream;
+    float* out = reinterpret_cast<float*>(out_planes);
+    if (terms == 3) return launch256p<E3D_ACT_NONE, __bf16, 2>(A, lda, W, bias, out, N, M, N, K, epi, s, q_cols, v_col0, v_col1);
+    return launch256p<E3D_ACT_NONE, _Float16, 2>(A, lda, W, bias, out, N, M, N, K, epi, s, q_cols, v_col0, v_col1);
+}
diff --git a/e3-invaraint-diffusion-model_amd/hip.py b/e3-invaraint-diffusion-model_amd/hip.py
--- a/e3-invaraint-diffusion-model_amd/hip.py
+++ b/e3-invaraint-diffusion-model_amd/hip.py
@@ -65,6 +65,13 @@
     "e3d_gemm_bias_act_planes_split": (c_int, [_P, c_int64, _P, _P, _P, c_int, c_int, c_int, c_int, c_int, _P, c_float, _P]),
     "e3d_attn_planes_supported": (c_int, [c_int64, c_int64, c_int64, c_int, c_int, c_int, c_int]),
     "e3d_relkey_attn_fwd_split_planes": (c_int, _QKV + [_P] + _SHAPE + [c_int] + _BOUNDS + _STREAM),
+    "e3d_attn_operand_planes_f32_split": (c_int, [_P, c_int64, c_int, c_int, c_int, c_int, c_int, c_int, _P, _P]),
+    "e3d_gemm_attn_planes_supported": (c_int, [c_int, c_int, c_int, c_int64, c_int, c_int, c_int, c_int]),
+    "e3d_gemm_bias_act_attn_planes_split": (c_int, [_P, c_int64, _P, _P, _P, c_int, c_int, c_int, c_int, c_int, c_int, c_int, _P,
+                                                    c_float, _P]),
+    "e3d_attn_in_planes_supported": (c_int, [c_int, c_int, c_int, c_int]),
+    "e3d_relkey_attn_fwd_split_in_planes": (c_int, [_P, c_int, c_int, _P, c_int, c_int, c_int, _P, c_int, _P, _P, c_int] + _SHAPE +
+                                            [c_int] + _BOUNDS + _STREAM),
     "e3d_gemm_wgrad_ragged_f32_split": (c_int, [_P, _P, _P, _P, _P, _P, _P, _P, c_uint64, c_int, c_int, c_int, _P]),
     "e3d_relkey_attn_bwd_workspace_floats": (c_int64, [c_int, c_int, c_int, c_int, c_int]),
     "e3d_relkey_attn_bwd": (c_int, _ATTN_BWD + _STREAM),
diff --git a/e3-invaraint-diffusion-model_amd/ops.py b/e3-invaraint-diffusion-model_amd/ops.py
--- a/e3-invaraint-diffusion-model_amd/ops.py
+++ b/e3-invaraint-diffusion-model_amd/ops.py
@@ -644,6 +644,136 @@
             and bool(hip.lib().e3d_attn_planes_supported(k.stride(0), Lk * v.stride(0), v.stride(0), Lq, Lk, terms, 1)))
 
 
+QKV_PLANES = {"1": True, "0": False}.get(os.environ.get("E3D_QKV_PLANES", "1"))
+if QKV_PLANES is None:
+    raise ValueError(f"E3D_QKV_PLANES must be 1 or 0, got {os.environ['E3D_QKV_PLANES']!r}")
+QKV_PLANES_CALLS = 0
+
+
+class AttnPlanes:
+    __slots__ = ("data", "shape", "terms", "q_cols", "v_col0", "v_col1", "_e3d_absmax")
+    requires_grad = False
+
+    def __init__(self, data, M, N, terms, q_cols, v_col0, v_col1):
+        self.data, self.shape, self.terms = data, (M, N), terms
+        self.q_cols, self.v_col0, self.v_col1 = q_cols, v_col0, v_col1
+
+    @property
+    def device(self):
+        return self.data.device
+
+    def decode(self):
+        M, N = self.shape
+        dt = torch.float16 if self.terms == 19 else torch.bfloat16
+        t = self.data.view(dt).view(M // 32, N // 16, 2, 64, 8).clone()
+        lane = torch.arange(64, device=t.device)
+        for ks in range(self.v_col0 // 16, self.v_col1 // 16):
+            t[:, ks] = t[:, ks][:, :, lane ^ (4 * (lane >> 5) + 8 * (ks & 1))]
+        t = t.view(M // 32, N // 16, 2, 2, 32, 8).permute(2, 0, 4, 1, 3, 5).reshape(2, M, N)
+        return t[0], t[1]
+
+
+def attn_operand_planes(x, q_cols, v_col0, v_col1, mode=None):
+    _chk(x, "attn_operand_planes.x")
+    M, N = x.shape
+    terms = GEMM_MODES[ATTN_MODE if mode is None else mode]
+    if terms not in (3, 19) or x.stride(1) != 1:
+        raise ValueError(f"attn_operand_planes: unsupported input / terms {terms}")
+    out = torch.empty((M * N * 4,), dtype=torch.uint8, device=x.device)
+    hip.check(hip.lib().e3d_attn_operand_planes_f32_split(_p(x), x.stride(0), M, N, terms, q_cols, v_col0, v_col1, _p(out),
+                                                          _stream()), "e3d_attn_operand_planes_f32_split")
+    return AttnPlanes(out, M, N, terms, q_cols, v_col0, v_col1)
+
+
+def gemm_attn_planes(a, weight, bias, q_cols, v_col0, v_col1, mode=None, absmax=None):
+    _chk(a, "gemm_attn_planes.a"); _chk(weight, "gemm_attn_planes.weight"); _chk(bias, "gemm_attn_planes.bias")
+    assert a.dim() == 2 and a.stride(1) == 1 and weight.is_contiguous()
+    M, K = a.shape
+    N = weight.shape[0]
+    terms = GEMM_MODES[GEMM_MODE if mode is None else mode]
+    assert weight.shape[1] == K and terms in (3, 19)
+    if absmax is not None:
+        _chk(absmax, "gemm_attn_planes.absmax")
+        assert absmax.numel() == 1
+    scale = 1.0
+    if terms == 19:
+        weight, scale = f16_weight(weight)
+    out = torch.empty((M * N * 4,), device=a.device, dtype=torch.uint8)
+    with _timed("gemm", (M, N, K, ACT_NONE)):
+        hip.check(hip.lib().e3d_gemm_bias_act_attn_planes_split(_p(a), a.stride(0), _p(weight), _p(bias), _p(out), M, N, K, terms,
+                                                                q_cols, v_col0, v_col1, _p(absmax), scale, _stream()),
+                  "e3d_gemm_bias_act_attn_planes_split")
+    return AttnPlanes(out, M, N, terms, q_cols, v_col0, v_col1)
+
+
+def qkv_planes_ok(a, weight, bias, Lq, Lk, mode=None):
+    if not QKV_PLANES or torch.is_grad_enabled():
+        return False
+    terms = GEMM_MODES[GEMM_MODE if mode is None else mode]
+    if terms != GEMM_MODES[ATTN_MODE] or terms not in (3, 19):
+        return False
+    M, K = a.shape
+    N = weight.shape[0]
+    return (a.stride(1) == 1 and a.data_ptr() % 16 == 0 and (bias is None or bias.data_ptr() % 16 == 0) and N % 64 == 0
+            and not (_skinny_ok(terms, M, N, K, a) and M <= min(SKINNY_MAX_M, SKINNY_GEMM_MAX_M))
+            and bool(hip.lib().e3d_gemm_attn_planes_supported(M, N, K, a.stride(0), terms, 0, 0, 0))
+            and bool(hip.lib().e3d_attn_in_planes_supported(Lq, Lk, terms, 1)))
+
+
+def attention_in_planes(q_src, kv_src, B, nh, Lq, Lk, key_mask=None, dist_emb=None, max_pos=0, bounds=None, planes_out=False):
+    global QKV_PLANES_CALLS
+    H = nh * 64
+    kv = q_src if kv_src is None else kv_src
+    k_col = H if kv_src is None else 0
+    terms = q_src.terms
+    if (kv.terms != terms or q_src.q_cols != H or kv.v_col0 != k_col + H or kv.v_col1 != k_col + 2 * H
+            or q_src.shape[0] != B * Lq or kv.shape[0] != B * Lk or (kv_src is not None and kv.q_cols != 0)):
+        raise ValueError("attention_in_planes: the operand planes do not hold Q | K | V (or Q and K | V) of this call")
+    _chk(q_src.data, "attention_in_planes.q", torch.uint8); _chk(kv.data, "attention_in_planes.kv", torch.uint8)
+    _chk(key_mask, "attention_in_planes.key_mask"); _chk(dist_emb, "attention_in_planes.dist_emb")
+    if key_mask is not None:
+        assert key_mask.is_contiguous() and key_mask.shape == (B, Lk)
+    if dist_emb is not None:
+        assert dist_emb.is_contiguous() and dist_emb.shape == (2 * max_pos - 1, 64), dist_emb.shape
+    if planes_out:
+        out = torch.empty((B * Lq * H * 4,), device=q_src.device, dtype=torch.uint8)
+    else:
+        out = torch.empty((B * Lq, H), device=q_src.device, dtype=torch.float32)
+    with _timed("attn_relkey" if dist_emb is not None else "attn_cross", (B, nh, Lq, Lk)):
+        scratch, ready, e_abs = None, 0, None
+        q_abs, k_abs = bounds if bounds is not None else (None, None)
+        if dist_emb is not None:
+            ent = getattr(dist_emb, "_e3d_planes", None)
+            if ent is not None and ent[0] == weight_key(dist_emb) + (Lk, terms):
+                scratch, ready, e_abs = ent[1], 1, ent[2]
+            else:
+                scratch = torch.empty((hip.lib().e3d_attn_scratch_bytes(Lk),), device=q_src.device, dtype=torch.uint8)
+                if q_abs is not None and k_abs is not None:
+                    e_abs = torch.zeros(1, device=q_src.device, dtype=torch.float32)
+                if not torch.cuda.is_current_stream_capturing():
+                    try:
+                        if e_abs is None:
+                            e_abs = absmax(dist_emb.detach())
+                        dist_emb._e3d_planes = (weight_key(dist_emb) + (Lk, terms), scratch, e_abs)
+                    except AttributeError:
+                        pass
+        if q_abs is None or k_abs is None or (dist_emb is not None and e_abs is None):
+            q_abs = k_abs = e_abs = None
+        hip.check(hip.lib().e3d_relkey_attn_fwd_split_in_planes(
+            _p(q_src.data), q_src.shape[1] // 16, 0, _p(kv.data), kv.shape[1] // 16, k_col // 16, (k_col + H) // 16, _p(dist_emb),
+            max_pos, _p(key_mask), _p(out), int(planes_out), B, nh, Lq, Lk, terms, _p(scratch), ready, _p(q_abs), _p(k_abs),
+            _p(e_abs), _stream()), "e3d_relkey_attn_fwd_split_in_planes")
+    QKV_PLANES_CALLS += 1
+    return ActPlanes(out, B * Lq, H, terms) if planes_out else out
+
+
+def attention_planes_ok_in(M, nh, out_features, residual=None):
+    if ACT_PLANES not in (True, "attn") or torch.is_grad_enabled():
+        return False
+    terms = GEMM_MODES[ATTN_MODE]
+    return terms == GEMM_MODES[GEMM_MODE] and terms in (3, 19) and rowln_ok(terms, M, out_features, nh * 64, None, residual)
+
+
 def linear_residual_layernorm(a, weight, bias, residual, gamma, beta, eps, mode=None):
     M, K = a.shape
     H = weight.shape[0]
diff --git a/e3-invaraint-diffusion-model_amd/structure_model/model.py b/e3-invaraint-diffusion-model_amd/structure_model/model.py
--- a/e3-invaraint-diffusion-model_amd/structure_model/model.py
+++ b/e3-invaraint-diffusion-model_amd/structure_model/model.py
@@ -38,7 +38,7 @@
         self.angles_predictor = Predictor(decoder_config.hidden_size, feature_size)
 
     def encode_receptor(self, receptor_seq, receptor_angles, receptor_attention_masks,
-                        project_cross_kv=True, layout=None) -> ReceptorCache:
+                        project_cross_kv=True, layout=None, ligand_len=None) -> ReceptorCache:
         require_gpu(receptor_seq, receptor_angles, receptor_attention_masks)
         B, L = receptor_angles.shape[:2]
         ops.reset_absmax(receptor_angles.device)
@@ -61,7 +61,8 @@
         x = bert.run_encoder(self.encoder, x, mask, B, L, row_keys=rk)
         kv = None
         if project_cross_kv:
-            kv = [bert.project_cross_kv(layer.crossattention, x) for layer in self.decoder.layer]
+            kv = [bert.project_cross_kv(layer.crossattention, x, ligand_len, L if ligand_len is not None else None)
+                  for layer in self.decoder.layer]
         return ReceptorCache(x, kv, mask, B, L)
 
     def timestep_modulation(self, timesteps):
diff --git a/e3-invaraint-diffusion-model_amd/structure_model/sample.py b/e3-invaraint-diffusion-model_amd/structure_model/sample.py
--- a/e3-invaraint-diffusion-model_amd/structure_model/sample.py
+++ b/e3-invaraint-diffusion-model_amd/structure_model/sample.py
@@ -220,7 +220,8 @@
         t_index = int(t_unique.item())
         t_dev = timestep.to(device=x_t.device, dtype=torch.long).contiguous()
     if receptor_cache is None:
-        receptor_cache = model.encode_receptor(receptor_seq, receptor_angle, receptor_mask)
+        receptor_cache = model.encode_receptor(receptor_seq, receptor_angle, receptor_mask,
+                                               ligand_len=x_t.shape[1] if layout is None else None)
     eps_hat = model.decode(timestep, x_t, ligand_mask, receptor_cache, mod=mod, layout=layout)
     x = plan.update(x_t.contiguous().float(), eps_hat, t_dev, noise, out, wrap, t_index)
     return plan.compose(x, t_dev, known_noise, t_index)
@@ -299,12 +300,12 @@
     ids = None if seed is None else keyed.item_ids(item_ids, x.shape[0])
     frame = packing.Frame(ligand_mask, receptor_mask, trim=trim_padding, pack=pack)
     layout, pocket_layout = frame.layouts or (None, None)
+    x = frame.ligand(x)
     if pocket_layout is None:
         cache = model.encode_receptor(frame.pocket(receptor_seq), frame.pocket(receptor_angle),
-                                      frame.pocket(receptor_mask))
+                                      frame.pocket(receptor_mask), ligand_len=x.shape[1])
     else:
         cache = model.encode_receptor(receptor_seq, receptor_angle, receptor_mask, layout=pocket_layout)
-    x = frame.ligand(x)
     mask = None if layout is not None else frame.ligand(ligand_mask).contiguous().float()
     if noises is not None:
         noises = frame.ligand(noises.to(x.device).float(), dim=1)
diff --git a/include/e3d_hip.h b/include/e3d_hip.h
--- a/include/e3d_hip.h
+++ b/include/e3d_hip.h
@@ -301,6 +301,19 @@
                                      const float* dist_emb, int P, const float* key_mask, void* out_planes,
                                      int B, int nh, int Lq, int Lk, int terms, void* e_scratch, int e_scratch_ready,
                                      const float* q_absmax, const float* k_absmax, float* e_absmax, void* stream);
+
+int e3d_attn_operand_planes_f32_split(const float* X, int64_t ldx, int M, int N, int terms, int q_cols, int v_col0, int v_col1,
+                                      void* planes, void* stream);
+int e3d_gemm_attn_planes_supported(int M, int N, int K, int64_t lda, int terms, int q_cols, int v_col0, int v_col1);
+int e3d_gemm_bias_act_attn_planes_split(const float* A, int64_t lda, const float* W, const float* bias, void* out_planes,
+                                        int M, int N, int K, int terms, int q_cols, int v_col0, int v_col1, float* out_absmax,
+                                        float out_scale, void* stream);
+int e3d_attn_in_planes_supported(int Lq, int Lk, int terms, int have_scratch);
+int e3d_relkey_attn_fwd_split_in_planes(const void* q_planes, int q_nks, int q_k16, const void* kv_planes, int kv_nks,
+                                        int k_k16, int v_k16, const float* dist_emb, int P, const float* key_mask, void* out,
+                                        int out_planes, int B, int nh, int Lq, int Lk, int terms, void* e_scratch,
+                                        int e_scratch_ready, const float* q_absmax, const float* k_absmax, float* e_absmax,
+                                        void* stream);
 
 int e3d_adamw_step_dyn(float* const* params, const float* const* grads, float* const* exp_avg, float* const* exp_avg_sq,
                        const int64_t* numel, const int* chunk_tensor, const int64_t* chunk_first, int n_chunks,
```

Result: no change. 4322 pocket-steps/s, median of 6 (+1.0%).
